# soham97/mellow

Hardware: AMD Instinct MI355X
Metric: audio-pair responses/sec (v0 167M, 2x10s clips, max_len=64, greedy) (higher is better)
Workload: dtype f32 (encoder/prefill GEMM operands split EXACTLY into 3 bf16 terms, 6 bf16 MFMA products per fp32 product, f32 accumulate: fp32-accurate, parity suite green; mel included, the STFT is an fp32 FFT; attentions and decode on exact fp32 MFMA / VALU)

## Files before the change

### mellow_amd/csrc/decode.hip

```cpp
#include "common.h"
#include "kernels.h"
#include <cstdio>
#include <mutex>
#include <set>
#include <type_traits>
#include <utility>

namespace mellow {

__device__ uint64_t* g_kdbg = nullptr;
#ifdef MELLOW_KDEBUG
__device__ __forceinline__ void kstamp(int slot, int idx, bool who) {
    if (g_kdbg && who) g_kdbg[slot * 8 + idx] = __builtin_readcyclecounter();
}
__device__ __forceinline__ void kspan(int seq, int end) {
    if (g_kdbg && seq >= 0 && seq < 480 && threadIdx.x == 0) {
        const unsigned long long t = wall_clock64();
        if (end) atomicMax(reinterpret_cast<unsigned long long*>(g_kdbg) + 64 + 2 * seq + 1, t);
        else atomicMin(reinterpret_cast<unsigned long long*>(g_kdbg) + 64 + 2 * seq, t);
    }
}
#else
#define kstamp(slot, idx, who) ((void)0)
#define kspan(seq, end) ((void)0)
#endif
void set_kernel_debug_buffer(uint64_t* p) { (void)hipMemcpyToSymbol(HIP_SYMBOL(g_kdbg), &p, sizeof(p)); }

__device__ __forceinline__ float fast_exp(float x) { return __builtin_amdgcn_exp2f(x * 1.44269504088896340736f); }
#ifdef MELLOW_NO_BLK_EXIT
#define MELLOW_BLK_EXIT(RB)
#else
#define MELLOW_BLK_EXIT(RB) if (BLK) { if (a.blk_live[RB] == 0) return; }
#endif
__device__ __forceinline__ float4 ldg_nt(const float4* p) {
#ifdef MELLOW_NO_NT
    return *p;
#else
    const f32x4 v = __builtin_nontemporal_load(reinterpret_cast<const f32x4*>(p));
    return make_float4(v[0], v[1], v[2], v[3]);
#endif
}
template <bool W8>
__device__ __forceinline__ float4 ldw(const float* __restrict__ Wp, int64_t slot) {
    if constexpr (W8) {
        const uint32_t u = __builtin_nontemporal_load(reinterpret_cast<const uint32_t*>(Wp) + slot);
        const auto lo = __builtin_amdgcn_cvt_pk_f32_fp8(u, false), hi = __builtin_amdgcn_cvt_pk_f32_fp8(u, true);
        return make_float4(lo[0], lo[1], hi[0], hi[1]);
    } else {
        return ldg_nt(reinterpret_cast<const float4*>(Wp) + slot);
    }
}
__device__ __forceinline__ uint32_t ldw8(const float* __restrict__ Wp, int64_t slot) {
    return __builtin_nontemporal_load(reinterpret_cast<const uint32_t*>(Wp) + slot);
}
__device__ __forceinline__ float f4amax(float4 v) { return fmaxf(fmaxf(fabsf(v.x), fabsf(v.y)), fmaxf(fabsf(v.z), fabsf(v.w))); }
__device__ __forceinline__ uint32_t q4_e4m3(float4 v, float inv) {
    int w = 0;
    w = __builtin_amdgcn_cvt_pk_fp8_f32(v.x * inv, v.y * inv, w, false);
    w = __builtin_amdgcn_cvt_pk_fp8_f32(v.z * inv, v.w * inv, w, true);
    return (uint32_t)w;
}
__device__ __forceinline__ long pk64(uint32_t lo, uint32_t hi) { return (long)(((uint64_t)hi << 32) | (uint64_t)lo); }
template <int N>
__device__ __forceinline__ f32x16 mfma8_32(f32x16 acc, const uint32_t (&w)[N], const uint32_t (&x)[N]) {
#pragma unroll
    for (int i = 0; i < N; i += 2)
        acc = __builtin_amdgcn_mfma_f32_32x32x16_fp8_fp8(pk64(w[i], i + 1 < N ? w[i + 1] : 0u), pk64(x[i], i + 1 < N ? x[i + 1] : 0u), acc, 0, 0, 0);
    return acc;
}
template <int N>
__device__ __forceinline__ f32x4 mfma8_16(f32x4 acc, const uint32_t (&w)[N], const uint32_t (&x)[N]) {
#pragma unroll
    for (int i = 0; i < N; i += 2)
        acc = __builtin_amdgcn_mfma_f32_16x16x32_fp8_fp8(pk64(w[i], i + 1 < N ? w[i + 1] : 0u), pk64(x[i], i + 1 < N ? x[i + 1] : 0u), acc, 0, 0, 0);
    return acc;
}
__device__ __forceinline__ void a8_scales(float amax, float& inv, float& sc) {
    inv = amax > 0.f ? 448.0f / amax : 0.f;
    sc = amax * (1.0f / 448.0f);
}
#ifndef MELLOW_ST_MODE
#define MELLOW_ST_MODE 0
#endif
__device__ __forceinline__ void st_out(float4* p, float4 v) {
#if MELLOW_ST_MODE == 1
    __builtin_nontemporal_store(f32x4{v.x, v.y, v.z, v.w}, reinterpret_cast<f32x4*>(p));
#elif MELLOW_ST_MODE == 2
    const f32x4 r = {v.x, v.y, v.z, v.w};
    asm volatile("global_store_dwordx4 %0, %1, off sc0 sc1" ::"v"(p), "v"(r) : "memory");
#else
    *p = v;
#endif
}
#ifdef MELLOW_HOIST_ON
#define MELLOW_HOIST(x) asm volatile("" ::"s"(x))
#else
#define MELLOW_HOIST(x) ((void)0)
#endif
__device__ __forceinline__ float4 f4add(float4 a, float4 b) { return make_float4(a.x + b.x, a.y + b.y, a.z + b.z, a.w + b.w); }
__device__ __forceinline__ float f4ssq(float4 v) { return (v.x * v.x + v.y * v.y) + (v.z * v.z + v.w * v.w); }
__device__ __forceinline__ f32x16 mfma4(f32x16 acc, float4 w, float4 x) {
    acc = __builtin_amdgcn_mfma_f32_32x32x2f32(w.x, x.x, acc, 0, 0, 0);
    acc = __builtin_amdgcn_mfma_f32_32x32x2f32(w.y, x.y, acc, 0, 0, 0);
    acc = __builtin_amdgcn_mfma_f32_32x32x2f32(w.z, x.z, acc, 0, 0, 0);
    acc = __builtin_amdgcn_mfma_f32_32x32x2f32(w.w, x.w, acc, 0, 0, 0);
    return acc;
}
__device__ __forceinline__ int64_t f32_idx(int rb, int K8, int m, int k) {
    return ((int64_t)rb * K8 + (k >> 3)) * 64 + m + 32 * ((k >> 2) & 1);
}

__device__ __forceinline__ void split_pair(float4 a, float4 b, i32x4& p0, i32x4& p1, i32x4& p2) {
    const float v[8] = {a.x, a.y, a.z, a.w, b.x, b.y, b.z, b.w};
    split8(v, p0, p1, p2);
}
#define MELLOW_BF16(W, X, ACC) ACC = __builtin_amdgcn_mfma_f32_32x32x16_bf16(__builtin_bit_cast(bf16x8, W), __builtin_bit_cast(bf16x8, X), ACC, 0, 0, 0)
__device__ __forceinline__ f32x16 mma6(f32x16 acc, const i32x4 (&w)[3], const i32x4 (&x)[3]) {
    MELLOW_BF16(w[2], x[0], acc);
    MELLOW_BF16(w[0], x[2], acc);
    MELLOW_BF16(w[1], x[1], acc);
    MELLOW_BF16(w[1], x[0], acc);
    MELLOW_BF16(w[0], x[1], acc);
    MELLOW_BF16(w[0], x[0], acc);
    return acc;
}

struct F3Quad { uint2 p[3]; };
__device__ __forceinline__ F3Quad f3_split4(float4 y) {
    __bf16 h[4], m[4], l[4];
    split3(y.x, h[0], m[0], l[0]); split3(y.y, h[1], m[1], l[1]); split3(y.z, h[2], m[2], l[2]); split3(y.w, h[3], m[3], l[3]);
    typedef __bf16 bf16x4 __attribute__((ext_vector_type(4)));
    F3Quad q;
    q.p[0] = __builtin_bit_cast(uint2, bf16x4{h[0], h[1], h[2], h[3]});
    q.p[1] = __builtin_bit_cast(uint2, bf16x4{m[0], m[1], m[2], m[3]});
    q.p[2] = __builtin_bit_cast(uint2, bf16x4{l[0], l[1], l[2], l[3]});
    return q;
}
__device__ __forceinline__ unsigned dpp_xor1(unsigned v) { return (unsigned)__builtin_amdgcn_update_dpp(0, (int)v, 0xB1, 0xF, 0xF, true); }
__device__ __forceinline__ F3Quad f3_partner(const F3Quad& q) {
    F3Quad o;
#pragma unroll
    for (int c = 0; c < 3; ++c) { o.p[c].x = dpp_xor1(q.p[c].x); o.p[c].y = dpp_xor1(q.p[c].y); }
    return o;
}
__device__ __forceinline__ void f3_store8(void* base, int64_t slot0, const F3Quad& lo, const F3Quad& hi) {
    uint4* p = reinterpret_cast<uint4*>(base) + slot0;
    p[0] = make_uint4(lo.p[0].x, lo.p[0].y, hi.p[0].x, hi.p[0].y);
    p[64] = make_uint4(lo.p[1].x, lo.p[1].y, hi.p[1].x, hi.p[1].y);
    p[128] = make_uint4(lo.p[2].x, lo.p[2].y, hi.p[2].x, hi.p[2].y);
}
__device__ __forceinline__ int64_t f3_32_slot(int rb, int KP, int m, int k) {
    return ((int64_t)rb * KP + (k >> 4)) * 3 * 64 + m + 32 * ((k >> 3) & 1);
}
__device__ __forceinline__ int64_t f3_16_slot(int rb, int KP, int m, int k) {
    return (((int64_t)rb * KP + (k >> 5)) * 2 + (m >> 4)) * 3 * 64 + (m & 15) + 16 * ((k >> 3) & 3);
}
__device__ __forceinline__ void pair_natural(float4& a, float4& b) {
    float* pa = &a.x; float* pb = &b.x;
#pragma unroll
    for (int j = 0; j < 4; ++j) {
        auto r = __builtin_amdgcn_permlane32_swap(__float_as_uint(pa[j]), __float_as_uint(pb[j]), false, false);
        pa[j] = __uint_as_float(r[0]);
        pb[j] = __uint_as_float(r[1]);
    }
}

#ifndef MELLOW_QKV_WAVES
#define MELLOW_QKV_WAVES 9
#endif
constexpr int QW = MELLOW_QKV_WAVES;
constexpr int QKV_THREADS = QW * 64 < 256 ? 256 : QW * 64;
template <int KCD, bool BLK, bool FIRST, int W8>
__global__ __launch_bounds__(QKV_THREADS) void dec_qkv_kernel(const float* __restrict__ Wp, const float* __restrict__ xmidF_p,
                                                              const float* __restrict__ dslabF_p, int K8p, const DecArgs a,
                                                              const float* __restrict__ wscale) {
    kspan(a.dbg_seq, 0);
    __shared__ __attribute__((aligned(16))) float red[QW * 16 * 64];
    __shared__ float ssq_s[QW * 32];
    const int tid = threadIdx.x, lane = tid & 63, wave = tid >> 6;
    const int nt = blockIdx.x, kc = blockIdx.y, rb = blockIdx.z;
    constexpr int KPW = 72 / (DEC_KC_QKV * QW);
    if (FIRST && nt == 29 && kc == 0 && rb == 0 && tid < 32) {
        const int p = *a.d_pos + a.inc_pos;
        const float c = a.rope_cos[(int64_t)p * 32 + tid], sn = a.rope_sin[(int64_t)p * 32 + tid];
        a.rope_cur[tid] = c;
        a.rope_cur[32 + tid] = sn;
        if (tid == 0 && a.inc_pos) *a.d_pos = p;
    }
    MELLOW_BLK_EXIT(rb)
    if (wave < QW) {
        const int k8_0 = (kc * QW + wave) * KPW;
        const int64_t wslot = ((int64_t)nt * K8p + k8_0) * 64 + lane;
        const float4* xb = reinterpret_cast<const float4*>(xmidF_p) + ((int64_t)rb * 72 + k8_0) * 64 + lane;
        const float4* sb = reinterpret_cast<const float4*>(dslabF_p) + ((int64_t)rb * 72 + k8_0) * 64 + lane;
        float4 w[KPW], x[KPW], sl[KPW][KCD > 0 ? KCD : 1];
        uint32_t w8[KPW];
#pragma unroll
        for (int i = 0; i < KPW; ++i) {
            if constexpr (W8 == 2) w8[i] = ldw8(Wp, wslot + i * 64);
            else w[i] = ldw<W8 != 0>(Wp, wslot + i * 64);
            x[i] = xb[i * 64];
#pragma unroll
            for (int s = 0; s < KCD; ++s) sl[i][s] = sb[(int64_t)s * a.slabF_stride4 + i * 64];
        }
        MELLOW_HOIST(a.pq); MELLOW_HOIST(a.rows); MELLOW_HOIST(a.ssq1); MELLOW_HOIST(a.xnewR);
        if (W8) MELLOW_HOIST(wscale);
        __builtin_amdgcn_sched_barrier(0);
        f32x16 acc;
#pragma unroll
        for (int r = 0; r < 16; ++r) acc[r] = 0.f;
        float ssp = 0.f;
#pragma unroll
        for (int i = 0; i < KPW; ++i) {
            float4 xv = x[i];
#pragma unroll
            for (int s = 0; s < KCD; ++s) xv = f4add(xv, sl[i][s]);
            if constexpr (W8 == 2) x[i] = xv;
            else acc = mfma4(acc, w[i], xv);
            if (nt == 0) ssp += f4ssq(xv);
            if (nt == 1)
                *reinterpret_cast<float4*>(a.xnewR + ((int64_t)rb * 32 + (lane & 31)) * 576 + (k8_0 + i) * 8 + (lane >> 5) * 4) = xv;
        }
        if constexpr (W8 == 2) {
            float am = 0.f, inv, sc;
#pragma unroll
            for (int i = 0; i < KPW; ++i) am = fmaxf(am, f4amax(x[i]));
            a8_scales(half_max(am), inv, sc);
            uint32_t xq[KPW];
#pragma unroll
            for (int i = 0; i < KPW; ++i) xq[i] = q4_e4m3(x[i], inv);
            acc = mfma8_32<KPW>(acc, w8, xq);
#pragma unroll
            for (int r = 0; r < 16; ++r) acc[r] *= sc;
        }
        if (nt == 0) {
            ssp = half_sum(ssp);
            if (lane < 32) ssq_s[wave * 32 + lane] = ssp;
        }
#pragma unroll
        for (int r = 0; r < 16; ++r) red[(wave * 16 + r) * 64 + lane] = acc[r];
    }
    __syncthreads();
    if (nt == 0 && tid < 32)
    {
        float ssum = ssq_s[tid & 31];
// ... 576 lines not shown
            acc = __builtin_amdgcn_mfma_f32_16x16x4f32(w[i].z, O.z * inv, acc, 0, 0, 0);
            acc = __builtin_amdgcn_mfma_f32_16x16x4f32(w[i].w, O.w * inv, acc, 0, 0, 0);
        }
    }
    if constexpr (W8 == 2) {
        float am = 0.f, inv, sc;
#pragma unroll
        for (int i = 0; i < TPW; ++i) am = fmaxf(am, f4amax(os[i][0]));
        am = fmaxf(am, swz_xor16(am));
        a8_scales(half_max(am), inv, sc);
        uint32_t xq[TPW];
#pragma unroll
        for (int i = 0; i < TPW; ++i) xq[i] = q4_e4m3(os[i][0], inv);
        acc = mfma8_16<TPW>(acc, w8, xq);
#pragma unroll
        for (int r = 0; r < 4; ++r) acc[r] *= sc;
    }
#pragma unroll
    for (int r = 0; r < 4; ++r) red[(wave * 4 + r) * 64 + lane] = acc[r];
    __syncthreads();
    if (tid < 64 && erow_ok) {
        const int src_lane = em + 16 * enq;
        float v[4] = {0.f, 0.f, 0.f, 0.f};
#pragma unroll
        for (int wv = 0; wv < OP_WAVES; ++wv)
#pragma unroll
            for (int r = 0; r < 4; ++r) v[r] += red[(wv * 4 + r) * 64 + src_lane];
        if (W8) {
#pragma unroll
            for (int r = 0; r < 4; ++r) v[r] *= wscale[nt * 16 + enq * 4 + r];
        }
        const float4 y = make_float4(xres.x + v[0], xres.y + v[1], xres.z + v[2], xres.w + v[3]);
        const int k = nt * 16 + enq * 4;
        st_out(reinterpret_cast<float4*>(a.xmidF) + f32_idx(rb, 72, mh * 16 + em, k), y);
        if (a.xmid3_32) {
            const F3Quad yq = f3_split4(y), yo = f3_partner(yq);
            if (!(enq & 1)) {
                f3_store8(a.xmid3_32, f3_32_slot(rb, 36, mh * 16 + em, k), yq, yo);
                f3_store8(a.xmid3_16, f3_16_slot(rb, 18, mh * 16 + em, k), yq, yo);
            }
        } else
        st_out(reinterpret_cast<float4*>(a.xmidF16) + (((int64_t)rb * 36 + nt) * 2 + mh) * 64 + em + 16 * enq, y);
        float ss = f4ssq(y);
        ss += dpp_mov<0xB1>(ss);
        ss += dpp_mov<0x4E>(ss);
        if (enq == 0) a.ssq[erow * 40 + nt] = ss;
    }
    kspan(a.dbg_seq, 1);
}

enum { OUT_LOGITS = 1 };
#ifndef MELLOW_LM_WAVES
#define MELLOW_LM_WAVES 8
#endif
constexpr int LM_WAVES = MELLOW_LM_WAVES;
template <int OUT, bool BLK, int W8>
__global__ __launch_bounds__(LM_WAVES * 64) void dec_fullk_kernel(const float* __restrict__ Wp, const float* __restrict__ XF, int K8p,
                                                        int N, const DecArgs a, const float* __restrict__ wscale) {
    kspan(a.dbg_seq, 0);
    __shared__ __attribute__((aligned(16))) float red[LM_WAVES * 16 * 64];
    constexpr int KPW = 72 / LM_WAVES;
    const int tid = threadIdx.x, lane = tid & 63, wave = tid >> 6;
    const int nt = blockIdx.x, rb = blockIdx.z;
    MELLOW_BLK_EXIT(rb)
    const int k8_0 = wave * KPW;
    const int64_t wslot = ((int64_t)nt * K8p + k8_0) * 64 + lane;
    const float4* xp = reinterpret_cast<const float4*>(XF) + ((int64_t)rb * 72 + k8_0) * 64 + lane;
    float4 w[KPW], x[KPW];
    uint32_t w8[KPW];
    const bool dbg = tid == 0 && nt == 0 && rb == 0;
    const int dslot = 5;
    kstamp(dslot, 0, dbg);
#pragma unroll
    for (int i = 0; i < KPW; ++i) {
        if constexpr (W8 == 2) w8[i] = ldw8(Wp, wslot + i * 64);
        else w[i] = ldw<W8 != 0>(Wp, wslot + i * 64);
        x[i] = xp[i * 64];
    }
    MELLOW_HOIST(a.logits); MELLOW_HOIST(a.cand_val); MELLOW_HOIST(a.cand_idx); MELLOW_HOIST(N);
    if (W8) MELLOW_HOIST(wscale);
    __builtin_amdgcn_sched_barrier(0);
    kstamp(dslot, 1, dbg);
    f32x16 acc;
#pragma unroll
    for (int r = 0; r < 16; ++r) acc[r] = 0.f;
    if constexpr (W8 == 2) {
        float am = 0.f, inv, sc;
#pragma unroll
        for (int i = 0; i < KPW; ++i) am = fmaxf(am, f4amax(x[i]));
        a8_scales(half_max(am), inv, sc);
        uint32_t xq[KPW];
#pragma unroll
        for (int i = 0; i < KPW; ++i) xq[i] = q4_e4m3(x[i], inv);
        acc = mfma8_32<KPW>(acc, w8, xq);
#pragma unroll
        for (int r = 0; r < 16; ++r) acc[r] *= sc;
    } else {
#pragma unroll
        for (int i = 0; i < KPW; ++i) acc = mfma4(acc, w[i], x[i]);
    }
    kstamp(dslot, 2, dbg && acc[0] == acc[0]);
#pragma unroll
    for (int r = 0; r < 16; ++r) red[(wave * 16 + r) * 64 + lane] = acc[r];
    __syncthreads();
    kstamp(dslot, 3, dbg);
    const bool epi = tid < 256;
    const int mm = tid & 31, hh = (tid >> 5) & 1, gq = (tid >> 6) & 3;
    float v[4];
#pragma unroll
    for (int j = 0; j < 4; ++j) {
        const int r = 4 * gq + j;
        float sacc = red[r * 64 + mm + 32 * hh];
#pragma unroll
        for (int wv = 1; wv < LM_WAVES; ++wv) sacc += red[(wv * 16 + r) * 64 + mm + 32 * hh];
        v[j] = sacc;
    }
    {
        const int n = nt * 32 + 8 * gq + 4 * hh;
        if (W8) {
#pragma unroll
            for (int j = 0; j < 4; ++j) v[j] *= wscale[n + j];
        }
        const int64_t row = (int64_t)rb * 32 + mm;
        if (epi && a.logits && n < N) *reinterpret_cast<float4*>(a.logits + row * N + n) = make_float4(v[0], v[1], v[2], v[3]);
        __syncthreads();
        float bv = v[0];
        int bi = n;
#pragma unroll
        for (int j = 1; j < 4; ++j)
            if (arg_better(v[j], n + j, bv, bi)) { bv = v[j]; bi = n + j; }
        if (epi) {
            red[tid] = bv;
            reinterpret_cast<int*>(red)[256 + tid] = bi;
        }
        __syncthreads();
        if (tid < 32) {
            float best = red[tid];
            int idx = reinterpret_cast<int*>(red)[256 + tid];
#pragma unroll
            for (int q = 1; q < 8; ++q) {
                const float ov = red[tid + 32 * q];
                const int oi = reinterpret_cast<int*>(red)[256 + tid + 32 * q];
                if (arg_better(ov, oi, best, idx)) { best = ov; idx = oi; }
            }
            const int64_t o = ((int64_t)rb * 32 + tid) * (N >> 5) + nt;
            a.cand_val[o] = best;
            a.cand_idx[o] = idx;
        }
    }
    kspan(a.dbg_seq, 1);
}


#ifndef MELLOW_H3_NW
#define MELLOW_H3_NW 8
#endif
#ifndef MELLOW_H3R_D1
#define MELLOW_H3R_D1 1
#endif
#ifndef MELLOW_H3R_D2
#define MELLOW_H3R_D2 1
#endif
#ifndef MELLOW_H3R_D4
#define MELLOW_H3R_D4 1
#endif
constexpr int H3_NW = MELLOW_H3_NW, H3_CP = 3, H3_NC = 36 / H3_CP;
template <int G, int D, bool BLK>
__global__ __launch_bounds__(H3_NW * 64) void dec_head3r_kernel(const float* __restrict__ Wp, const i32x4* __restrict__ X3, int K8p, int N,
                                                                int RB_p, const DecArgs a) {
    kspan(a.dbg_seq, 0);
    extern __shared__ __attribute__((aligned(16))) i32x4 xs[];
    constexpr int PPH = 36 / G, NCH = PPH / H3_CP;
    constexpr int STAGE = G * PPH * 3 * 64;
    static_assert(PPH * G == 36 && NCH * H3_CP == PPH && H3_NC % D == 0 && NCH % D == 0, "phases hold whole chunks");
    const int tid = threadIdx.x, lane = tid & 63, wave = tid >> 6;
    const int nt = blockIdx.x * H3_NW + wave;
    const float4* wbase = reinterpret_cast<const float4*>(Wp) + (int64_t)nt * K8p * 64 + lane;
    for (int rb0 = 0; rb0 < RB_p; rb0 += G) {
        const int gn = min(G, RB_p - rb0);
        f32x16 acc[G];
#pragma unroll
        for (int g = 0; g < G; ++g)
#pragma unroll
            for (int r = 0; r < 16; ++r) acc[g][r] = 0.f;
        float4 wn[D][2 * H3_CP];
#pragma unroll
        for (int d = 0; d < D; ++d)
#pragma unroll
            for (int i = 0; i < 2 * H3_CP; ++i) wn[d][i] = ldg_nt(wbase + (d * 2 * H3_CP + i) * 64);
        for (int ph = 0; ph < G; ++ph) {
            if (ph || rb0) __syncthreads();
            {
                constexpr int FILL = (STAGE + H3_NW * 64 - 1) / (H3_NW * 64);
                i32x4 t[FILL];
#pragma unroll
                for (int j = 0; j < FILL; ++j) {
                    const int i = tid + j * H3_NW * 64;
                    if (i < STAGE) {
                        const int g = i / (PPH * 3 * 64), rest = i % (PPH * 3 * 64);
                        t[j] = X3[(((int64_t)(rb0 + (g < gn ? g : 0)) * 36 + ph * PPH) * 3) * 64 + rest];
                    }
                }
#pragma unroll
                for (int j = 0; j < FILL; ++j) {
                    const int i = tid + j * H3_NW * 64;
                    if (i < STAGE) xs[i] = t[j];
                }
            }
            __syncthreads();
            for (int c0 = 0; c0 < NCH; c0 += D) {
#pragma unroll
                for (int d = 0; d < D; ++d) {
                    const int cc = c0 + d, c = ph * NCH + cc;
                    float4 w[2 * H3_CP];
#pragma unroll
                    for (int i = 0; i < 2 * H3_CP; ++i) w[i] = wn[d][i];
                    if (c + D < H3_NC) {
#pragma unroll
                        for (int i = 0; i < 2 * H3_CP; ++i) wn[d][i] = ldg_nt(wbase + ((c + D) * 2 * H3_CP + i) * 64);
                    }
                    __builtin_amdgcn_sched_barrier(0);
                    i32x4 wp[H3_CP][3];
#pragma unroll
                    for (int p = 0; p < H3_CP; ++p) {
                        pair_natural(w[2 * p], w[2 * p + 1]);
                        split_pair(w[2 * p], w[2 * p + 1], wp[p][0], wp[p][1], wp[p][2]);
                    }
                    const i32x4* st = xs + (cc * H3_CP) * 3 * 64 + lane;
#pragma unroll
                    for (int g = 0; g < G; ++g) {
                        if (g < gn) {
#pragma unroll
                            for (int p = 0; p < H3_CP; ++p) {
                                const i32x4 xq[3] = {st[((g * PPH + p) * 3 + 0) * 64], st[((g * PPH + p) * 3 + 1) * 64], st[((g * PPH + p) * 3 + 2) * 64]};
                                acc[g] = mma6(acc[g], wp[p], xq);
                            }
                        }
                    }
                    __builtin_amdgcn_sched_barrier(0);
                }
            }
        }
        const int m = lane & 31, h = lane >> 5;
#pragma unroll
        for (int g = 0; g < G; ++g) {
            if (g < gn && !(BLK && a.blk_live[rb0 + g] == 0)) {
                const int64_t row = (int64_t)(rb0 + g) * 32 + m;
                float bv = -INFINITY;
                int bi = 0x7fffffff;
#pragma unroll
                for (int q = 0; q < 4; ++q) {
                    const int n = nt * 32 + 8 * q + 4 * h;
                    if (a.logits) *reinterpret_cast<float4*>(a.logits + row * N + n) = make_float4(acc[g][4 * q], acc[g][4 * q + 1], acc[g][4 * q + 2], acc[g][4 * q + 3]);
#pragma unroll
                    for (int j = 0; j < 4; ++j)
                        if (arg_better(acc[g][4 * q + j], n + j, bv, bi)) { bv = acc[g][4 * q + j]; bi = n + j; }
                }
                auto rv = __builtin_amdgcn_permlane32_swap(__float_as_uint(bv), __float_as_uint(bv), false, false);
                auto ri = __builtin_amdgcn_permlane32_swap((unsigned)bi, (unsigned)bi, false, false);
                const float ov = __uint_as_float(h ? rv[0] : rv[1]);
                const int oi = (int)(h ? ri[0] : ri[1]);
                if (arg_better(ov, oi, bv, bi)) { bv = ov; bi = oi; }
                if (h == 0) {
                    const int64_t o = row * (N >> 5) + nt;
                    a.cand_val[o] = bv;
                    a.cand_idx[o] = bi;
                }
            }
        }
    }
    kspan(a.dbg_seq, 1);
}

#define MELLOW_BF16S(W, X, ACC) ACC = __builtin_amdgcn_mfma_f32_16x16x32_bf16(__builtin_bit_cast(bf16x8, W), __builtin_bit_cast(bf16x8, X), ACC, 0, 0, 0)
__device__ __forceinline__ f32x4 mma6s(f32x4 acc, const i32x4 (&w)[3], const i32x4 (&x)[3]) {
    MELLOW_BF16S(w[2], x[0], acc);
    MELLOW_BF16S(w[0], x[2], acc);
    MELLOW_BF16S(w[1], x[1], acc);
    MELLOW_BF16S(w[1], x[0], acc);
    MELLOW_BF16S(w[0], x[1], acc);
    MELLOW_BF16S(w[0], x[0], acc);
    return acc;
}
template <int NP, int NPA>
__device__ __forceinline__ void x3_load(i32x4 (&xq)[NPA][3], const i32x4* __restrict__ x3, int64_t off) {
#pragma unroll
    for (int p = 0; p < NP; ++p)
#pragma unroll
        for (int c = 0; c < 3; ++c) xq[p][c] = x3[off + (p * 3 + c) * 64];
}
template <int NP, int RBM, int NPA>
__device__ __forceinline__ void x3_tile_job(const i32x4 (&wp)[NPA][3], i32x4 (&xq)[2][NPA][3], const i32x4* __restrict__ x3 ,
                                            int64_t rb_stride, int rb0, int gn, f32x16 (&acc)[RBM]) {
#pragma unroll
    for (int g = 0; g < RBM; ++g) {
        if (g < gn) {
            if (g + 1 < RBM && g + 1 < gn) x3_load<NP, NPA>(xq[(g + 1) & 1], x3, (int64_t)(rb0 + g + 1) * rb_stride);
#pragma unroll
            for (int p = 0; p < NP; ++p) acc[g] = mma6(acc[g], wp[p], xq[g & 1][p]);
        }
    }
}
#ifndef MELLOW_Q3_WAVES
#define MELLOW_Q3_WAVES 6
#endif
constexpr int Q3W = MELLOW_Q3_WAVES;
template <int NP, int RBM, bool BLK>
__device__ __forceinline__ void q3_body(const float4* __restrict__ wp4, const i32x4* __restrict__ xsrc, int64_t rb_stride, int nt, int slab,
                                        bool side, int RB_p, const DecArgs& a, float* red) {
    const int tid = threadIdx.x, lane = tid & 63, wave = tid >> 6;
    i32x4 wp[NP][3];
    i32x4 xq[2][NP][3];
    constexpr bool ALL = RBM <= 2;
    {
        float4 w[2 * NP];
#pragma unroll
        for (int i = 0; i < 2 * NP; ++i) w[i] = ldg_nt(wp4 + i * 64);
        x3_load<NP, NP>(xq[0], xsrc, 0);
        if (ALL && RBM == 2 && RB_p > 1) x3_load<NP, NP>(xq[1], xsrc, rb_stride);
        __builtin_amdgcn_sched_barrier(0);
#pragma unroll
        for (int p = 0; p < NP; ++p) {
            pair_natural(w[2 * p], w[2 * p + 1]);
            split_pair(w[2 * p], w[2 * p + 1], wp[p][0], wp[p][1], wp[p][2]);
        }
    }
    for (int rb0 = 0; rb0 < RB_p; rb0 += RBM) {
        const int gn = min(RBM, RB_p - rb0);
        f32x16 acc[RBM];
#pragma unroll
        for (int g = 0; g < RBM; ++g)
#pragma unroll
            for (int r = 0; r < 16; ++r) acc[g][r] = 0.f;
        if (rb0) {
            x3_load<NP, NP>(xq[0], xsrc, (int64_t)rb0 * rb_stride);
            if (ALL && RBM == 2 && gn > 1) x3_load<NP, NP>(xq[1], xsrc, (int64_t)(rb0 + 1) * rb_stride);
        }
        if constexpr (ALL && RBM == 2) {
            if (gn > 1) {
#pragma unroll
                for (int p = 0; p < NP; ++p) {
#define MELLOW_Q3_TERM(PW, PX) MELLOW_BF16(wp[p][PW], xq[0][p][PX], acc[0]); MELLOW_BF16(wp[p][PW], xq[1][p][PX], acc[1]);
                    MELLOW_Q3_TERM(2, 0) MELLOW_Q3_TERM(0, 2) MELLOW_Q3_TERM(1, 1) MELLOW_Q3_TERM(1, 0) MELLOW_Q3_TERM(0, 1) MELLOW_Q3_TERM(0, 0)
#undef MELLOW_Q3_TERM
                }
            } else {
#pragma unroll
                for (int p = 0; p < NP; ++p) acc[0] = mma6(acc[0], wp[p], xq[0][p]);
            }
        } else if constexpr (ALL) {
#pragma unroll
            for (int p = 0; p < NP; ++p) acc[0] = mma6(acc[0], wp[p], xq[0][p]);
        } else {
            x3_tile_job<NP, RBM, NP>(wp, xq, xsrc, rb_stride, rb0, gn, acc);
        }
        if (rb0) __syncthreads();
#pragma unroll
        for (int g = 0; g < RBM; ++g)
#pragma unroll
            for (int r = 0; r < 16; ++r) red[((wave * RBM + g) * 16 + r) * 64 + lane] = acc[g][r];
        __syncthreads();
        if (tid < 256) {
            const int mm = tid & 31, hh = (tid >> 5) & 1, gq = tid >> 6;
            const int n = nt * 32 + 8 * gq + 4 * hh;
            for (int g = 0; g < gn; ++g) {
                const int rb = rb0 + g;
                if (BLK && a.blk_live[rb] == 0) continue;
                float v[4];
#pragma unroll
                for (int j = 0; j < 4; ++j) {
                    const int q = 4 * gq + j;
                    float sacc = red[((0 * RBM + g) * 16 + q) * 64 + mm + 32 * hh];
#pragma unroll
                    for (int wv = 1; wv < Q3W; ++wv) sacc += red[((wv * RBM + g) * 16 + q) * 64 + mm + 32 * hh];
                    v[j] = sacc;
                }
                const float4 o = make_float4(v[0], v[1], v[2], v[3]);
                if (side) st_out(reinterpret_cast<float4*>(a.dslabF) + (int64_t)slab * a.slabF_stride4 + f32_idx(rb, 72, mm, n), o);
                else st_out(reinterpret_cast<float4*>(a.pq + ((int64_t)slab * a.rows + rb * 32 + mm) * 960 + n), o);
            }
        }
    }
}
template <bool BLK, int RBM>
__global__ __launch_bounds__(Q3W * 64) void dec_qkv2x3_kernel(const float* __restrict__ Wx, const float* __restrict__ Wh,
                                                              const float* __restrict__ Wd, const i32x4* __restrict__ xmid3,
                                                              const i32x4* __restrict__ h3, int K8x, int K8h, int RB_p, const DecArgs a) {
    kspan(a.dbg_seq, 0);
    extern __shared__ __attribute__((aligned(16))) float red_dyn[];
    const int lane = threadIdx.x & 63, wave = threadIdx.x >> 6;
    const int b = blockIdx.x;
    constexpr int XP = 18 / Q3W, HP = (96 / Q2_HC) / Q3W;
    static_assert(XP * Q3W == 18 && HP * Q3W * Q2_HC == 96 && Q3W * 64 >= 256, "waves must divide the k-chunks into whole pairs; the epilogue is 256 threads wide");
    if (b < 60) {
        const int nt = b % 30, slab = b / 30;
        const int T0 = slab * 18 + wave * XP;
        q3_body<XP, RBM, BLK>(reinterpret_cast<const float4*>(Wx) + ((int64_t)nt * K8x + 2 * T0) * 64 + lane, xmid3 + (int64_t)T0 * 3 * 64 + lane,
                              (int64_t)36 * 3 * 64, nt, slab, false, RB_p, a, red_dyn);
    } else {
        const int idx = b - 60, hc = idx / 48, nt = idx % 48;
        const bool side = nt >= 30;
        const int T0 = hc * (96 / Q2_HC) + wave * HP;
        const float4* wp4 = side ? reinterpret_cast<const float4*>(Wd) + ((int64_t)(nt - 30) * 192 + 2 * T0) * 64 + lane
                                 : reinterpret_cast<const float4*>(Wh) + ((int64_t)nt * K8h + 2 * T0) * 64 + lane;
        q3_body<HP, RBM, BLK>(wp4, h3 + (int64_t)T0 * 3 * 64 + lane, (int64_t)96 * 3 * 64, side ? nt - 30 : nt, side ? hc : 2 + hc, side, RB_p, a, red_dyn);
    }
    kspan(a.dbg_seq, 1);
}

#ifndef MELLOW_GU3_WAVES
#define MELLOW_GU3_WAVES 6
#endif
#ifndef MELLOW_G3_ABL
#define MELLOW_G3_ABL 0
#endif
constexpr int GU3W = MELLOW_GU3_WAVES;
template <bool BLK, int RBM>
__global__ __launch_bounds__(GU3W * 64) void dec_gateup3_kernel(const float* __restrict__ Wp16, const i32x4* __restrict__ x3,
                                                                const float* __restrict__ ssq_in, int RB_p, const DecArgs a) {
    kspan(a.dbg_seq, 0);
    extern __shared__ __attribute__((aligned(16))) float red_dyn[];
// ... 64 lines not shown
                    for (int p = 0; p < NP; ++p)
#pragma unroll
                        for (int c = 0; c < 6; ++c) xq[(g + 1) & 1][p][c / 3][c % 3] = xsrc[(int64_t)(rb0 + g + 1) * RBS + (p * 6 + c) * 64];
                }
#pragma unroll
                for (int p = 0; p < NP; ++p) {
                    if (MELLOW_G3_ABL & 2) { acc0[g][0] += __int_as_float(wp[p][0][0] ^ xq[g & 1][p][0][0][0]); acc1[g][1] += __int_as_float(wp[p][2][1] ^ xq[g & 1][p][1][2][1]); continue; }
#define MELLOW_G3_TERM(PW, PX) MELLOW_BF16S(wp[p][PW], xq[g & 1][p][0][PX], acc0[g]); MELLOW_BF16S(wp[p][PW], xq[g & 1][p][1][PX], acc1[g]);
                    MELLOW_G3_TERM(2, 0) MELLOW_G3_TERM(0, 2) MELLOW_G3_TERM(1, 1) MELLOW_G3_TERM(1, 0) MELLOW_G3_TERM(0, 1) MELLOW_G3_TERM(0, 0)
#undef MELLOW_G3_TERM
                }
            }
        }
        if (rb0) __syncthreads();
#pragma unroll
        for (int g = 0; g < RBM; ++g)
#pragma unroll
            for (int r = 0; r < 4; ++r) {
                red[((wave * RBM + g) * 8 + r) * 64 + lane] = acc0[g][r];
                red[((wave * RBM + g) * 8 + 4 + r) * 64 + lane] = acc1[g][r];
            }
        __syncthreads();
        static_assert(RBM * 64 <= 2 * GU3W * 64, "two epilogue rounds cover a pass");
#pragma unroll
        for (int k = 0; k < 2; ++k) {
            const int e = tid + k * GU3W * 64;
            if (e >= gn * 64 || (k == 1 && RBM * 64 <= GU3W * 64)) continue;
            const int g = e >> 6, t = e & 63, rb = rb0 + g;
            if (BLK && a.blk_live[rb] == 0) continue;
            const int m = t >> 1, q = t & 1;
            const int gl = (m & 15) + 16 * q, ul = gl + 32, rbase = (m >> 4) * 4;
            float ss = 0.f;
#pragma unroll
            for (int j = 0; j < 9; ++j) ss += (s4[k][j].x + s4[k][j].y) + (s4[k][j].z + s4[k][j].w);
            const float r2 = 1.0f / sqrtf(ss / 576.0f + a.eps);
            float h[4];
#pragma unroll
            for (int r = 0; r < 4; ++r) {
                float gv = red[((0 * RBM + g) * 8 + rbase + r) * 64 + gl], uv = red[((0 * RBM + g) * 8 + rbase + r) * 64 + ul];
#pragma unroll
                for (int wv = 1; wv < GU3W; ++wv) {
                    gv += red[((wv * RBM + g) * 8 + rbase + r) * 64 + gl];
                    uv += red[((wv * RBM + g) * 8 + rbase + r) * 64 + ul];
                }
                h[r] = __fmul_rn(siluf_(gv * r2), uv * r2);
            }
            const float4 hv = make_float4(h[0], h[1], h[2], h[3]);
            if (!(MELLOW_G3_ABL & 16)) st_out(reinterpret_cast<float4*>(a.guF) + ((int64_t)rb * 192 + nt) * 64 + m + 32 * q, hv);
            const F3Quad hq = f3_split4(hv), ho = f3_partner(hq);
            if (!(MELLOW_G3_ABL & 1) && q == 0) f3_store8(a.h3, f3_32_slot(rb, 96, m, 8 * nt), hq, ho);
        }
    }
    kspan(a.dbg_seq, 1);
}

#ifndef MELLOW_GU_WAVES
#define MELLOW_GU_WAVES 4
#endif
constexpr int GU_WAVES = MELLOW_GU_WAVES;
template <bool BLK, int W8>
__global__ __launch_bounds__(GU_WAVES * 64) void dec_gateup16_kernel(const float* __restrict__ Wp16, const float* __restrict__ xF16,
                                                                     const float* __restrict__ ssq_in, const DecArgs a,
                                                                     const float* __restrict__ wscale) {
    kspan(a.dbg_seq, 0);
    __shared__ __attribute__((aligned(16))) float red[GU_WAVES * 8 * 64];
    constexpr int K16 = 36, TPW = K16 / GU_WAVES;
    static_assert(TPW * GU_WAVES == K16, "waves must divide the 36 k16-tiles");
    const int tid = threadIdx.x, lane = tid & 63, wave = tid >> 6;
    const int nt = blockIdx.x, rb = blockIdx.y;
    MELLOW_BLK_EXIT(rb)
    const int t0 = wave * TPW;
    const int64_t wslot = ((int64_t)nt * K16 + t0) * 64 + lane;
    const float4* xp = reinterpret_cast<const float4*>(xF16) + (((int64_t)rb * 36 + t0) * 2) * 64 + lane;
    const float4* sq = reinterpret_cast<const float4*>(ssq_in + ((int64_t)rb * 32 + ((tid >> 1) & 31)) * 40);
    float4 w[TPW], x0[TPW], x1[TPW], s4[9];
    uint32_t w8[TPW];
#pragma unroll
    for (int i = 0; i < TPW; ++i) {
        if constexpr (W8 == 2) w8[i] = ldw8(Wp16, wslot + i * 64);
        else w[i] = ldw<W8 != 0>(Wp16, wslot + i * 64);
        x0[i] = xp[(i * 2) * 64];
        x1[i] = xp[(i * 2 + 1) * 64];
    }
    if (tid < 64) {
#pragma unroll
        for (int j = 0; j < 9; ++j) s4[j] = sq[j];
    }
    MELLOW_HOIST(a.eps); MELLOW_HOIST(a.guF);
    if (W8) MELLOW_HOIST(wscale);
    __builtin_amdgcn_sched_barrier(0);
    f32x4 acc0 = {0.f, 0.f, 0.f, 0.f}, acc1 = {0.f, 0.f, 0.f, 0.f};
    if constexpr (W8 == 2) {
        float am0 = 0.f, am1 = 0.f, inv0, sc0, inv1, sc1;
#pragma unroll
        for (int i = 0; i < TPW; ++i) { am0 = fmaxf(am0, f4amax(x0[i])); am1 = fmaxf(am1, f4amax(x1[i])); }
        am0 = fmaxf(am0, swz_xor16(am0)); am1 = fmaxf(am1, swz_xor16(am1));
        a8_scales(half_max(am0), inv0, sc0);
        a8_scales(half_max(am1), inv1, sc1);
        uint32_t q0[TPW], q1[TPW];
#pragma unroll
        for (int i = 0; i < TPW; ++i) { q0[i] = q4_e4m3(x0[i], inv0); q1[i] = q4_e4m3(x1[i], inv1); }
        acc0 = mfma8_16<TPW>(acc0, w8, q0);
        acc1 = mfma8_16<TPW>(acc1, w8, q1);
#pragma unroll
        for (int r = 0; r < 4; ++r) { acc0[r] *= sc0; acc1[r] *= sc1; }
    } else {
#pragma unroll
    for (int i = 0; i < TPW; ++i) {
        acc0 = __builtin_amdgcn_mfma_f32_16x16x4f32(w[i].x, x0[i].x, acc0, 0, 0, 0);
        acc1 = __builtin_amdgcn_mfma_f32_16x16x4f32(w[i].x, x1[i].x, acc1, 0, 0, 0);
        acc0 = __builtin_amdgcn_mfma_f32_16x16x4f32(w[i].y, x0[i].y, acc0, 0, 0, 0);
        acc1 = __builtin_amdgcn_mfma_f32_16x16x4f32(w[i].y, x1[i].y, acc1, 0, 0, 0);
        acc0 = __builtin_amdgcn_mfma_f32_16x16x4f32(w[i].z, x0[i].z, acc0, 0, 0, 0);
        acc1 = __builtin_amdgcn_mfma_f32_16x16x4f32(w[i].z, x1[i].z, acc1, 0, 0, 0);
        acc0 = __builtin_amdgcn_mfma_f32_16x16x4f32(w[i].w, x0[i].w, acc0, 0, 0, 0);
        acc1 = __builtin_amdgcn_mfma_f32_16x16x4f32(w[i].w, x1[i].w, acc1, 0, 0, 0);
    }
    }
#pragma unroll
    for (int r = 0; r < 4; ++r) {
        red[(wave * 8 + r) * 64 + lane] = acc0[r];
        red[(wave * 8 + 4 + r) * 64 + lane] = acc1[r];
    }
    __syncthreads();
    if (tid < 64) {
        const int m = tid >> 1, q = tid & 1;
        const int gl = (m & 15) + 16 * q, ul = gl + 32, rbase = (m >> 4) * 4;
        float ss = 0.f;
#pragma unroll
        for (int j = 0; j < 9; ++j) ss += (s4[j].x + s4[j].y) + (s4[j].z + s4[j].w);
        const float r2 = 1.0f / sqrtf(ss / 576.0f + a.eps);
        float h[4];
#pragma unroll
        for (int r = 0; r < 4; ++r) {
            float gv = red[(rbase + r) * 64 + gl], uv = red[(rbase + r) * 64 + ul];
#pragma unroll
            for (int wv = 1; wv < GU_WAVES; ++wv) {
                gv += red[(wv * 8 + rbase + r) * 64 + gl];
                uv += red[(wv * 8 + rbase + r) * 64 + ul];
            }
            if (W8) { gv *= wscale[nt * 16 + 4 * q + r]; uv *= wscale[nt * 16 + 8 + 4 * q + r]; }
            h[r] = __fmul_rn(siluf_(gv * r2), uv * r2);
        }
        st_out(reinterpret_cast<float4*>(a.guF) + ((int64_t)rb * 192 + nt) * 64 + m + 32 * q, make_float4(h[0], h[1], h[2], h[3]));
    }
    kspan(a.dbg_seq, 1);
}

#ifndef MELLOW_DOWN_WAVES
#define MELLOW_DOWN_WAVES 4
#endif
constexpr int DN_WAVES = MELLOW_DOWN_WAVES;
static_assert(DN_WAVES >= 4 && 192 % (8 * DN_WAVES) == 0, "the epilogue needs 256 threads; waves must divide the k-tiles");
template <bool BLK, int W8>
__global__ __launch_bounds__(DN_WAVES * 64) void dec_down_kernel(const float* __restrict__ Wp, const float* __restrict__ guF_p, int K8p,
                                                                 const DecArgs a, const float* __restrict__ wscale) {
    kspan(a.dbg_seq, 0);
    __shared__ __attribute__((aligned(16))) float red[DN_WAVES * 16 * 64];
    constexpr int KPW = 192 / (DEC_KC_DOWN * DN_WAVES);
    const int tid = threadIdx.x, lane = tid & 63, wave = tid >> 6;
    const int nt = blockIdx.x, kc = blockIdx.y, rb = blockIdx.z;
    MELLOW_BLK_EXIT(rb)
    const int k8_0 = (kc * DN_WAVES + wave) * KPW;
    const int64_t wslot = ((int64_t)nt * K8p + k8_0) * 64 + lane;
    const float4* hp = reinterpret_cast<const float4*>(guF_p) + ((int64_t)rb * 192 + k8_0) * 64 + lane;
    const bool dbg = tid == 0 && nt == 0 && kc == 0 && rb == 0;
    kstamp(4, 0, dbg);
    float4 w[KPW], h4[KPW];
    uint32_t w8[KPW];
#pragma unroll
    for (int i = 0; i < KPW; ++i) {
        if constexpr (W8 == 2) w8[i] = ldw8(Wp, wslot + i * 64);
        else w[i] = ldw<W8 != 0>(Wp, wslot + i * 64);
        h4[i] = hp[i * 64];
    }
    MELLOW_HOIST(a.dslabF); MELLOW_HOIST(a.slabF_stride4);
    if (W8) MELLOW_HOIST(wscale);
    __builtin_amdgcn_sched_barrier(0);
    kstamp(4, 1, dbg);
    f32x16 acc;
#pragma unroll
    for (int q = 0; q < 16; ++q) acc[q] = 0.f;
    if constexpr (W8 == 2) {
        float am = 0.f, inv, sc;
#pragma unroll
        for (int i = 0; i < KPW; ++i) am = fmaxf(am, f4amax(h4[i]));
        a8_scales(half_max(am), inv, sc);
        uint32_t xq[KPW];
#pragma unroll
        for (int i = 0; i < KPW; ++i) xq[i] = q4_e4m3(h4[i], inv);
        acc = mfma8_32<KPW>(acc, w8, xq);
#pragma unroll
        for (int q = 0; q < 16; ++q) acc[q] *= sc;
    } else {
#pragma unroll
        for (int i = 0; i < KPW; ++i) acc = mfma4(acc, w[i], h4[i]);
    }
    kstamp(4, 2, dbg && acc[0] == acc[0]);
#pragma unroll
    for (int q = 0; q < 16; ++q) red[(wave * 16 + q) * 64 + lane] = acc[q];
    __syncthreads();
    kstamp(4, 3, dbg);
    if (tid < 256) {
        const int mm = tid & 31, hh = (tid >> 5) & 1, gq = tid >> 6;
        float v[4];
#pragma unroll
        for (int j = 0; j < 4; ++j) {
            const int q = 4 * gq + j;
            float sacc = 0.f;
#pragma unroll
            for (int wv = 0; wv < DN_WAVES; ++wv) sacc += red[(wv * 16 + q) * 64 + mm + 32 * hh];
            v[j] = sacc;
        }
        const int n = nt * 32 + 8 * gq + 4 * hh;
        if (W8) {
#pragma unroll
            for (int j = 0; j < 4; ++j) v[j] *= wscale[n + j];
        }
        reinterpret_cast<float4*>(a.dslabF)[(int64_t)kc * a.slabF_stride4 + f32_idx(rb, 72, mm, n)] = make_float4(v[0], v[1], v[2], v[3]);
    }
    kstamp(4, 4, dbg);
    kspan(a.dbg_seq, 1);
}

template <bool BLK, int Q2W, int W8>
__global__ __launch_bounds__(Q2W * 64) void dec_qkv2_kernel(const float* __restrict__ Wx, const float* __restrict__ Wh,
                                                            const float* __restrict__ Wd, const float* __restrict__ xmidF_p,
                                                            const float* __restrict__ guF_p, int K8x, int K8h, const DecArgs a,
                                                            const float* __restrict__ sc_x, const float* __restrict__ sc_h,
                                                            const float* __restrict__ sc_d) {
    kspan(a.dbg_seq, 0);
    __shared__ __attribute__((aligned(16))) float red[Q2W * 16 * 64];
    const int tid = threadIdx.x, lane = tid & 63, wave = tid >> 6;
    const int b = blockIdx.x, rb = blockIdx.y;
    MELLOW_BLK_EXIT(rb)
    const bool dbg = tid == 0 && b == 60 && rb == 0;
    kstamp(7, 0, dbg);
    constexpr int XT = 36 / Q2W, HT = (192 / Q2_HC) / Q2W;
    static_assert(XT * Q2W == 36 && HT * Q2W * Q2_HC == 192, "waves must divide the k-chunks");
    f32x16 acc;
#pragma unroll
    for (int r = 0; r < 16; ++r) acc[r] = 0.f;
    int nt, slab;
    bool side = false;
    const float* wsc = sc_x;
    if (b < 60) {
        nt = b % 30; slab = b / 30;
        const int k8_0 = slab * 36 + wave * XT;
        const int64_t wslot = ((int64_t)nt * K8x + k8_0) * 64 + lane;
        const float4* xb = reinterpret_cast<const float4*>(xmidF_p) + ((int64_t)rb * 72 + k8_0) * 64 + lane;
        float4 w[XT], x[XT];
        uint32_t w8[XT];
#pragma unroll
        for (int i = 0; i < XT; ++i) {
            if constexpr (W8 == 2) w8[i] = ldw8(Wx, wslot + i * 64);
            else w[i] = ldw<W8 != 0>(Wx, wslot + i * 64);
            x[i] = xb[i * 64];
        }
        MELLOW_HOIST(a.pq); MELLOW_HOIST(a.rows);
        if (W8) MELLOW_HOIST(sc_x);
        __builtin_amdgcn_sched_barrier(0);
        if constexpr (W8 == 2) {
            float am = 0.f, inv, sc;
#pragma unroll
            for (int i = 0; i < XT; ++i) am = fmaxf(am, f4amax(x[i]));
            a8_scales(half_max(am), inv, sc);
            uint32_t xq[XT];
#pragma unroll
            for (int i = 0; i < XT; ++i) xq[i] = q4_e4m3(x[i], inv);
            acc = mfma8_32<XT>(acc, w8, xq);
#pragma unroll
            for (int r = 0; r < 16; ++r) acc[r] *= sc;
        } else {
#pragma unroll
            for (int i = 0; i < XT; ++i) acc = mfma4(acc, w[i], x[i]);
        }
    } else {
        const int idx = b - 60, hc = idx / 48;
        nt = idx % 48;
        side = nt >= 30;
        slab = side ? hc : 2 + hc;
        wsc = side ? sc_d : sc_h;
        const int k8_0 = hc * (192 / Q2_HC) + wave * HT;
        const float* wbase = side ? Wd : Wh;
        const int64_t wslot = side ? ((int64_t)(nt - 30) * 192 + k8_0) * 64 + lane : ((int64_t)nt * K8h + k8_0) * 64 + lane;
        const float4* hp = reinterpret_cast<const float4*>(guF_p) + ((int64_t)rb * 192 + k8_0) * 64 + lane;
        float4 w[HT], h4[HT];
        uint32_t w8[HT];
#pragma unroll
        for (int i = 0; i < HT; ++i) {
            if constexpr (W8 == 2) w8[i] = ldw8(wbase, wslot + i * 64);
            else w[i] = ldw<W8 != 0>(wbase, wslot + i * 64);
            h4[i] = hp[i * 64];
        }
        MELLOW_HOIST(a.pq); MELLOW_HOIST(a.rows); MELLOW_HOIST(a.dslabF); MELLOW_HOIST(a.slabF_stride4);
        if (W8) MELLOW_HOIST(wsc);
        __builtin_amdgcn_sched_barrier(0);
        kstamp(7, 1, dbg);
        if constexpr (W8 == 2) {
            float am = 0.f, inv, sc;
#pragma unroll
            for (int i = 0; i < HT; ++i) am = fmaxf(am, f4amax(h4[i]));
            a8_scales(half_max(am), inv, sc);
            uint32_t xq[HT];
#pragma unroll
            for (int i = 0; i < HT; ++i) xq[i] = q4_e4m3(h4[i], inv);
            acc = mfma8_32<HT>(acc, w8, xq);
#pragma unroll
            for (int r = 0; r < 16; ++r) acc[r] *= sc;
        } else {
#pragma unroll
            for (int i = 0; i < HT; ++i) acc = mfma4(acc, w[i], h4[i]);
        }
        kstamp(7, 2, dbg && acc[0] == acc[0]);
        if (side) nt -= 30;
    }
#pragma unroll
    for (int r = 0; r < 16; ++r) red[(wave * 16 + r) * 64 + lane] = acc[r];
    __syncthreads();
    kstamp(7, 3, dbg);
    if (tid < 256) {
        const int mm = tid & 31, hh = (tid >> 5) & 1, gq = tid >> 6;
        float v[4];
#pragma unroll
        for (int j = 0; j < 4; ++j) {
            const int q = 4 * gq + j;
            float sacc = red[q * 64 + mm + 32 * hh];
#pragma unroll
            for (int wv = 1; wv < Q2W; ++wv) sacc += red[(wv * 16 + q) * 64 + mm + 32 * hh];
            v[j] = sacc;
        }
        const int n = nt * 32 + 8 * gq + 4 * hh;
        if (W8) {
#pragma unroll
            for (int j = 0; j < 4; ++j) v[j] *= wsc[n + j];
        }
        const float4 o = make_float4(v[0], v[1], v[2], v[3]);
        if (side) st_out(reinterpret_cast<float4*>(a.dslabF) + (int64_t)slab * a.slabF_stride4 + f32_idx(rb, 72, mm, n), o);
        else st_out(reinterpret_cast<float4*>(a.pq + ((int64_t)slab * a.rows + rb * 32 + mm) * 960 + n), o);
    }
    kstamp(7, 4, dbg);
    kspan(a.dbg_seq, 1);
}

template <int KCD, bool BLK>
__global__ __launch_bounds__(192) void dec_final_norm_kernel(const float* __restrict__ norm_w, const float* __restrict__ xmidF_p,
                                                             const float* __restrict__ dslabF_p, int64_t stride4_p, const DecArgs a) {
    kspan(a.dbg_seq, 0);
    __shared__ float part[3];
    const int b = blockIdx.x, tid = threadIdx.x;
    if (BLK && b == 0 && tid < 32) a.blk_snap[tid] = a.blk_live[tid];
    MELLOW_BLK_EXIT(b >> 5)
    const int xi = tid < 144 ? tid : 0;
    const int64_t fi = f32_idx(b >> 5, 72, b & 31, xi * 4);
    float4 v = reinterpret_cast<const float4*>(xmidF_p)[fi];
    float4 xs[KCD > 0 ? KCD : 1];
#pragma unroll
    for (int s = 0; s < KCD; ++s) xs[s] = reinterpret_cast<const float4*>(dslabF_p)[(int64_t)s * stride4_p + fi];
    const float4 wv = reinterpret_cast<const float4*>(norm_w)[xi];
#pragma unroll
    for (int s = 0; s < KCD; ++s) v = f4add(v, xs[s]);
    float ss = tid < 144 ? f4ssq(v) : 0.f;
    ss = wave_sum(ss);
    if ((tid & 63) == 0) part[tid >> 6] = ss;
    __syncthreads();
    const float r = 1.0f / sqrtf((part[0] + part[1] + part[2]) / 576.0f + a.eps);
    if (tid < 144) {
        float4 y;
        y.x = __fmul_rn(wv.x, __fmul_rn(v.x, r)); y.y = __fmul_rn(wv.y, __fmul_rn(v.y, r));
        y.z = __fmul_rn(wv.z, __fmul_rn(v.z, r)); y.w = __fmul_rn(wv.w, __fmul_rn(v.w, r));
        if (!a.xn3) reinterpret_cast<float4*>(a.xnF)[fi] = y;
    }
// ... 85 lines not shown
    const int tid = threadIdx.x, lane = tid & 63, wave = tid >> 6;
    const int nblk = (B + 31) >> 5;
    int row = -1, active = 0;
    if (tid < B) {
        row = lp.row_of_slot[tid];
        active = row >= 0 && lp.blk_live[tid >> 5] != 0 && lp.seen_stop[row] == 0;
    }
    const unsigned long long m = __ballot(active);
    const int before = __popcll(m & ((1ull << lane) - 1ull));
    if (lane == 0) wsum[wave] = __popcll(m);
    if (tid == 0) {
        int live = 0;
        for (int k = 0; k < nblk; ++k) live += lp.blk_live[k] != 0;
        n_live_s = live;
    }
    src_of[tid] = -1;
    row_new[tid] = -1;
    __syncthreads();
    int base = 0;
    for (int w = 0; w < wave; ++w) base += wsum[w];
    if (tid == 0) {
        int n = 0;
        for (int w = 0; w < 16; ++w) n += wsum[w];
        n_act_s = n;
    }
    __syncthreads();
    const int n_act = n_act_s;
    if ((n_act + 31) / 32 >= n_live_s) return;
    if (active) { src_of[base + before] = tid; row_new[base + before] = row; }
    __syncthreads();
    float4* x = reinterpret_cast<float4*>(a.xmidF);
    for (int d0 = 0; d0 < n_act; d0 += 7) {
        const int d = d0 + tid / 144, c = tid % 144;
        const bool mv = tid < 1008 && d < n_act && src_of[d] != d;
        float4 v = make_float4(0.f, 0.f, 0.f, 0.f);
        if (mv) v = x[f32_idx(src_of[d] >> 5, 72, src_of[d] & 31, c * 4)];
        __syncthreads();
        if (mv) x[f32_idx(d >> 5, 72, d & 31, c * 4)] = v;
        __syncthreads();
    }
    if (tid < B) lp.row_of_slot[tid] = row_new[tid];
    if (tid < 32) {
        const int left = tid < nblk ? min(max(n_act - 32 * tid, 0), 32) : 0;
        lp.blk_left[tid] = left;
        lp.blk_live[tid] = left > 0;
    }
    if (tid == 0) *lp.n_compactions += 1;
}
__global__ __launch_bounds__(256) void kv_to_bf16_kernel(const float4* __restrict__ src, uint4* __restrict__ dst, int64_t n8) {
    for (int64_t i = (int64_t)blockIdx.x * 256 + threadIdx.x; i < n8; i += (int64_t)gridDim.x * 256) {
        const float4 a = src[2 * i], b = src[2 * i + 1];
        typedef __bf16 bf16x8v __attribute__((ext_vector_type(8)));
        const bf16x8v o = {static_cast<__bf16>(a.x), static_cast<__bf16>(a.y), static_cast<__bf16>(a.z), static_cast<__bf16>(a.w),
                           static_cast<__bf16>(b.x), static_cast<__bf16>(b.y), static_cast<__bf16>(b.z), static_cast<__bf16>(b.w)};
        dst[i] = __builtin_bit_cast(uint4, o);
    }
}
void launch_kv_to_bf16(const float* src, void* dst, int64_t n, hipStream_t s) {
    const int64_t n8 = n >> 3;
    const int blocks = (int)((n8 + 255) / 256 < 8192 ? (n8 + 255) / 256 : 8192);
    hipLaunchKernelGGL(kv_to_bf16_kernel, dim3(blocks), dim3(256), 0, s, reinterpret_cast<const float4*>(src), reinterpret_cast<uint4*>(dst), n8);
}
void launch_dec_compact(const DecArgs& a, int B, const LoopArgs& loop, hipStream_t s) {
    hipLaunchKernelGGL(dec_compact_kernel, dim3(1), dim3(1024), 0, s, a, B, loop);
}

__global__ __launch_bounds__(192) void dec_load_rows_kernel(const DecArgs a, const float* __restrict__ in, int64_t ld,
                                                            const int32_t* __restrict__ row_ids, int T_last, int n_src) {
    const int b = blockIdx.x, tid = threadIdx.x;
    const int64_t src = row_ids ? (int64_t)min(max(row_ids[b], 0), n_src - 1) : (int64_t)b * T_last + (T_last - 1);
    if (tid < 144) {
        const float4 e = reinterpret_cast<const float4*>(in + src * ld)[tid];
        reinterpret_cast<float4*>(a.xmidF)[f32_idx(b >> 5, 72, b & 31, tid * 4)] = e;
    }
}

void set_max_dynamic_lds(const void* fn, size_t bytes) {
    if (bytes <= 64 * 1024) return;
    static std::mutex mu;
    static std::set<std::pair<const void*, int>> done;
    int dev = 0;
    (void)hipGetDevice(&dev);
    std::lock_guard<std::mutex> lk(mu);
    if (done.insert({fn, dev}).second) {
        const hipError_t e = hipFuncSetAttribute(fn, hipFuncAttributeMaxDynamicSharedMemorySize, (int)bytes);
        if (e != hipSuccess) fprintf(stderr, "mellow: hipFuncSetAttribute(max dynamic LDS %zu) failed: %s\n", bytes, hipGetErrorString(e));
    }
}
template <class F> static inline void with_bool(bool v, F&& f) {
    if (v) f(std::true_type{}); else f(std::false_type{});
}
template <int V0, int... Vs, class F> static inline void with_int(int v, F&& f) {
    if constexpr (sizeof...(Vs) == 0) f(std::integral_constant<int, V0>{});
    else if (v == V0) f(std::integral_constant<int, V0>{});
    else with_int<Vs...>(v, f);
}
static inline int w8_mode(const DecArgs& a, const float* wscale) { return wscale ? (a.a8 ? 2 : 1) : 0; }
template <class F> static inline void with_blk_w8(const DecArgs& a, const float* wscale, F&& f) {
    with_bool(a.blk_live != nullptr, [&](auto blk) { with_int<2, 1, 0>(w8_mode(a, wscale), [&](auto w8) { f(blk, w8); }); });
}
void launch_dec_qkv(const DecArgs& a, const float* Wp, int K8p, int kcd, hipStream_t s, const float* wscale) {
    const dim3 grid(30, DEC_KC_QKV, a.RB);
    with_int<0, DEC_KC_DOWN>(kcd, [&](auto kcd_c) { with_bool(a.first != 0, [&](auto first) { with_blk_w8(a, wscale, [&](auto blk, auto w8) {
        hipLaunchKernelGGL((dec_qkv_kernel<kcd_c.value, blk.value, first.value, w8.value>), grid, dim3(QKV_THREADS), 0, s, Wp, (const float*)a.xmidF,
                           (const float*)a.dslabF, K8p, a, wscale);
    }); }); });
}
void launch_dec_attn(const DecArgs& a, float* k_cache, float* v_cache, bool fused, hipStream_t s) {
    const dim3 grid(3, a.rows, a.ts);
    const bool one = a.RB == 1 && !a.blk_live;
    if (a.ts != DEC_TS && (one || a.kv16 || a.ts != DEC_TS_MULTI)) {
        fprintf(stderr, "mellow: decode attention launched with %d key splits at RB = %d\n", a.ts, a.RB);
        abort();
    }
    auto launch = [&](auto blk, auto one_c) { with_bool(fused, [&](auto fused_c) { with_bool(a.kv16 != 0, [&](auto kv16) {
        constexpr bool ONE = one_c.value, KV16 = kv16.value;
        constexpr int NW = !KV16 ? DA_WAVES : MELLOW_DA16_MFMA && DA_WAVES == 8 && !ONE ? MELLOW_DA16_NW : DA_WAVES;
        constexpr int TSM = ONE || KV16 ? DEC_TS : DEC_TS_MULTI;
        with_int<DEC_TS, TSM>(a.ts, [&](auto ts) {
            hipLaunchKernelGGL((dec_attn_kernel<blk.value, fused_c.value, ONE, KV16, NW, ts.value>), grid, dim3(NW * 64), 0, s, k_cache, v_cache,
                               (const int32_t*)a.d_pos, (const float*)a.pq, (const float*)a.xmidF, a.Tmax, a.gs, a.rows, a);
        });
    }); }); };
    if (one) launch(std::false_type{}, std::true_type{});
    else with_bool(a.blk_live != nullptr, [&](auto blk) { launch(blk, std::false_type{}); });
}
static void launch_dec_qkv2_any(const DecArgs& a, const float* Wx, int K8x, const float* Wh, int K8h, const float* Wd,
                                const float* sc_x, const float* sc_h, const float* sc_d, hipStream_t s) {
    const dim3 grid(Q2_BLOCKS, a.RB);
#ifdef MELLOW_Q2_WAVES_FORCED
    bool few = false;
#else
    bool few = a.RB == 1;
#endif
    if (w8_mode(a, sc_x) == 2) few = false;
    with_bool(few, [&](auto few_c) { with_blk_w8(a, sc_x, [&](auto blk, auto w8) {
        constexpr int WV = few_c.value ? 4 : Q2_WAVES;
        hipLaunchKernelGGL((dec_qkv2_kernel<blk.value, WV, w8.value>), grid, dim3(WV * 64), 0, s, Wx, Wh, Wd, (const float*)a.xmidF,
                           (const float*)a.guF, K8x, K8h, a, sc_x, sc_h, sc_d);
    }); });
}
constexpr size_t dec_qkv2x3_lds(int rbm) { return (size_t)Q3W * rbm * 16 * 64 * 4; }
constexpr size_t dec_gateup3_lds(int rbm) { return (size_t)GU3W * rbm * 8 * 64 * 4; }
constexpr size_t dec_head3r_lds() { return (size_t)36 * 3 * 64 * 16; }
template <class F> static inline void with_qkv2x3(int rb, bool blk, F&& f) {
    with_int<1, 2, 4>(rb, [&](auto rbm) { with_bool(blk, [&](auto b) { f(&dec_qkv2x3_kernel<b.value, rbm.value>, dec_qkv2x3_lds(rbm.value)); }); });
}
template <class F> static inline void with_gateup3(int rb, bool blk, F&& f) {
    with_int<1, 2, 4>(rb, [&](auto rbm) { with_bool(blk, [&](auto b) { f(&dec_gateup3_kernel<b.value, rbm.value>, dec_gateup3_lds(rbm.value)); }); });
}
template <class F> static inline void with_head3r(int rb, bool blk, F&& f) {
    with_int<1, 2, 4>(rb, [&](auto g) { with_bool(blk, [&](auto b) {
        constexpr int G = g.value, D = G == 1 ? MELLOW_H3R_D1 : G == 2 ? MELLOW_H3R_D2 : MELLOW_H3R_D4;
        f(&dec_head3r_kernel<G, D, b.value>, dec_head3r_lds());
    }); });
}
void launch_dec_qkv2x3(const DecArgs& a, const float* Wq2, const float* Wd, hipStream_t s) {
    const float* Wh = Wq2 + (size_t)72 * 64 * 4;
    const i32x4 *x3 = reinterpret_cast<const i32x4*>(a.xmid3_32), *h3 = reinterpret_cast<const i32x4*>(a.h3);
    with_qkv2x3(a.RB, a.blk_live != nullptr, [&](auto* kernel, size_t lds) {
        set_max_dynamic_lds(reinterpret_cast<const void*>(kernel), lds);
        hipLaunchKernelGGL(kernel, dim3(Q2_BLOCKS), dim3(Q3W * 64), lds, s, Wq2, Wh, Wd, x3, h3, Q2_K8, Q2_K8, a.RB, a);
    });
}
void launch_dec_gateup3(const DecArgs& a, const float* Wp16, hipStream_t s) {
    const i32x4* x3 = reinterpret_cast<const i32x4*>(a.xmid3_16);
    with_gateup3(a.RB, a.blk_live != nullptr, [&](auto* kernel, size_t lds) {
        set_max_dynamic_lds(reinterpret_cast<const void*>(kernel), lds);
        hipLaunchKernelGGL(kernel, dim3(192), dim3(GU3W * 64), lds, s, Wp16, x3, (const float*)a.ssq, a.RB, a);
    });
}
void launch_dec_qkv2(const DecArgs& a, const float* Wq2, const float* Wd, hipStream_t s) {
    launch_dec_qkv2_any(a, Wq2, Q2_K8, Wq2 + (size_t)72 * 64 * 4, Q2_K8, Wd, nullptr, nullptr, nullptr, s);
}
void launch_dec_qkv2_w8(const DecArgs& a, const float* Wx8, const float* sc_x, const float* Wh8, const float* sc_h,
                        const float* Wd8, const float* sc_d, hipStream_t s) {
    launch_dec_qkv2_any(a, Wx8, 72, Wh8, 192, Wd8, sc_x, sc_h, sc_d, s);
}
__global__ __launch_bounds__(256) void compose_f64_kernel(const float* __restrict__ A, const float* __restrict__ B, float* __restrict__ C,
                                                          int M, int N, int K) {
    __shared__ double as[16][17], bs[16][17];
    const int tx = threadIdx.x & 15, ty = threadIdx.x >> 4;
    const int m = blockIdx.y * 16 + ty, n = blockIdx.x * 16 + tx;
    double acc = 0.0;
    for (int k0 = 0; k0 < K; k0 += 16) {
        as[ty][tx] = (m < M && k0 + tx < K) ? (double)A[(int64_t)m * K + k0 + tx] : 0.0;
        bs[ty][tx] = (k0 + ty < K && n < N) ? (double)B[(int64_t)(k0 + ty) * N + n] : 0.0;
        __syncthreads();
#pragma unroll
        for (int kk = 0; kk < 16; ++kk) acc += as[ty][kk] * bs[kk][tx];
        __syncthreads();
    }
    if (m < M && n < N) C[(int64_t)m * N + n] = (float)acc;
}
void launch_compose_f64(const float* A, const float* B, float* C, int M, int N, int K, hipStream_t s) {
    hipLaunchKernelGGL(compose_f64_kernel, dim3((N + 15) / 16, (M + 15) / 16), dim3(256), 0, s, A, B, C, M, N, K);
}
int dec_attn_chunk_groups(bool kv16) { return DA_WAVES * (kv16 && MELLOW_DA16_MFMA ? DA_GM : DA_G); }
void launch_dec_oproj(const DecArgs& a, const float* Wp16, hipStream_t s, const float* wscale) {
#ifdef MELLOW_OPROJ_ROWS
    const int rows = MELLOW_OPROJ_ROWS;
#else
    const int rows = a.RB == 1 ? 8 : 16;
#endif
    with_int<8, 16>(rows, [&](auto rows_c) { with_int<1, DEC_TS>(a.ts, [&](auto ts) { with_blk_w8(a, wscale, [&](auto blk, auto w8) {
        constexpr int ROWS = rows_c.value, PARTS = ROWS == 8 ? 4 : 2;
        hipLaunchKernelGGL((dec_oproj_kernel<blk.value, w8.value, ROWS, ts.value>), dim3(36, PARTS * a.RB), dim3(OP_WAVES * 64), 0, s, Wp16,
                           (const float*)a.attF16, (const float*)a.att_ml, (const float*)a.xnewR, a.RB, a.rows, a, wscale);
    }); }); });
}
void launch_dec_gateup(const DecArgs& a, const float* Wp16, hipStream_t s, const float* wscale) {
    with_blk_w8(a, wscale, [&](auto blk, auto w8) {
        hipLaunchKernelGGL((dec_gateup16_kernel<blk.value, w8.value>), dim3(192, a.RB), dim3(GU_WAVES * 64), 0, s, Wp16, a.xmidF16, a.ssq, a, wscale);
    });
}
void launch_dec_down(const DecArgs& a, const float* Wp, int K8p, hipStream_t s, const float* wscale) {
    with_blk_w8(a, wscale, [&](auto blk, auto w8) {
        hipLaunchKernelGGL((dec_down_kernel<blk.value, w8.value>), dim3(18, DEC_KC_DOWN, a.RB), dim3(DN_WAVES * 64), 0, s, Wp, (const float*)a.guF,
                           K8p, a, wscale);
    });
}
void launch_dec_final_norm(const DecArgs& a, const float* norm_w, int kcd, hipStream_t s) {
    with_int<0, DEC_KC_DOWN>(kcd, [&](auto kcd_c) { with_bool(a.blk_live != nullptr, [&](auto blk) {
        hipLaunchKernelGGL((dec_final_norm_kernel<kcd_c.value, blk.value>), dim3(a.rows), dim3(192), 0, s, norm_w, (const float*)a.xmidF,
                           (const float*)a.dslabF, a.slabF_stride4, a);
    }); });
}
bool dec_head3r_fits(int vocab) { return vocab % 32 == 0 && (vocab / 32) % H3_NW == 0; }
void launch_dec_lm_head(const DecArgs& a, const float* Wp, int K8p, int vocab, hipStream_t s, const float* wscale) {
    if ((a.x3 & DEC_X3_HEAD) && !wscale && a.xn3 && (vocab / 32) % H3_NW == 0) {
        const i32x4* X3 = reinterpret_cast<const i32x4*>(a.xn3);
        with_head3r(a.RB, a.blk_live != nullptr, [&](auto* kernel, size_t lds) {
            set_max_dynamic_lds(reinterpret_cast<const void*>(kernel), lds);
            hipLaunchKernelGGL(kernel, dim3(vocab / 32 / H3_NW), dim3(H3_NW * 64), lds, s, Wp, X3, K8p, vocab, a.RB, a);
        });
        return;
    }
    with_blk_w8(a, wscale, [&](auto blk, auto w8) {
        hipLaunchKernelGGL((dec_fullk_kernel<OUT_LOGITS, blk.value, w8.value>), dim3(vocab / 32, 1, a.RB), dim3(LM_WAVES * 64), 0, s, Wp,
                           (const float*)a.xnF, K8p, vocab, a, wscale);
    });
}
void dec_prepare_lds_attributes() {
    const auto raise = [](auto* kernel, size_t lds) { set_max_dynamic_lds(reinterpret_cast<const void*>(kernel), lds); };
    for (const int rb : {1, 2, 4})
        for (const bool blk : {false, true}) {
            with_head3r(rb, blk, raise);
            with_qkv2x3(rb, blk, raise);
            with_gateup3(rb, blk, raise);
        }
}
__global__ __launch_bounds__(256) void pack_dec_fp8_kernel(const float4* __restrict__ Wp, int slots, int rows, uint32_t* __restrict__ out,
                                                           float* __restrict__ scale) {
    __shared__ unsigned amax_s[32];
    __shared__ float inv_s[32];
    const int tile = blockIdx.x, tid = threadIdx.x;
    if (tid < 32) amax_s[tid] = 0u;
    __syncthreads();
    const float4* src = Wp + (int64_t)tile * slots;
    for (int i = tid; i < slots; i += 256) {
        const float4 v = src[i];
        const float m = fmaxf(fmaxf(fabsf(v.x), fabsf(v.y)), fmaxf(fabsf(v.z), fabsf(v.w)));
        atomicMax(&amax_s[(i & 63) & (rows - 1)], __float_as_uint(m));
    }
    __syncthreads();
    if (tid < rows) {
        const float am = __uint_as_float(amax_s[tid]);
        const float sc = am > 0.f ? am / 448.0f : 1.0f;
        scale[(int64_t)tile * rows + tid] = sc;
        inv_s[tid] = 1.0f / sc;
    }
    __syncthreads();
    for (int i = tid; i < slots; i += 256) {
        const float4 v = src[i];
        const float inv = inv_s[(i & 63) & (rows - 1)];
        int w = 0;
        w = __builtin_amdgcn_cvt_pk_fp8_f32(v.x * inv, v.y * inv, w, false);
        w = __builtin_amdgcn_cvt_pk_fp8_f32(v.z * inv, v.w * inv, w, true);
        out[(int64_t)tile * slots + i] = (uint32_t)w;
    }
}
void launch_pack_dec_fp8(const float* Wp, int tiles, int slots_per_tile, int rows_per_tile, void* out, float* scale, hipStream_t s) {
    hipLaunchKernelGGL(pack_dec_fp8_kernel, dim3(tiles), dim3(256), 0, s, reinterpret_cast<const float4*>(Wp), slots_per_tile,
                       rows_per_tile, reinterpret_cast<uint32_t*>(out), scale);
}
void launch_dec_argmax(const DecArgs& a, int B, int n_tiles, int32_t* tokens, const float* embed, int write_x,
                       const LoopArgs& loop, hipStream_t s) {
    hipLaunchKernelGGL(dec_argmax_kernel, dim3(B), dim3(256), 0, s, (const float*)a.cand_val, (const int32_t*)a.cand_idx, n_tiles, a, tokens, embed,
                       write_x, loop);
}
void launch_dec_load_rows(const DecArgs& a, int B, const float* in, int64_t ld, const int32_t* row_ids, int T_last,
                          int n_src, hipStream_t s) {
    hipLaunchKernelGGL(dec_load_rows_kernel, dim3(B), dim3(192), 0, s, a, in, ld, row_ids, T_last, n_src);
}

__global__ __launch_bounds__(1024) void argmax_kernel(const float* __restrict__ logits, int V, int64_t ld,
                                                      int32_t* __restrict__ tokens) {
    __shared__ float bv[16];
    __shared__ int bi[16];
    const int b = blockIdx.x, tid = threadIdx.x;
    const float4* row = reinterpret_cast<const float4*>(logits + (int64_t)b * ld);
    float best = -INFINITY;
    int idx = 0x7fffffff;
    for (int i = tid; i < (V >> 2); i += 1024) {
        const float4 v = row[i];
        const float vv[4] = {v.x, v.y, v.z, v.w};
#pragma unroll
        for (int j = 0; j < 4; ++j)
            if (arg_better(vv[j], 4 * i + j, best, idx)) { best = vv[j]; idx = 4 * i + j; }
    }
#pragma unroll
    for (int off = 32; off > 0; off >>= 1) {
        const float ov = __shfl_xor(best, off, 64);
        const int oi = __shfl_xor(idx, off, 64);
        if (arg_better(ov, oi, best, idx)) { best = ov; idx = oi; }
    }
    if ((tid & 63) == 0) { bv[tid >> 6] = best; bi[tid >> 6] = idx; }
    __syncthreads();
    if (tid == 0) {
        for (int w = 1; w < 16; ++w)
            if (arg_better(bv[w], bi[w], best, idx)) { best = bv[w]; idx = bi[w]; }
        tokens[b] = min(max(idx, 0), V - 1);
    }
}
void launch_argmax(const float* logits, int B, int V, int64_t ld, int32_t* tokens, hipStream_t s) {
    hipLaunchKernelGGL(argmax_kernel, dim3(B), dim3(1024), 0, s, logits, V, ld, tokens);
}

__global__ void pack_weight16_kernel(const float* __restrict__ w, int N, int K, float* __restrict__ out) {
    const int64_t total = (int64_t)(N / 16) * (K / 16) * 64;
    for (int64_t i = (int64_t)blockIdx.x * blockDim.x + threadIdx.x; i < total; i += (int64_t)gridDim.x * blockDim.x) {
        const int lane = (int)(i & 63);
        const int64_t tile = i >> 6;
        const int k16 = (int)(tile % (K / 16)), nt = (int)(tile / (K / 16));
        const int n = nt * 16 + (lane & 15), k0 = k16 * 16 + 4 * (lane >> 4);
        reinterpret_cast<float4*>(out)[i] = *reinterpret_cast<const float4*>(w + (int64_t)n * K + k0);
    }
}
__global__ void pack_weight16n_kernel(const float* __restrict__ w, int N, int K, float* __restrict__ out) {
    const int64_t total = (int64_t)(N / 16) * (K / 32) * 128;
    for (int64_t i = (int64_t)blockIdx.x * blockDim.x + threadIdx.x; i < total; i += (int64_t)gridDim.x * blockDim.x) {
        const int lane = (int)(i & 63), half = (int)((i >> 6) & 1);
        const int64_t tile = i >> 7;
        const int T = (int)(tile % (K / 32)), nt = (int)(tile / (K / 32));
        const int n = nt * 16 + (lane & 15), k0 = T * 32 + 8 * (lane >> 4) + 4 * half;
        reinterpret_cast<float4*>(out)[i] = *reinterpret_cast<const float4*>(w + (int64_t)n * K + k0);
    }
}
void launch_pack_weight16n(const float* w, int N, int K, float* out, hipStream_t s) {
    const int64_t total = (int64_t)(N / 16) * (K / 32) * 128;
    const int blocks = (int)((total + 255) / 256 < 4096 ? (total + 255) / 256 : 4096);
    hipLaunchKernelGGL(pack_weight16n_kernel, dim3(blocks), dim3(256), 0, s, w, N, K, out);
}
void launch_pack_weight16(const float* w, int N, int K, float* out, hipStream_t s) {
    const int64_t total = (int64_t)(N / 16) * (K / 16) * 64;
    const int blocks = (int)((total + 255) / 256 < 4096 ? (total + 255) / 256 : 4096);
    hipLaunchKernelGGL(pack_weight16_kernel, dim3(blocks), dim3(256), 0, s, w, N, K, out);
}

}
```

### mellow_amd/csrc/engine.cpp

```cpp
#include "engine_internal.h"

static thread_local std::string g_err;
int fail(const char* fmt, ...) {
    char buf[1024];
    va_list ap;
    va_start(ap, fmt);
    vsnprintf(buf, sizeof(buf), fmt, ap);
    va_end(ap);
    g_err = buf;
    return 1;
}
int ensure(mellow_engine* e, mellow_engine::Buf& b, size_t floats) {
    if (b.cap >= floats) return 0;
    if (b.p) HIPCHK(hipFree(b.p));
    b.p = nullptr;
    b.cap = 0;
    HIPCHK(hipMalloc(&b.p, floats * sizeof(float)));
    b.cap = floats;
    return 0;
}
int dev_alloc(mellow_engine* e, float** out, size_t floats) {
    const size_t bytes = (floats * sizeof(float) + 4095) / 4096 * 4096;
    if (!e->arena) {
        const size_t want = (size_t)(e->opt.arena_mb < 0 ? 0 : e->opt.arena_mb) << 20;
// ... 113 lines not shown
        for (int wc = 0; wc < nwc; ++wc)
            for (int i = 0; i < ws; ++i)
                for (int j = 0; j < ws; ++j) {
                    const int hs = wr * ws + i, wsx = wc * ws + j;
                    const int m = (wr * nwc + wc) * ws * ws + i * ws + j;
                    out[m] = ((hs + shift) % R) * R + (wsx + shift) % R;
                }
}
void pack_weight_host(const float* w, int N, int K, int NP, int KP, float* out) {
    const int K8 = KP / 8;
    for (int nt = 0; nt < NP / 32; ++nt)
        for (int k8 = 0; k8 < K8; ++k8)
            for (int lane = 0; lane < 64; ++lane)
                for (int j = 0; j < 4; ++j) {
                    const int n = nt * 32 + (lane & 31), k = k8 * 8 + 4 * (lane >> 5) + j;
                    out[(((int64_t)nt * K8 + k8) * 64 + lane) * 4 + j] = (n < N && k < K) ? w[(int64_t)n * K + k] : 0.f;
                }
}

void rope_tables_host(float theta, int head_dim, int P, float* c, float* s) {
    const int half = head_dim / 2;
    for (int i = 0; i < half; ++i) {
        const float x = (float)(2 * i) / (float)head_dim;
        const float inv = 1.0f / (float)pow((double)theta, (double)x);
        for (int p = 0; p < P; ++p) {
            const float a = inv * (float)p;
            c[(size_t)p * half + i] = (float)cos((double)a);
            s[(size_t)p * half + i] = (float)sin((double)a);
        }
    }
}

extern "C" {

int mellow_abi_version(void) { return MELLOW_ABI_VERSION; }
int mellow_host_rope_tables(float theta, int head_dim, int max_pos, float* cos_out, float* sin_out) {
    if (!(theta > 0.f) || head_dim <= 0 || head_dim % 2 || max_pos <= 0 || !cos_out || !sin_out) return fail("bad rope table arguments");
    rope_tables_host(theta, head_dim, max_pos, cos_out, sin_out);
    return 0;
}
const char* mellow_last_error(void) { return g_err.c_str(); }
int mellow_device_count(void) {
    int n = 0;
    if (hipGetDeviceCount(&n) != hipSuccess) return 0;
    return n;
}
int mellow_engine_num_required(void) { return (int)default_required().size(); }
const char* mellow_engine_required_key(int i) {
    const auto& k = default_required();
    if (i < 0 || i >= (int)k.size()) return nullptr;
    return k[i].c_str();
}
int mellow_prof_num_families(void) { return PF_COUNT; }
const char* mellow_prof_family_name(int i) { return (i >= 0 && i < PF_COUNT) ? kFamilyNames[i] : nullptr; }

int mellow_host_window_map(int R, int shift, int32_t* out) {
    if (R <= 0 || (R % 8 && R > 8) || !out) return fail("bad window map arguments");
    window_map_host(R, shift, out);
    return 0;
}
int mellow_host_pack_weight(const float* w, int N, int K, int npad, float* out, int64_t out_capacity) {
    if (!w || !out || N <= 0 || K <= 0 || npad <= 0 || npad % 32) return fail("bad pack arguments");
    const int NP = rup(N, npad), KP = rup(K, 32);
    if (out_capacity < (int64_t)NP * KP) return fail("pack output too small: need %lld floats", (long long)NP * KP);
    pack_weight_host(w, N, K, NP, KP, out);
    return 0;
}

int mellow_engine_create(const mellow_config_t* cfg, int device, mellow_engine_t** out) {
    if (!cfg || !out) return fail("null argument");
    if (cfg->abi_version != MELLOW_ABI_VERSION) return fail("ABI version mismatch: caller %d, library %d", cfg->abi_version, MELLOW_ABI_VERSION);
    if (cfg->hidden_size != 576 || cfg->head_dim != 64 || cfg->num_heads != 9 || cfg->num_kv_heads != 3 ||
        cfg->intermediate_size != 1536)
        return fail("unsupported decoder geometry (engine is built for SmolLM2-135M: hidden 576, 9q/3kv heads x 64, inter 1536)");
    if (cfg->prefix_len != 2 * 129 + 2 + cfg->text_len) return fail("prefix_len must be 2*129+2+text_len");
    if (cfg->vocab_size % 128) return fail("vocab_size must be a multiple of 128");
    int n = 0;
    if (hipGetDeviceCount(&n) != hipSuccess || n <= 0) return fail("no HIP device available: the Mellow engine has no CPU fallback");
    if (device < 0 || device >= n) return fail("device %d out of range (%d devices)", device, n);
    HIPCHK(hipSetDevice(device));
    mellow_engine* e = new mellow_engine();
    e->cfg = *cfg;
    e->device = device;
    HIPCHK(hipStreamCreateWithFlags(&e->stream, hipStreamNonBlocking));
    HIPCHK(hipEventCreateWithFlags(&e->ev_fork, hipEventDisableTiming));
    for (int i = 0; i < 3; ++i) HIPCHK(hipEventCreateWithFlags(&e->ev_join[i], hipEventDisableTiming));
    for (int i = 0; i < 4; ++i) HIPCHK(hipEventCreate(&e->ev_phase[i]));
    *out = e;
    return mellow_engine_set_precision(e, MELLOW_PRECISION_F32X3);
}

void mellow_engine_destroy(mellow_engine_t* e) {
    if (!e) return;
    hipSetDevice(e->device);
    if (e->stream) hipStreamSynchronize(e->stream);
    if (e->parent && --e->parent->n_forks == 0) e->parent->prefill_parts = e->parent->prefill_parts_saved;
    e->graphs.reset();
    for (void* p : e->allocs) hipFree(p);
    for (auto ev : e->ev_pool) hipEventDestroy(ev);
    for (int i = 0; i < 4; ++i)
        if (e->ev_phase[i]) hipEventDestroy(e->ev_phase[i]);
    if (e->d_tokens) hipFree(e->d_tokens);
    if (e->h_progress) hipHostFree(e->h_progress);
    if (e->ev_fork) hipEventDestroy(e->ev_fork);
    for (int i = 0; i < 3; ++i) {
        if (e->ev_join[i]) hipEventDestroy(e->ev_join[i]);
        if (e->stream2[i]) hipStreamDestroy(e->stream2[i]);
    }
    if (e->stream) hipStreamDestroy(e->stream);
    delete e;
}

int mellow_engine_load_tensor(mellow_engine_t* e, const char* key, const void* data, const int64_t* shape, int ndim,
                              int dtype) {
    if (!e || !key || !data) return fail("null argument");
    if (e->finalized) return fail("engine already finalized");
    std::string k = key;
    if (k.rfind("module.", 0) == 0) k = k.substr(7);
    if (is_ignored_key(k)) return 0;
    bool known = (k == "mellow.rope_cos" || k == "mellow.rope_sin");
    if (!known) {
        for (const auto& r : build_required(&e->cfg))
            if (r == k) { known = true; break; }
    }
    if (!known) return fail("unexpected key in state_dict: %s", key);
    HostTensor t;
    t.dtype = dtype;
    for (int i = 0; i < ndim; ++i) t.shape.push_back(shape[i]);
    const size_t esz = dtype == MELLOW_I64 ? 8 : 4;
    t.data.resize((size_t)t.numel() * esz);
    HIPCHK(hipSetDevice(e->device));
    HIPCHK(hipMemcpy(t.data.data(), data, t.data.size(), hipMemcpyDefault));
    e->host[k] = std::move(t);
    return 0;
}

}

int alloc_state_words(mellow_engine* e) {
    HIPCHK(hipMalloc(&e->d_tokens, 4096 * sizeof(int32_t)));
    HIPCHK(hipMemset(e->d_tokens, 0, 4096 * sizeof(int32_t)));
    e->d_step = e->d_tokens + 1024;
    e->d_pos = e->d_tokens + 1025;
    e->d_nseen = e->d_tokens + 1026;
    e->d_arrive = e->d_tokens + 1027;
    e->d_ticket = e->d_tokens + 1028;
    e->d_params = e->d_tokens + 1032;
    e->d_sparams = reinterpret_cast<uint32_t*>(e->d_tokens + 1536);
    e->d_blk_left = e->d_tokens + 1040;
    e->d_blk_live = e->d_tokens + 1072;
    e->d_seen = e->d_tokens + 2048;
    e->d_row_of_slot = e->d_tokens + 3072;
    e->d_ncompact = e->d_tokens + 1029;
    HIPCHK(hipHostMalloc(reinterpret_cast<void**>(&e->h_progress), 64, hipHostMallocMapped | hipHostMallocCoherent));
    *e->h_progress = 0;
    HIPCHK(hipHostGetDevicePointer(reinterpret_cast<void**>(&e->d_progress), e->h_progress, 0));
    return 0;
}

__global__ void stream_probe_kernel(unsigned long long* out, unsigned long long ticks) {
    const unsigned long long t0 = wall_clock64();
    out[0] = t0;
    while (wall_clock64() - t0 < ticks) __builtin_amdgcn_s_sleep(8);
    out[1] = wall_clock64();
}
static int streams_overlap(mellow_engine* e, hipStream_t a, hipStream_t b, bool* yes) {
    unsigned long long* d = nullptr;
    HIPCHK(hipMalloc(&d, 4 * sizeof(unsigned long long)));
    HIPCHK(hipMemsetAsync(d, 0, 4 * sizeof(unsigned long long), a));
    HIPCHK(hipStreamSynchronize(a));
    HIPCHK(hipStreamSynchronize(b));
    hipLaunchKernelGGL(stream_probe_kernel, dim3(1), dim3(1), 0, a, d, 20000ull);
    hipLaunchKernelGGL(stream_probe_kernel, dim3(1), dim3(1), 0, b, d + 2, 2000ull);
    HIPCHK(hipStreamSynchronize(a));
    HIPCHK(hipStreamSynchronize(b));
    unsigned long long h[4];
    HIPCHK(hipMemcpy(h, d, sizeof(h), hipMemcpyDeviceToHost));
    HIPCHK(hipFree(d));
    *yes = h[2] < h[1];
    return 0;
}
int ensure_prefill_streams(mellow_engine* e) {
    if (e->n_forks > 0 || e->parent) return 0;
    if (e->streams_probed) {
        if (++e->probe_backoff < 16) { e->prefill_parts = e->prefill_parts_ok; return 0; }
        e->streams_probed = false;
        e->probe_backoff = 0;
        e->prefill_parts = e->prefill_parts_want;
    }
    int nh = e->prefill_parts < 1 ? 1 : (e->prefill_parts > 4 ? 4 : e->prefill_parts);
    for (int h = 1; h < nh; ++h) {
        if (e->stream2[h - 1]) continue;
        bool ok = false;
        for (int attempt = 0; attempt < 8 && !ok; ++attempt) {
            hipStream_t st = nullptr;
            HIPCHK(hipStreamCreateWithFlags(&st, hipStreamNonBlocking));
            int rc = streams_overlap(e, e->stream, st, &ok);
            for (int k = 1; k < h && ok && !rc; ++k) rc = streams_overlap(e, e->stream2[k - 1], st, &ok);
            if (rc) { hipStreamDestroy(st); return rc; }
            if (ok) e->stream2[h - 1] = st; else hipStreamDestroy(st);
        }
        if (!ok) {
            e->prefill_parts_want = e->prefill_parts;
            e->prefill_parts = e->prefill_parts_ok = h;
            e->streams_probed = true;
            break;
        }
    }
    return 0;
}
struct OptDesc { const char* key; const char* dflt; bool answers; const char* what; };
static const OptDesc kOptions[] = {
    {"prefill_split", "2", false, "f32x3: parts of the split LM prefill (1..4); bit-identical for every value"},
    {"prefill_fuse_norm", "1", true, "f32x3: norm-free LM prefill (GEMM epilogues emit split output + RMS partials); 0 = a normalisation launch per GEMM input"},
    {"decode_fuse", "1", true, "down projection of layer l fused with q/k/v of layer l + 1 through the load-time product W'Wd; 0 = five launches per layer"},
    {"decode_fuse_max_rb", "1", true, "largest number of 32-row blocks that runs the fused down + q/k/v launch on fp32 weights"},
    {"splitk", "8", true, "f32x3 encoder: largest split count of the split-K launches (0 = never split; a summation order)"},
    {"enc_apb", "0x1CC", false, "f32x3 encoder: Swin stages whose producers hand over pre-split (bit st, 4 + st, 8 + st); bit-identical"},
    {"graph", "1", false, "decode steps as hipGraph replays (0 = eager launches)"},
    {"fp8_decode", "1", true, "fp8 mode: e4m3 weights in the decode kernels"},
    {"fp8_prefill", "1", true, "fp8 mode: e4m3 GEMMs in encoder + LM prefill"},
    {"fp8_decode_act", "1", true, "fp8 mode: e4m3 activations in the decode GEMM kernels (fp8 matrix pipe)"},
    {"fp8_kv16", "1", true, "fp8 mode: bf16 shadow of the K/V pages for the decode step"},
    {"fp8_attn_bf16", "1", true, "fp8 mode: q / k / v stored once as bf16 (LM: bf16 K/V pages + bf16-once prefill attention; Swin: bf16 q/k/v rows into the exact window attention); 0 = fp32 q/k/v, the 3-way split attention"},
    {"decode_x3", "7", true, "f32x3: mask of decode GEMM launches on the bf16 pipe (1 lm_head, 2 gate/up, 4 fused down + q/k/v)"},
    {"decode_x3_min_rb", "2", true, "f32x3: fewest 32-row blocks at which the layer launches take their f32x3 forms"},
    {"x3_stft", "1", true, "f32x3: STFT / mel GEMMs on the split kernel (0 = exact fp32 kernel)"},
    {"stft_fft", "1", true, "f32x3: STFT as a 1024-point FFT when the checkpoint's conv weights are the windowed DFT basis"},
    {"x3_apb", "1", true, "f32x3 LM prefill: producers hand over pre-split, GEMMs staged by LDS-DMA (0 = register-staged kernel on fp32 activations)"},
    {"x3_attn", "1", true, "f32x3: prefill attention on exact bf16 splits (0 = exact fp32 MFMA kernel)"},
    {"x3w", "1", false, "f32x3: K = 96 GEMMs on the weight-stationary persistent kernel; bit-identical"},
    {"row_migration", "1", false, "reference-semantics loop, B > 32: rows still running are packed into the lowest 32-row blocks; tokens unchanged"},
    {"arena_mb", "3400", false, "size of the weight arena in MiB (before the first tensor is loaded)"},
};
static const OptDesc* find_opt(const char* key) {
    for (const auto& o : kOptions)
        if (!strcmp(o.key, key)) return &o;
    return nullptr;
}
static long opt_val(const mellow_engine* e, const char* key) {
    auto it = e->opt.given.find(key);
    return strtol(it != e->opt.given.end() ? it->second.c_str() : find_opt(key)->dflt, nullptr, 0);
}
int apply_options(mellow_engine* e) {
    const int mode = e->opt.mode;
    e->prefill_parts = (int)opt_val(e, "prefill_split");
    e->opt.prefill_fuse_norm = opt_val(e, "prefill_fuse_norm") != 0;
    e->opt.decode_fuse = opt_val(e, "decode_fuse") != 0;
    e->opt.dec_fuse_max_rb = (int)opt_val(e, "decode_fuse_max_rb");
    e->opt.sk_max = (int)opt_val(e, "splitk");
    e->opt.enc_apb_stages = (int)opt_val(e, "enc_apb");
    e->use_graph = opt_val(e, "graph") != 0;
    e->opt.x3_stft = opt_val(e, "x3_stft") != 0;
    e->opt.stft_fft = opt_val(e, "stft_fft") != 0 && e->opt.x3_stft;
    e->opt.x3_apb = opt_val(e, "x3_apb") != 0;
    e->opt.x3_attn = opt_val(e, "x3_attn") != 0;
    e->opt.x3w = opt_val(e, "x3w") != 0;
    e->opt.row_migration = opt_val(e, "row_migration") != 0;
    e->opt.arena_mb = (int)opt_val(e, "arena_mb");
    e->opt.fp8 = mode == MELLOW_PRECISION_FP8;
    e->opt.fp8_decode = e->opt.fp8 && opt_val(e, "fp8_decode") != 0;
    e->opt.fp8_decode_act = e->opt.fp8_decode && opt_val(e, "fp8_decode_act") != 0;
    e->opt.fp8_prefill = opt_val(e, "fp8_prefill") != 0;
    e->opt.fp8_attn_bf16 = opt_val(e, "fp8_attn_bf16") != 0;
    e->opt.kv16 = e->opt.fp8_decode && opt_val(e, "fp8_kv16") != 0;
    e->opt.f32x3_terms = mode == MELLOW_PRECISION_F32X3 ? 6 : 0;
    e->opt.dec_x3 = mode == MELLOW_PRECISION_F32X3 ? ((int)opt_val(e, "decode_x3") & DEC_X3_ALL) : 0;
    e->opt.dec_x3_min_rb = (int)opt_val(e, "decode_x3_min_rb") < 1 ? 1 : (int)opt_val(e, "decode_x3_min_rb");
    return 0;
}

extern "C" {

int mellow_engine_set_option(mellow_engine_t* e, const char* key, const char* value) {
    if (!e || !key || !value) return fail("null argument");
    if (e->finalized) return fail("options must be set before mellow_engine_finalize");
    const OptDesc* o = find_opt(key);
    if (!o) return fail("unknown option \"%s\" (mellow_engine_describe lists them)", key);
    char* end = nullptr;
    const long v = strtol(value, &end, 0);
    if (end == value || *end) return fail("option \"%s\": \"%s\" is not an integer", key, value);
    if (!strcmp(key, "prefill_split") && (v < 1 || v > 4)) return fail("option prefill_split must be 1..4");
    if (!strcmp(key, "arena_mb") && e->arena) return fail("option arena_mb must be set before the first tensor is loaded");
    e->opt.given[key] = value;
    return apply_options(e);
}

int64_t mellow_engine_describe(mellow_engine_t* e, char* buf, int64_t capacity) {
    if (!e) return -1;
    std::string s = "{\"abi\": [" + std::to_string(MELLOW_ABI_VERSION) + ", " + std::to_string(MELLOW_ABI_MINOR) + "], \"precision\": \"";
    s += e->opt.mode == MELLOW_PRECISION_F32 ? "f32" : e->opt.mode == MELLOW_PRECISION_FP8 ? "fp8" : "f32x3";
    s += "\", \"reads_environment\": false, \"finalized\": ";
    s += e->finalized ? "true" : "false";
    s += ", \"stft_is_fft\": ";
    s += e->w.fft_win ? "true" : "false";
    s += ", \"non_default\": [";
    bool first = true;
    for (const auto& o : kOptions)
        if (opt_val(e, o.key) != strtol(o.dflt, nullptr, 0)) { s += std::string(first ? "" : ", ") + "\"" + o.key + "\""; first = false; }
    s += "], \"options\": {";
    first = true;
    for (const auto& o : kOptions) {
        s += std::string(first ? "" : ", ") + "\"" + o.key + "\": {\"value\": " + std::to_string(opt_val(e, o.key)) + ", \"default\": " +
             std::to_string(strtol(o.dflt, nullptr, 0)) + ", \"changes_answers\": " + (o.answers ? "true" : "false") + "}";
        first = false;
    }
    s += "}}";
    if (buf && capacity > (int64_t)s.size()) memcpy(buf, s.c_str(), s.size() + 1);
    return (int64_t)s.size() + 1;
}

int mellow_last_steps_enqueued(mellow_engine_t* e) { return e ? e->last_steps_enqueued : -1; }

int mellow_last_row_repacks(mellow_engine_t* e) { return e ? e->last_compactions : -1; }

int mellow_stft_is_fft(mellow_engine_t* e) { return e && e->w.fft_win ? 1 : 0; }

int mellow_abi_minor(void) { return MELLOW_ABI_MINOR; }
int mellow_prefill_parts(mellow_engine_t* e) {
    if (!e) return -1;
    if (!e->opt.f32x3_terms && !(e->opt.fp8 && e->opt.fp8_prefill)) return 1;
    if (hipSetDevice(e->device) != hipSuccess) return -1;
    if (ensure_prefill_streams(e) != 0) return -1;
    return e->prefill_parts < 1 ? 1 : (e->prefill_parts > 4 ? 4 : e->prefill_parts);
}

int mellow_prof_enable(mellow_engine_t* e, int on) {
    if (!e) return fail("null engine");
    e->prof_on = on != 0;
    return 0;
}

int mellow_prof_reset(mellow_engine_t* e) {
    if (!e) return fail("null engine");
    hipStreamSynchronize(e->stream);
    e->prof.clear();
    e->ev_used = 0;
    return 0;
}

int mellow_prof_get(mellow_engine_t* e, int i, int64_t* launches, double* ms, double* flops, double* bytes) {
    if (!e || i < 0 || i >= PF_COUNT) return fail("bad argument");
    HIPCHK(hipSetDevice(e->device));
    HIPCHK(hipStreamSynchronize(e->stream));
    int64_t n = 0;
    double t = 0, f = 0, by = 0;
    for (const auto& r : e->prof)
        if (r.fam == i) {
            float m = 0.f;
            HIPCHK(hipEventElapsedTime(&m, r.a, r.b));
            t += m; f += r.flops; by += r.bytes; ++n;
        }
    if (launches) *launches = n;
    if (ms) *ms = t;
    if (flops) *flops = f;
    if (bytes) *bytes = by;
    return 0;
}

int mellow_last_phase_ms(mellow_engine_t* e, float* encode_ms, float* prefill_ms, float* decode_ms) {
    if (!e) return fail("null engine");
    if (encode_ms) *encode_ms = e->phase_ms[0];
    if (prefill_ms) *prefill_ms = e->phase_ms[1];
    if (decode_ms) *decode_ms = e->phase_ms[2];
    return 0;
}

int mellow_engine_set_precision(mellow_engine_t* e, int mode) {
    if (!e) return fail("null engine");
    if (e->finalized) return fail("precision must be chosen before mellow_engine_finalize");
    if (mode != MELLOW_PRECISION_F32 && mode != MELLOW_PRECISION_FP8 && mode != MELLOW_PRECISION_F32X3)
        return fail("unknown precision mode %d", mode);
    e->opt.mode = mode;
    return apply_options(e);
}

int mellow_engine_fork(mellow_engine_t* parent, mellow_engine_t** out) {
    if (!parent || !out) return fail("null argument");
    if (!parent->finalized) return fail("fork needs a finalized engine");
    HIPCHK(hipSetDevice(parent->device));
    HIPCHK(hipStreamSynchronize(parent->stream));
    mellow_engine* c = new mellow_engine();
    c->cfg = parent->cfg; c->device = parent->device; c->finalized = true; c->owns_weights = false;
    c->opt = parent->opt;
    c->w = parent->w;
    c->use_graph = parent->use_graph;
    c->resample_banks = parent->resample_banks;
#define FORK_HIPCHK(x) do { hipError_t e_ = (x); if (e_ != hipSuccess) { mellow_engine_destroy(c); return fail("HIP error %s at %s:%d", hipGetErrorString(e_), __FILE__, __LINE__); } } while (0)
    FORK_HIPCHK(hipStreamCreateWithFlags(&c->stream, hipStreamNonBlocking));
    c->prefill_parts = 1;
    FORK_HIPCHK(hipEventCreateWithFlags(&c->ev_fork, hipEventDisableTiming));
    for (int i = 0; i < 3; ++i) FORK_HIPCHK(hipEventCreateWithFlags(&c->ev_join[i], hipEventDisableTiming));
    for (int i = 0; i < 4; ++i) FORK_HIPCHK(hipEventCreate(&c->ev_phase[i]));
#undef FORK_HIPCHK
    if (alloc_state_words(c)) { mellow_engine_destroy(c); return 1; }
    c->parent = parent;
    if (parent->n_forks++ == 0) { parent->prefill_parts_saved = parent->prefill_parts; parent->prefill_parts = 1; }
    *out = c;
    return 0;
}

// ... 8 lines not shown
```

### mellow_amd/csrc/engine_internal.h

```cpp
#pragma once
#include <hip/hip_runtime.h>

#include <chrono>
#include <cmath>
#include <cstdarg>
#include <cstdio>
#include <cstdlib>
#include <cstring>
#include <map>
#include <unordered_map>
#include <string>
#include <thread>
#include <type_traits>
#include <utility>
#include <vector>

#include "../../include/mellow_hip.h"
#include "kernels.h"

using namespace mellow;

int fail(const char* fmt, ...);
struct mellow_engine;
int apply_options(mellow_engine* e);
#define HIPCHK(expr)                                                                              \
    do {                                                                                          \
        hipError_t _e = (expr);                                                                   \
        if (_e != hipSuccess) return fail("%s failed: %s (%s:%d)", #expr, hipGetErrorString(_e), __FILE__, __LINE__); \
    } while (0)
#define CHK(expr)            \
    do {                     \
        int _r = (expr);     \
        if (_r) return _r;   \
    } while (0)

static const int kDepths[4] = {2, 2, 6, 2};
static const int kHeads[4] = {4, 8, 16, 32};
static const int kWin = 8;
static const int kHop = 320, kNfft = 1024, kNfreq = 513, kMel = 64;
static const int kClasses = 527, kEncOut = 768, kProj = 576;
static const int kLongCrop = 689, kLongHop = 344;
static const char* ENC = "audio_encoder.base.htsat.";
static const char* C2L = "audio_encoder.base.c2l.";
static const char* PRJ = "audio_encoder.projection.";
static const char* LMK = "caption_decoder.lm.";

static inline int rup(int x, int m) { return (x + m - 1) / m * m; }

enum { PF_GEMM = 0, PF_SKINNY, PF_PREFILL_ATTN, PF_DECODE_ATTN, PF_WINDOW_ATTN, PF_NORM, PF_MISC, PF_LM_HEAD, PF_COUNT };
static const char* kFamilyNames[PF_COUNT] = {"gemm_f32_mfma", "skinny_gemm_m32", "prefill_attention",
                                             "decode_attention", "window_attention", "norm", "misc", "lm_head_all_positions"};

struct HostTensor {
    std::vector<char> data;
    std::vector<int64_t> shape;
    int dtype = 0;
    int64_t numel() const {
        int64_t n = 1;
        for (auto d : shape) n *= d;
        return n;
    }
    const float* f() const { return reinterpret_cast<const float*>(data.data()); }
};

struct Packed {
    float* p = nullptr;
    int N = 0, K = 0, NP = 0, KP = 0;
    int Nw = 0;
};

struct SwinBlockW {
    float *n1w, *n1b, *n2w, *n2b;
    Packed qkv, proj, fc1, fc2;
    float *qkv_b, *proj_b, *fc1_b, *fc2_b;
    float* bias_exp;
    float* mask;
};
struct MergeW {
    float *nw, *nb;
    Packed red;
};
struct DecW {
    const float *p, *scale;
};
struct LMLayerW {
    Packed qkv, o, gateup, down;
    Packed qkv_f, gateup_f;
    float* o16 = nullptr;
    float* gu16n = nullptr;
    float* gu16 = nullptr;
    float* qkv2 = nullptr;
    float *q2h8 = nullptr, *q2h_sc = nullptr;
    float *qkv8 = nullptr, *qkv_sc = nullptr, *o8 = nullptr, *o_sc = nullptr, *gu8 = nullptr, *gu_sc = nullptr, *dn8 = nullptr,
          *dn_sc = nullptr;
    float *in_ln, *post_ln;
    DecW qkv_w() const { return qkv8 ? DecW{qkv8, qkv_sc} : DecW{qkv_f.p, nullptr}; }
    DecW o_w() const { return o8 ? DecW{o8, o_sc} : DecW{o16, nullptr}; }
    DecW gateup_w() const { return gu8 ? DecW{gu8, gu_sc} : DecW{gu16, nullptr}; }
    DecW down_w() const { return dn8 ? DecW{dn8, dn_sc} : DecW{down.p, nullptr}; }
};

struct ProfRec {
    int fam;
    hipEvent_t a, b;
    double flops, bytes;
    int M = 0, N = 0, K = 0, epi = 0;
};

#define LOCAL __attribute__((visibility("hidden")))
struct mellow_engine {
    struct Buf {
        float* p = nullptr;
        size_t cap = 0;
        Buf() = default; Buf(const Buf&) = delete; Buf& operator=(const Buf&) = delete;
        Buf(Buf&& o) noexcept : p(o.p), cap(o.cap) { o.p = nullptr; o.cap = 0; }
        Buf& operator=(Buf&& o) noexcept { std::swap(p, o.p); std::swap(cap, o.cap); return *this; }
        LOCAL ~Buf() { if (p) (void)hipFree(p); }
    };
    struct LOCAL Options {
        std::map<std::string, std::string> given;
        int mode = MELLOW_PRECISION_F32X3;
        bool x3_stft = true, stft_fft = true, x3_apb = true, x3_attn = true, x3w = true, row_migration = true, decode_fuse = true;
        int arena_mb = 3400;
        bool kv16 = false;
        bool fp8 = false;
        bool fp8_decode = false;
        bool fp8_decode_act = false;
        bool fp8_attn_bf16 = true;
        bool fp8_prefill = true;
        int dec_x3_min_rb = 2;
        int dec_x3 = 0;
        int f32x3_terms = 0;
        bool prefill_fuse_norm = true;
        int enc_apb_stages = 0x1CC;
        int sk_max = 8;
        int dec_fuse_max_rb = 1;
    };
    struct Fp8W { uint8_t* w8; float* scale; };
    struct LOCAL Weights {
        Packed dft, mel;
        float *fft_win = nullptr, *fft_tw1 = nullptr, *fft_tw2 = nullptr;
        float *bn_alpha = nullptr, *bn_beta = nullptr;
        float *pe_w = nullptr, *pe_b = nullptr, *pe_nw = nullptr, *pe_nb = nullptr;
        std::vector<SwinBlockW> blocks[4];
        MergeW merge[3];
        int32_t* win_map[4][2] = {{nullptr}};
        float *fn_w = nullptr, *fn_b = nullptr;
        Packed tscam, c2l, lin1, lin2;
        float *tscam_b = nullptr, *c2l_b = nullptr, *pln_w = nullptr, *pln_b = nullptr;
        int32_t* emb_row_map = nullptr;
        float* embed = nullptr;
        Packed lm_head;
        std::vector<LMLayerW> layers;
        float* final_norm = nullptr;
        float *rope_cos = nullptr, *rope_sin = nullptr;
        float *head8 = nullptr, *head_sc = nullptr;
        DecW head_w() const { return head8 ? DecW{head8, head_sc} : DecW{lm_head.p, nullptr}; }
        std::unordered_map<const float*, void*> bf_w;
        std::unordered_map<const float*, Fp8W> fp8_w;
    };
    struct LOCAL StepGraphs {
        struct Key {
            int B = -1, Tmax = -1, sample = -1;
            const void *out_tok = nullptr, *blk_live = nullptr, *row_of_slot = nullptr;
            bool operator==(const Key& k) const { return B == k.B && Tmax == k.Tmax && out_tok == k.out_tok && blk_live == k.blk_live && row_of_slot == k.row_of_slot && sample == k.sample; }
        };
        hipGraphExec_t one = nullptr, eight = nullptr;
        Key key;
        StepGraphs() = default; StepGraphs(const StepGraphs&) = delete; StepGraphs& operator=(const StepGraphs&) = delete;
        void reset() {
            for (hipGraphExec_t* x : {&one, &eight}) if (*x) { (void)hipGraphExecDestroy(*x); *x = nullptr; }
        }
        ~StepGraphs() { reset(); }
    };

    mellow_config_t cfg;
    int device = 0;
    hipStream_t stream = nullptr;
    Options opt;
    Weights w;
    bool use_graph = true;
    int prefill_parts = 2;
    bool streams_probed = false;
    int probe_backoff = 0, prefill_parts_ok = 1, prefill_parts_want = 2;
    hipStream_t stream2[3] = {nullptr, nullptr, nullptr};
    hipEvent_t ev_fork = nullptr, ev_join[3] = {nullptr, nullptr, nullptr};
    bool finalized = false;
    bool owns_weights = true;
    std::map<std::string, HostTensor> host;
    std::vector<void*> allocs;
    char* arena = nullptr;
    size_t arena_size = 0, arena_used = 0;
    bool decode_only_weight = false;

    Buf wavcat, wpad, power, logmel, X0, X1, T, QKV, H, ats, fpx, fpxavg, latv, emb33, e1, gbuf, sbuf, proj33;
    Buf lm_x, lm_xn, lm_q, lm_o, lm_h, kcache, vcache;
    Buf kcache16, vcache16;
    bool kv16_direct = false;
    Buf lm_xn3, lm_o3, lm_h3;
    Buf lm_ssq;
    Buf dec;
    Buf dlogits, cand;
    Buf sc_prefix, sc_part, sc_ws;
    Buf sk_ws;
    bool sk_enable = false;
    Buf enc_a3, enc_h3;
    Buf a8, a8_scale;
    DecArgs da;
    int32_t *d_tokens = nullptr, *d_step = nullptr, *d_pos = nullptr, *d_seen = nullptr, *d_nseen = nullptr;
    int32_t *d_arrive = nullptr, *d_ticket = nullptr, *d_params = nullptr;
    int32_t *d_blk_left = nullptr, *d_blk_live = nullptr;
    int32_t *d_row_of_slot = nullptr, *d_ncompact = nullptr;
    int last_compactions = 0;
    unsigned long long* h_progress = nullptr;
    unsigned long long* d_progress = nullptr;
    std::map<std::pair<int, int>, float*> resample_banks;
    int32_t h_params[2] = {0, 0};
    uint32_t* d_sparams = nullptr;
    uint32_t h_sparams[SMP_WORDS] = {0};
    bool sample_on = false;
    int32_t h_blk[64] = {0};
    std::vector<int32_t> h_ident;
    int last_steps_enqueued = 0;
    Buf out_tok;
    int kv_B = 0, kv_Tmax = 0;
    int cur_B = 0, cur_pos = 0;
    int32_t h_pos_word = 0;
    StepGraphs graphs;

    bool taps_on = false;
    std::map<std::string, Buf> taps;
    std::map<std::string, int64_t> tap_numel;

    uint64_t dbg_spans[960] = {};
    int dbg_seq0 = -1;
    mellow_engine* parent = nullptr;
    int n_forks = 0, prefill_parts_saved = 2;

    bool prof_on = false;
    std::vector<ProfRec> prof;
    std::vector<hipEvent_t> ev_pool;
    size_t ev_used = 0;
    hipEvent_t ev_phase[4] = {nullptr, nullptr, nullptr, nullptr};
    float phase_ms[3] = {0, 0, 0};
};

#undef LOCAL
static_assert(!std::is_copy_constructible<mellow_engine::Buf>::value, "a Buf owns its device memory: it moves, it is never copied");
static_assert(std::is_copy_assignable<mellow_engine::Weights>::value && std::is_copy_assignable<mellow_engine::Options>::value, "a fork copies these by assignment: no owning member (Buf, StepGraphs) belongs in them");

int ensure(mellow_engine* e, mellow_engine::Buf& b, size_t floats);
int dev_alloc(mellow_engine* e, float** out, size_t floats);
int upload(mellow_engine* e, float** out, const float* src, size_t floats, size_t alloc_floats = 0);
hipEvent_t next_event(mellow_engine* e);
int tap(mellow_engine* e, const char* name, const float* src, int64_t n);
std::vector<std::string> build_required(const mellow_config_t* cfg);
const std::vector<std::string>& default_required();
bool is_ignored_key(const std::string& k);
void window_map_host(int R, int shift, int32_t* out);
void pack_weight_host(const float* w, int N, int K, int NP, int KP, float* out);
void rope_tables_host(float theta, int head_dim, int P, float* c, float* s);
int alloc_state_words(mellow_engine* e);
struct ProfScope {
    mellow_engine* e;
    ProfRec r;
    bool on;
    ProfScope(mellow_engine* e_, int fam, double flops, double bytes) : e(e_), on(e_->prof_on) {
        if (on) {
            r.fam = fam;
            r.flops = flops;
            r.bytes = bytes;
            r.a = next_event(e);
            r.b = next_event(e);
            hipEventRecord(r.a, e->stream);
        }
    }
    ~ProfScope() {
        if (on) {
            hipEventRecord(r.b, e->stream);
            e->prof.push_back(r);
        }
    }
};
int run_gemm(mellow_engine* e, const GemmArgs& a);
int run_gemm_apb(mellow_engine* e, const GemmArgs& a, const void* a3, hipStream_t st = nullptr, const void* a3_scales = nullptr);
GemmArgs lin(const float* A, int64_t lda, int M, const Packed& w, float* C, int64_t ldc, const float* bias);
int run_encoder(mellow_engine* e, const float* wav, int n, int64_t n_samples, int want_logmel_only, int apply_bn, float* logmel_out);
static inline int rb_of(int B) { return (B + 31) / 32; }
static inline size_t kv_layer_floats(const mellow_engine* e) { return (size_t)e->kv_B * 3 * e->kv_Tmax * 64; }
struct RecordArgs {
    bool embed_next = false;
};
int ensure_lm(mellow_engine* e, int B, int T, int Tmax, int ctx_end = 0);
int clear_page_tails(mellow_engine* e, int T, int t_end);
LoopArgs loop_args(mellow_engine* e);
int run_lm_head(mellow_engine* e, int B, int pending_kcd, const RecordArgs* rec);
int run_prefill(mellow_engine* e, int B, int T, const RecordArgs* rec, bool all_positions = false);
int enqueue_decode_layer_range(mellow_engine* e, int B, int l_begin, int l_end, bool inc_pos);
int enqueue_decode_layers(mellow_engine* e, int B, const RecordArgs* rec);
int ensure_prefill_streams(mellow_engine* e);
int encode_pair_to_prefix(mellow_engine* e, const float* a1, const float* a2, int64_t n_samples, const int32_t* ids, int B, float* prefix_out);
int run_score_head(mellow_engine* e, int B, int T, int from_pos, int n, const int32_t* targets, float* out_logprob,
                   int32_t* out_argmax, float* out_lse, float* out_max);
void clear_bad_id(mellow_engine* e);
int check_bad_id(mellow_engine* e);
```

### mellow_amd/csrc/engine_lm.cpp

```cpp
#include "engine_internal.h"

int ensure_lm(mellow_engine* e, int B, int T, int Tmax, int ctx_end) {
    if (B > 1024) return fail("batch of %d exceeds the 1024 rows one pass takes (mellow_generate chunks larger batches itself; the decode state block is sized for 32 row blocks)", B);
    if (ctx_end <= 0 || ctx_end > Tmax) ctx_end = Tmax;
    if (Tmax > e->cfg.max_positions) return fail("prefix + max_len = %d exceeds max_positions %d", Tmax, e->cfg.max_positions);
    const size_t Mp = (size_t)B * T;
    CHK(ensure(e, e->lm_x, Mp * 576));
    CHK(ensure(e, e->lm_xn, Mp * 576));
    CHK(ensure(e, e->lm_q, Mp * 576));
    CHK(ensure(e, e->lm_o, Mp * 576));
    CHK(ensure(e, e->lm_h, Mp * 1536));
    if (e->opt.f32x3_terms || (e->opt.fp8 && e->opt.fp8_prefill)) {
        const size_t Mq = (size_t)rup((int)Mp, 128) + 3 * 128;
        CHK(ensure(e, e->lm_xn3, Mq * 576 * 6 / 4));
        CHK(ensure(e, e->lm_o3, Mq * 576 * 6 / 4));
        CHK(ensure(e, e->lm_h3, Mq * 1536 * 6 / 4));
        CHK(ensure(e, e->lm_ssq, Mq * 2 * 16));
    }
    e->kv16_direct = e->opt.kv16 && e->opt.fp8 && e->opt.fp8_prefill && e->opt.fp8_attn_bf16 && e->opt.x3_apb && e->opt.x3_attn && !e->w.layers.empty() &&
                     e->w.fp8_w.count(e->w.layers[0].qkv.p) != 0;
    dec_prepare_lds_attributes();
    const int Bp = rb_of(B) * 32;
    if (e->kv_B != Bp || e->kv_Tmax != Tmax) {
        e->kv_B = Bp;
        e->kv_Tmax = Tmax;
        CHK(ensure(e, e->kcache, kv_layer_floats(e) * e->cfg.num_layers));
        CHK(ensure(e, e->vcache, kv_layer_floats(e) * e->cfg.num_layers));
        if (e->opt.kv16) {
            CHK(ensure(e, e->kcache16, kv_layer_floats(e) * e->cfg.num_layers / 2));
            CHK(ensure(e, e->vcache16, kv_layer_floats(e) * e->cfg.num_layers / 2));
        }
        HIPCHK(hipMemsetAsync(e->kcache.p, 0, kv_layer_floats(e) * e->cfg.num_layers * sizeof(float), e->stream));
        HIPCHK(hipMemsetAsync(e->vcache.p, 0, kv_layer_floats(e) * e->cfg.num_layers * sizeof(float), e->stream));
        if (e->opt.kv16) {
            HIPCHK(hipMemsetAsync(e->kcache16.p, 0, kv_layer_floats(e) * e->cfg.num_layers * sizeof(float) / 2, e->stream));
            HIPCHK(hipMemsetAsync(e->vcache16.p, 0, kv_layer_floats(e) * e->cfg.num_layers * sizeof(float) / 2, e->stream));
        }
        e->graphs.reset();
    }
    {
        const size_t RB = (size_t)Bp / 32, V = (size_t)e->cfg.vocab_size;
        const size_t n_x = (size_t)Bp * 576;
        size_t off = 0;
        auto take = [&](size_t n) { size_t o = off; off += (n + 63) / 64 * 64; return o; };
        const size_t o_xmidF = take(n_x), o_xnewR = take(n_x), o_xnF = take(n_x * 3 / 2);
        const size_t o_dslabF = take(DEC_KC_DOWN * n_x), o_ssq1 = take((size_t)Bp * DEC_KC_QKV), o_rope = take(64);
        const size_t o_pq = take((size_t)DEC_KC_QKV * Bp * 960);
        const size_t o_att = take((size_t)DEC_TS * n_x), o_aml = take((size_t)DEC_TS * 9 * Bp * 2);
        const size_t o_ssq = take((size_t)Bp * 40), o_gu = take(RB * 192 * 256), o_xmidF16 = take(n_x);
        const bool x3l = (e->opt.dec_x3 & DEC_X3_GATEUP) && (e->opt.dec_x3 & DEC_X3_QKV) && (int)RB >= e->opt.dec_x3_min_rb && !e->opt.fp8_decode &&
                         e->w.layers.size() > 1 && e->w.layers[1].qkv2 != nullptr && e->w.layers[1].gu16n != nullptr;
        const size_t o_x3a = take(x3l ? n_x * 3 / 2 : 0), o_x3b = take(x3l ? n_x * 3 / 2 : 0), o_h3 = take(x3l ? RB * 192 * 256 * 3 / 2 : 0);
        const bool fresh = e->dec.cap < off;
        CHK(ensure(e, e->dec, off));
        CHK(ensure(e, e->dlogits, (size_t)Bp * V));
        CHK(ensure(e, e->cand, (size_t)2 * Bp * (V / 32)));
        if (fresh) {
            HIPCHK(hipMemsetAsync(e->dec.p, 0, off * sizeof(float), e->stream));
            e->graphs.reset();
        }
        float* p = e->dec.p;
        DecArgs& a = e->da;
        a.rows = Bp; a.RB = (int)RB; a.Tmax = Tmax; a.eps = e->cfg.rms_norm_eps; a.d_pos = e->d_pos; a.inc_pos = 0; a.first = 0;
        a.a8 = e->opt.fp8_decode_act ? 1 : 0;
        a.kv16 = e->opt.kv16 ? 1 : 0;
        a.x3 = e->opt.dec_x3;
        a.blk_live = nullptr;
        a.row_of_slot = nullptr;
        a.rope_cos = e->w.rope_cos; a.rope_sin = e->w.rope_sin;
        a.xmidF = p + o_xmidF; a.xnewR = p + o_xnewR; a.xnF = p + o_xnF;
        a.xn3 = (a.x3 & DEC_X3_HEAD) && !e->w.head8 && dec_head3r_fits(e->cfg.vocab_size) ? (void*)(p + o_xnF) : nullptr;
        a.xmid3_32 = x3l ? (void*)(p + o_x3a) : nullptr; a.xmid3_16 = x3l ? (void*)(p + o_x3b) : nullptr; a.h3 = x3l ? (void*)(p + o_h3) : nullptr;
        a.dslabF = p + o_dslabF; a.slabF_stride4 = (int64_t)(n_x / 4); a.ssq1 = p + o_ssq1; a.rope_cur = p + o_rope;
        {
            const int ng_end = (ctx_end - 1 + 3) / 4, chunk = dec_attn_chunk_groups(e->opt.kv16);
            a.ts = dec_key_splits((int)RB, e->opt.kv16 || e->opt.mode != MELLOW_PRECISION_F32X3);
            int gs = (ng_end + a.ts - 1) / a.ts;
            if (gs > chunk && gs % chunk <= 4) gs -= gs % chunk;
            gs = gs < 1 ? 1 : gs;
            if (gs != a.gs) e->graphs.reset();
            a.gs = gs;
        }
        a.pq = p + o_pq; a.attF16 = p + o_att; a.att_ml = p + o_aml; a.ssq = p + o_ssq; a.guF = p + o_gu; a.xmidF16 = p + o_xmidF16;
        a.logits = e->dlogits.p; a.cand_val = e->cand.p; a.cand_idx = reinterpret_cast<int32_t*>(e->cand.p + (size_t)Bp * (V / 32));
    }
    if (Bp > 1024) return fail("batch too large for the decode state block");
    return 0;
}

int clear_page_tails(mellow_engine* e, int T, int t_end) {
    const int Tmax = e->kv_Tmax;
    if (t_end > Tmax) t_end = Tmax;
    if (T >= t_end) return 0;
    if (e->kv16_direct) launch_clear_page_slots(e->vcache16.p, (int64_t)e->cfg.num_layers * e->kv_B * 3, Tmax, T, t_end, e->stream, true);
    else launch_clear_page_slots(e->vcache.p, (int64_t)e->cfg.num_layers * e->kv_B * 3, Tmax, T, t_end, e->stream);
    HIPCHK(hipGetLastError());
    return 0;
}

LoopArgs loop_args(mellow_engine* e) {
    LoopArgs lp;
    lp.out_tokens = reinterpret_cast<int32_t*>(e->out_tok.p);
    lp.params = e->d_params; lp.seen_stop = e->d_seen; lp.n_seen = e->d_nseen; lp.arrive = e->d_arrive; lp.ticket = e->d_ticket;
    lp.host_progress = e->d_progress; lp.T0 = e->cfg.prefix_len;
    if (e->da.blk_live) { lp.blk_left = e->d_blk_left; lp.blk_live = e->d_blk_live; lp.blk_snap = e->d_blk_live + 32; }
    if (e->da.row_of_slot) { lp.row_of_slot = e->d_row_of_slot; lp.n_compactions = e->d_ncompact; }
    return lp;
}

int run_lm_head(mellow_engine* e, int B, int pending_kcd, const RecordArgs* rec) {
    const int NT = e->cfg.vocab_size / 32, Bp = e->da.rows;
    auto dh = [&](int k) { DecArgs x = e->da; x.dbg_seq = e->dbg_seq0 >= 0 ? e->dbg_seq0 + 5 * e->cfg.num_layers + k : -1000; return x; };
    { ProfScope ps(e, PF_NORM, 0, (double)(pending_kcd + 2) * Bp * 576 * 4);
      launch_dec_final_norm(dh(0), e->w.final_norm, pending_kcd, e->stream); }
    { ProfScope ps(e, PF_SKINNY, 2.0 * Bp * 576.0 * e->cfg.vocab_size, 576.0 * e->cfg.vocab_size * 4);
      const DecW h = e->w.head_w();
      launch_dec_lm_head(dh(1), h.p, e->w.lm_head.KP / 8, e->cfg.vocab_size, e->stream, h.scale); }
    { ProfScope ps(e, PF_MISC, 0, 0);
      if (e->sample_on) {
          SampleArgs sa;
          sa.logits = e->da.logits; sa.ld = e->cfg.vocab_size; sa.prm = e->d_sparams;
          launch_dec_sample(sa, dh(2), B, e->d_tokens, e->w.embed, (rec && rec->embed_next) ? 1 : 0, rec ? loop_args(e) : LoopArgs(),
                            e->stream);
      } else {
          launch_dec_argmax(dh(2), B, NT, e->d_tokens, e->w.embed, (rec && rec->embed_next) ? 1 : 0, rec ? loop_args(e) : LoopArgs(),
                            e->stream);
      }
      if (rec && e->da.row_of_slot) launch_dec_compact(e->da, B, loop_args(e), e->stream); }
    return 0;
}

int run_prefill(mellow_engine* e, int B, int T, const RecordArgs* rec, bool all_positions) {
    hipStream_t s = e->stream;
    const int M = B * T, Tmax = e->kv_Tmax;
    const int NL = e->cfg.num_layers;
    float *x = e->lm_x.p, *xn = e->lm_xn.p;
    const bool amx = e->opt.fp8 && e->opt.fp8_prefill && e->opt.x3_apb && e->w.fp8_w.count(e->w.layers[0].qkv.p) != 0;
    const bool apb = (e->opt.f32x3_terms && e->opt.x3_apb) || amx;
    if (apb && !e->prof_on && (e->prefill_parts > 1 || e->streams_probed)) CHK(ensure_prefill_streams(e));
    int nh = (apb && !e->prof_on) ? e->prefill_parts : 1;
    nh = nh < 1 ? 1 : (nh > 4 ? 4 : nh);
    if (nh > B) nh = B;
    int hb0[4], hB[4];
    size_t prow[4];
    hipStream_t hs[4] = {s, e->stream2[0], e->stream2[1], e->stream2[2]};
    for (int h = 0, b0 = 0, r = 0; h < nh; ++h) {
        hb0[h] = b0; hB[h] = B / nh + (h < B % nh ? 1 : 0); prow[h] = (size_t)r;
        b0 += hB[h]; r += rup(hB[h] * T, 128);
    }
    const bool split = nh > 1;
    struct Join {
        mellow_engine* e; hipStream_t* hs; int nh; bool done;
        int run() {
            if (done) return 0;
            done = true;
            for (int h = 1; h < nh; ++h) {
                HIPCHK(hipEventRecord(e->ev_join[h - 1], hs[h]));
                HIPCHK(hipStreamWaitEvent(hs[0], e->ev_join[h - 1], 0));
            }
            return 0;
        }
        ~Join() { (void)run(); }
    } join{e, hs, nh, !split};
    if (split) {
        HIPCHK(hipEventRecord(e->ev_fork, s));
        for (int h = 1; h < nh; ++h) HIPCHK(hipStreamWaitEvent(hs[h], e->ev_fork, 0));
    }
    for (int l = 0; l < NL; ++l) {
        const LMLayerW& w = e->w.layers[l];
        bool last = false;
        for (int h = 0; h < nh; ++h) {
            hipStream_t st = hs[h];
            const int64_t r0 = (int64_t)hb0[h] * T;
            const int Mh = hB[h] * T, Bh = hB[h];
            float* xh = x + r0 * 576;
            float* xnh = xn + r0 * 576;
            float* qh = e->lm_q.p + r0 * 576;
            float* oh = e->lm_o.p + r0 * 576;
            float* hh = e->lm_h.p + r0 * 1536;
            const bool p16 = amx && e->kv16_direct;
            float* kc = p16 ? e->kcache16.p + (kv_layer_floats(e) * l + (size_t)hb0[h] * 3 * Tmax * 64) / 2
                            : e->kcache.p + kv_layer_floats(e) * l + (size_t)hb0[h] * 3 * Tmax * 64;
            float* vc = p16 ? e->vcache16.p + (kv_layer_floats(e) * l + (size_t)hb0[h] * 3 * Tmax * 64) / 2
                            : e->vcache.p + kv_layer_floats(e) * l + (size_t)hb0[h] * 3 * Tmax * 64;
            char* xn3 = apb ? reinterpret_cast<char*>(e->lm_xn3.p) + prow[h] * 576 * 6 : nullptr;
            char* o3 = apb ? reinterpret_cast<char*>(e->lm_o3.p) + prow[h] * 576 * 6 : nullptr;
            char* h3 = apb ? reinterpret_cast<char*>(e->lm_h3.p) + prow[h] * 1536 * 6 : nullptr;
            char *xn3s = nullptr, *o3s = nullptr, *h3s = nullptr;
            if (amx) {
                xn3s = xn3 + (size_t)rup(Mh, 128) * 576; o3s = o3 + (size_t)rup(Mh, 128) * 576; h3s = h3 + (size_t)rup(Mh, 128) * 1536;
            }
            auto c3_amx = [&](GemmArgs& g, char* scales, int kt64) { if (amx) { g.c3_fmt = 1; g.C3s = reinterpret_cast<uint8_t*>(scales); g.c3_kt64 = kt64; } };
            const bool fz = apb && e->opt.prefill_fuse_norm && w.gateup_f.p != nullptr;
            float* ssq_in = fz ? e->lm_ssq.p + prow[h] * 9 : nullptr;
            float* ssq_mid = fz ? e->lm_ssq.p + e->lm_ssq.cap / 2 + prow[h] * 9 : nullptr;
            auto with_rs = [&](GemmArgs& g, const float* ssq) { g.rs_ssq = ssq; g.rs_parts = 9; g.rs_dim = 576.f; g.rs_eps = e->cfg.rms_norm_eps; };
            (void)ssq_mid;
            const bool fz_in = fz && l > 0;
            if (fz_in) {}
            else if (apb) { ProfScope ps(e, PF_NORM, 0, 2.5 * Mh * 576 * 4); launch_rmsnorm_apb(xh, xn3, Mh, 576, w.in_ln, e->cfg.rms_norm_eps, st, xn3s); }
            else { ProfScope ps(e, PF_NORM, 0, 2.0 * Mh * 576 * 4); launch_rmsnorm(xh, xnh, Mh, 576, w.in_ln, e->cfg.rms_norm_eps, st); }
            {
                GemmArgs g;
                g.A = xnh; g.lda = 576; g.M = Mh; g.K = 576; g.Wp = fz_in ? w.qkv_f.p : w.qkv.p; g.Nw = 960; g.N = 960; g.epi = EPI_QKV_ROPE;
                if (fz_in) with_rs(g, ssq_in);
                g.q_out = qh; g.k_cache = kc; g.v_cache = vc; g.rope_cos = e->w.rope_cos; g.rope_sin = e->w.rope_sin;
                g.T = T; g.Tmax = Tmax; g.q_heads = 9; g.kv_heads = 3; g.kv16 = p16 ? 1 : 0;
                if (apb) CHK(run_gemm_apb(e, g, xn3, st, xn3s)); else CHK(run_gemm(e, g));
            }
            if (l == NL - 1 && !all_positions) { last = true; continue; }
            {
                ProfScope ps(e, PF_PREFILL_ATTN, 4.0 * 64 * 9 * (double)Bh * ((double)T * (T + 1) / 2), 0);
                const bool attn_f32 = !e->opt.x3_attn;
                launch_prefill_attention(qh, kc, vc, oh, apb ? o3 : nullptr, Bh, T, Tmax, (e->opt.f32x3_terms != 0 || amx) && !attn_f32, st, o3s, amx && e->opt.fp8_attn_bf16, p16);
            }
            {
                GemmArgs g = lin(oh, 576, Mh, w.o, xh, 576, nullptr);
                g.resid = xh; g.ldr = 576;
                if (fz) { g.C3 = xn3; g.ssq_out = ssq_mid; g.ssq_parts = 9; c3_amx(g, xn3s, 9); }
                if (apb) CHK(run_gemm_apb(e, g, o3, st, o3s)); else CHK(run_gemm(e, g));
            }
            if (fz) {}
            else if (apb) { ProfScope ps(e, PF_NORM, 0, 2.5 * Mh * 576 * 4); launch_rmsnorm_apb(xh, xn3, Mh, 576, w.post_ln, e->cfg.rms_norm_eps, st, xn3s); }
            else { ProfScope ps(e, PF_NORM, 0, 2.0 * Mh * 576 * 4); launch_rmsnorm(xh, xnh, Mh, 576, w.post_ln, e->cfg.rms_norm_eps, st); }
            {
                GemmArgs g;
                g.A = xnh; g.lda = 576; g.M = Mh; g.K = 576; g.Wp = fz ? w.gateup_f.p : w.gateup.p; g.Nw = 3072; g.N = 1536; g.C = hh; g.ldc = 1536;
                g.epi = EPI_SWIGLU;
                if (fz) with_rs(g, ssq_mid);
                if (apb) { g.C3 = h3; c3_amx(g, h3s, 24); CHK(run_gemm_apb(e, g, xn3, st, xn3s)); } else CHK(run_gemm(e, g));
            }
            {
                GemmArgs g = lin(hh, 1536, Mh, w.down, xh, 576, nullptr);
                g.resid = xh; g.ldr = 576;
                if (fz) { g.C3 = xn3; g.ssq_out = ssq_in; g.ssq_parts = 9; c3_amx(g, xn3s, 9); }
                if (apb) CHK(run_gemm_apb(e, g, h3, st, h3s)); else CHK(run_gemm(e, g));
            }
        }
        if (last) break;
    }
    CHK(join.run());
    if (e->opt.kv16 && !e->kv16_direct && !all_positions) {
        ProfScope ps(e, PF_MISC, 0, 3.0 * kv_layer_floats(e) * NL * 4);
        launch_kv_to_bf16(e->kcache.p, e->kcache16.p, (int64_t)(kv_layer_floats(e) * NL), s);
        launch_kv_to_bf16(e->vcache.p, e->vcache16.p, (int64_t)(kv_layer_floats(e) * NL), s);
    }
    if (all_positions) {
        HIPCHK(hipGetLastError());
        return 0;
    }
    { ProfScope ps(e, PF_MISC, 0, 0); launch_dec_load_rows(e->da, B, x, 576, nullptr, T, 0, s); }
    e->cur_B = B;
    e->cur_pos = T;
    e->h_pos_word = T - 1;
    HIPCHK(hipMemcpyAsync(e->d_pos, &e->h_pos_word, sizeof(int32_t), hipMemcpyHostToDevice, s));
    CHK(enqueue_decode_layer_range(e, B, NL - 1, NL, false));
    CHK(run_lm_head(e, B, DEC_KC_DOWN, rec));
    HIPCHK(hipGetLastError());
    return 0;
}

int enqueue_decode_layer_range(mellow_engine* e, int B, int l_begin, int l_end, bool inc_pos) {
    hipStream_t s = e->stream;
    const int Bp = e->da.rows;
#ifdef MELLOW_DEVPROBE
    static const bool same_w = getenv("MELLOW_DEV_SAME_WEIGHTS") != nullptr, same_kv = getenv("MELLOW_DEV_SAME_KV") != nullptr;
    static const int skip = getenv("MELLOW_DEV_SKIP") ? atoi(getenv("MELLOW_DEV_SKIP")) : 0;
#else
    constexpr bool same_w = false, same_kv = false;
    constexpr int skip = 0;
#endif
    for (int l = l_begin; l < l_end; ++l) {
        const LMLayerW& w = e->w.layers[same_w ? 0 : l];
        const DecW qkv = w.qkv_w(), o = w.o_w(), gu = w.gateup_w(), dn = w.down_w();
        float* kc = e->opt.kv16 ? e->kcache16.p + kv_layer_floats(e) / 2 * (same_kv ? 0 : l) : e->kcache.p + kv_layer_floats(e) * (same_kv ? 0 : l);
        float* vc = e->opt.kv16 ? e->vcache16.p + kv_layer_floats(e) / 2 * (same_kv ? 0 : l) : e->vcache.p + kv_layer_floats(e) * (same_kv ? 0 : l);
        const int kcd = l == l_begin ? 0 : DEC_KC_DOWN;
        const bool x3l = e->da.xmid3_32 != nullptr;
        const bool fuse_rb = x3l || e->da.RB <= e->opt.dec_fuse_max_rb;
        const bool fused_in = l > l_begin && ((w.qkv2 != nullptr && fuse_rb) || w.q2h8 != nullptr) && !same_w;
        DecArgs a = e->da;
        const int sq = e->dbg_seq0 >= 0 ? e->dbg_seq0 + 5 * (l - l_begin) : -1000;
        auto da = [&](int k) { DecArgs x = e->da; x.dbg_seq = sq + k; return x; };
        a.dbg_seq = sq;
        a.first = l == l_begin ? 1 : 0;
        a.inc_pos = (inc_pos && l == l_begin) ? 1 : 0;
        if (!(skip & 1) && !fused_in)
        { ProfScope ps(e, PF_SKINNY, 2.0 * Bp * 576.0 * 960.0, 576.0 * 960.0 * 4);
          launch_dec_qkv(a, qkv.p, w.qkv_f.KP / 8, kcd, s, qkv.scale); }
        if (!(skip & 2))
        { ProfScope ps(e, PF_DECODE_ATTN, 4.0 * 64 * 9 * (double)B * (e->cur_pos + 1), 2.0 * (double)B * 3 * 64 * 4 * (e->cur_pos + 1));
          launch_dec_attn(da(1), kc, vc, fused_in, s); }
        if (!(skip & 4))
        { ProfScope ps(e, PF_SKINNY, 2.0 * Bp * 576.0 * 576.0, 576.0 * 576.0 * 4);
          launch_dec_oproj(da(2), o.p, s, o.scale); }
        if (!(skip & 8))
        { ProfScope ps(e, PF_SKINNY, 2.0 * Bp * 576.0 * 3072.0, 576.0 * 3072.0 * 4);
          if (x3l && !w.gu8) launch_dec_gateup3(da(3), w.gu16n, s);
          else launch_dec_gateup(da(3), gu.p, s, gu.scale); }
        const LMLayerW* nx = (l + 1 < l_end && !same_w) ? &e->w.layers[l + 1] : nullptr;
        if (nx && ((nx->qkv2 && fuse_rb) || nx->q2h8)) {
            if (!(skip & 16))
            { ProfScope ps(e, PF_SKINNY, 2.0 * Bp * (2112.0 * 960.0 + 1536.0 * 576.0), (2112.0 * 960.0 + 1536.0 * 576.0) * (nx->q2h8 ? 1 : 4));
              if (nx->q2h8) launch_dec_qkv2_w8(da(4), nx->qkv8, nx->qkv_sc, nx->q2h8, nx->q2h_sc, w.dn8, w.dn_sc, s);
              else if (x3l) launch_dec_qkv2x3(da(4), nx->qkv2, w.down.p, s);
              else launch_dec_qkv2(da(4), nx->qkv2, w.down.p, s); }
        } else if (!(skip & 16))
        { ProfScope ps(e, PF_SKINNY, 2.0 * Bp * 576.0 * 1536.0, 576.0 * 1536.0 * 4);
          launch_dec_down(da(4), dn.p, w.down.KP / 8, s, dn.scale); }
    }
    return 0;
}
int enqueue_decode_layers(mellow_engine* e, int B, const RecordArgs* rec) {
    CHK(enqueue_decode_layer_range(e, B, 0, e->cfg.num_layers, true));
    CHK(run_lm_head(e, B, DEC_KC_DOWN, rec));
    return 0;
}

static int capture_steps(mellow_engine* e, int B, const RecordArgs* rec, int n, hipGraphExec_t* exec) {
    hipGraph_t gr = nullptr;
    HIPCHK(hipStreamBeginCapture(e->stream, hipStreamCaptureModeThreadLocal));
    int rc = 0;
    for (int k = 0; k < n && !rc; ++k) rc = enqueue_decode_layers(e, B, rec);
    hipError_t err = hipStreamEndCapture(e->stream, &gr);
    if (!rc && err != hipSuccess) rc = fail("hipStreamEndCapture failed: %s", hipGetErrorString(err));
    if (!rc && (err = hipGraphInstantiate(exec, gr, nullptr, nullptr, 0)) != hipSuccess) { *exec = nullptr; rc = fail("instantiating the captured decode step failed: %s", hipGetErrorString(err)); }
    if (gr) (void)hipGraphDestroy(gr);
    return rc;
}

int encode_pair_to_prefix(mellow_engine* e, const float* a1, const float* a2, int64_t n_samples, const int32_t* ids,
                                 int B, float* prefix_out) {
    mellow_engine::Buf& cat = e->wavcat;
    CHK(ensure(e, cat, (size_t)2 * B * n_samples));
    HIPCHK(hipMemcpyAsync(cat.p, a1, (size_t)B * n_samples * 4, hipMemcpyDeviceToDevice, e->stream));
    HIPCHK(hipMemcpyAsync(cat.p + (size_t)B * n_samples, a2, (size_t)B * n_samples * 4, hipMemcpyDeviceToDevice, e->stream));
    CHK(run_encoder(e, cat.p, 2 * B, n_samples, 0, 1, nullptr));
    { ProfScope ps(e, PF_MISC, 0, 0);
      launch_prefix_assemble(e->proj33.p, e->w.embed, ids, B, e->cfg.text_len, e->cfg.sep_token_id, e->cfg.vocab_size, prefix_out,
                             e->d_progress + 1, e->stream); }
    HIPCHK(hipGetLastError());
    return 0;
}

void clear_bad_id(mellow_engine* e) { __atomic_store_n(e->h_progress + 1, 0ull, __ATOMIC_RELEASE); }

int check_bad_id(mellow_engine* e) {
    const unsigned long long w = __atomic_load_n(e->h_progress + 1, __ATOMIC_ACQUIRE);
    if (!w) return 0;
    return fail("index out of range in self: prompt id %d of example %u is outside the vocabulary [0, %d)", (int)(unsigned)(w & 0xffffffffu),
                (unsigned)((w >> 32) & 0x7fffffffu), e->cfg.vocab_size);
}

static int wait_ticket(mellow_engine* e, unsigned want, unsigned* nseen) {
    const auto t0 = std::chrono::steady_clock::now();
    for (unsigned spins = 1;; ++spins) {
        const unsigned long long v = __atomic_load_n(e->h_progress, __ATOMIC_ACQUIRE);
        if ((unsigned)(v >> 32) >= want) {
            if (nseen) *nseen = (unsigned)(v & 0xffffffffu);
            return 0;
        }
        if ((spins & 0x3ff) == 0) {
            const hipError_t q = hipStreamQuery(e->stream);
            if (q == hipSuccess) {
                const unsigned long long v2 = __atomic_load_n(e->h_progress, __ATOMIC_ACQUIRE);
                if ((unsigned)(v2 >> 32) >= want) continue;
                return fail("decode progress word stalled at ticket %u (wanted %u) with an idle stream", (unsigned)(v2 >> 32), want);
            }
            if (q != hipErrorNotReady) return fail("stream error while waiting for a decode step: %s", hipGetErrorString(q));
            if (std::chrono::steady_clock::now() - t0 > std::chrono::seconds(60))
                return fail("timed out waiting for decode ticket %u", want);
        }
#if defined(__x86_64__) || defined(__i386__)
        __builtin_ia32_pause();
#elif defined(__aarch64__)
        __asm__ __volatile__("yield");
#endif
        if (spins > 4096) std::this_thread::yield();
    }
}

static void clear_bad_target(mellow_engine* e) { __atomic_store_n(e->h_progress + 2, 0ull, __ATOMIC_RELEASE); }
static int check_bad_target(mellow_engine* e, const char* what, int lo) {
    const unsigned long long w = __atomic_load_n(e->h_progress + 2, __ATOMIC_ACQUIRE);
    if (!w) return 0;
    return fail("index out of range in self: %s id %d of row %u is outside [%d, %d)", what, (int)(unsigned)(w & 0xffffffffu),
                (unsigned)((w >> 32) & 0x7fffffffu), lo, e->cfg.vocab_size);
}

int run_score_head(mellow_engine* e, int B, int T, int from_pos, int n, const int32_t* targets, float* out_logprob,
                   int32_t* out_argmax, float* out_lse, float* out_max) {
    hipStream_t s = e->stream;
    const int V = e->cfg.vocab_size, rows = B * n, groups = V / 64;
    if (V % 64 != 0 || e->w.lm_head.Nw != V) return fail("the scoring head tiles the vocabulary in groups of 64 columns (vocab %d)", V);
    const size_t ld = (size_t)rup(rows, 64);
    CHK(ensure(e, e->sc_part, (size_t)groups * ld * 3));
    float2* part_ms = reinterpret_cast<float2*>(e->sc_part.p);
    int32_t* part_arg = reinterpret_cast<int32_t*>(e->sc_part.p + (size_t)groups * ld * 2);
    float* tgt_logit = e->sc_ws.p;
    GemmArgs g = lin(e->lm_xn.p, 576, rows, e->w.lm_head, nullptr, 0, nullptr);
    g.epi = EPI_LSE;
    g.lse_target = targets; g.lse_ms = part_ms; g.lse_arg = part_arg; g.lse_tgt = tgt_logit; g.lse_ld = (int64_t)ld;
    ProfScope ps(e, PF_LM_HEAD, gemm_flops(g), 576.0 * V * 4 + (double)rows * 576 * 4 + 3.0 * rows * groups * 12);
    launch_gather_span(e->lm_x.p, B, T, from_pos, n, e->lm_o.p, s);
    launch_rmsnorm(e->lm_o.p, e->lm_xn.p, rows, 576, e->w.final_norm, e->cfg.rms_norm_eps, s);
    launch_gemm(g, s);
    launch_lse_merge(part_ms, part_arg, (int64_t)ld, groups, rows, targets, tgt_logit, V, out_logprob, out_argmax, out_lse, out_max,
                     e->d_progress + 2, s);
    HIPCHK(hipGetLastError());
    return 0;
}

extern "C" {

int mellow_prefix(mellow_engine_t* e, const float* audio1, const float* audio2, int64_t n_samples, const int32_t* input_ids,
                  int B, float* out) {
    if (!e || !e->finalized) return fail("engine not finalized");
    if (!audio1 || !audio2 || !input_ids || !out) return fail("null argument");
    if (B <= 0) return fail("B must be positive");
    HIPCHK(hipSetDevice(e->device));
    clear_bad_id(e);
    CHK(encode_pair_to_prefix(e, audio1, audio2, n_samples, input_ids, B, out));
    HIPCHK(hipStreamSynchronize(e->stream));
    return check_bad_id(e);
}

int mellow_lm_prefill(mellow_engine_t* e, const float* prefix, int B, int T, int reserve, float* logits) {
    if (!e || !e->finalized) return fail("engine not finalized");
    if (!prefix || B <= 0 || T <= 0 || reserve < 0) return fail("bad argument");
    HIPCHK(hipSetDevice(e->device));
    CHK(ensure_lm(e, B, T, T + reserve + 1));
    HIPCHK(hipMemcpyAsync(e->lm_x.p, prefix, (size_t)B * T * 576 * 4, hipMemcpyDeviceToDevice, e->stream));
    CHK(clear_page_tails(e, T, e->kv_Tmax));
    CHK(run_prefill(e, B, T, nullptr));
    if (logits)
        HIPCHK(hipMemcpyAsync(logits, e->dlogits.p, (size_t)B * e->cfg.vocab_size * 4, hipMemcpyDeviceToDevice, e->stream));
    HIPCHK(hipStreamSynchronize(e->stream));
    return 0;
}

int mellow_lm_decode_step(mellow_engine_t* e, const int32_t* token_ids, float* logits) {
    if (!e || !e->finalized) return fail("engine not finalized");
    if (!token_ids) return fail("null argument");
    if (e->cur_B <= 0) return fail("decode step without a prefill");
    if (e->cur_pos + 1 > e->kv_Tmax) return fail("KV pages exhausted (reserve too small)");
    HIPCHK(hipSetDevice(e->device));
    const int B = e->cur_B;
    launch_dec_load_rows(e->da, B, e->w.embed, 576, token_ids, 0, e->cfg.vocab_size, e->stream);
    CHK(enqueue_decode_layers(e, B, nullptr));
    e->cur_pos += 1;
    if (logits)
        HIPCHK(hipMemcpyAsync(logits, e->dlogits.p, (size_t)B * e->cfg.vocab_size * 4, hipMemcpyDeviceToDevice, e->stream));
    HIPCHK(hipGetLastError());
    HIPCHK(hipStreamSynchronize(e->stream));
    return 0;
}

int mellow_debug_dec_head(mellow_engine_t* e, const float* x, int B, int act_fp8, float* logits) {
    if (!e || !e->finalized) return fail("engine not finalized");
    if (!x || !logits || B <= 0 || B > 1024) return fail("bad argument");
    if (e->cfg.hidden_size != 576) return fail("the decode kernels are built for hidden size 576");
    HIPCHK(hipSetDevice(e->device));
// ... 360 lines not shown
```

### mellow_amd/csrc/kernels.h

```cpp
#pragma once
#include <hip/hip_runtime.h>
#include <stdint.h>

namespace mellow {

void launch_pack_weight(const float* w, int N, int K, int64_t ldw, float* out, int NP, int KP, hipStream_t s);
void launch_pack_weight_pairs(const float* w0, const float* w1, int N, int K, int64_t ldw, float* out, int NP,
                              int KP, hipStream_t s);

enum { ACT_NONE = 0, ACT_GELU = 1, ACT_SIGMOID = 2 };
enum { EPI_LINEAR = 0, EPI_POWER = 1, EPI_LOGMEL = 2, EPI_SWIGLU = 3, EPI_QKV_ROPE = 4, EPI_LSE = 5 };
enum { A_PLAIN = 0, A_FRAMES = 1 };

struct GemmArgs {
    const float* A = nullptr;
    int64_t lda = 0;
    int M = 0;
    int K = 0;
    int a_mode = A_PLAIN;
    int fpc = 1;
    int64_t clip_stride = 0;
    int hop = 0;
    const float* Wp = nullptr;
    int Nw = 0;
    int N = 0;
    float* C = nullptr;
    int64_t ldc = 0;
    const float* bias = nullptr;
    const float* resid = nullptr;
    int64_t ldr = 0;
    const int32_t* crow_map = nullptr;
    int rows_in = 1, rows_out = 1;
    int act = ACT_NONE;
    int epi = EPI_LINEAR;
    const float* bn_alpha = nullptr;
    const float* bn_beta = nullptr;
    int apply_bn = 0;
    float* q_out = nullptr;
    float* k_cache = nullptr;
    float* v_cache = nullptr;
    const float* rope_cos = nullptr;
    const float* rope_sin = nullptr;
    int T = 1, Tmax = 1, q_heads = 9, kv_heads = 3;
    int c16 = 0;
    int kv16 = 0;
    void* C3 = nullptr;
    float* sk_ws = nullptr;
    int sk_tiles = 0, sk_max = 0;
    bool no_x3w = false;
    float* ssq_out = nullptr;
    int ssq_parts = 0;
    const float* rs_ssq = nullptr;
    int rs_parts = 0;
    float rs_dim = 1.f, rs_eps = 0.f;
    const uint8_t* A8 = nullptr;
    int64_t lda8 = 0;
    const uint32_t* a_sc = nullptr;
    const uint8_t* W8 = nullptr;
    const float* w_scale = nullptr;
    int c3_fmt = 0;
    uint8_t* C3s = nullptr;
    int c3_kt64 = 0;
    const int32_t* lse_target = nullptr;
    float2* lse_ms = nullptr;
    int32_t* lse_arg = nullptr;
    float* lse_tgt = nullptr;
    int64_t lse_ld = 0;
};
void launch_gemm(const GemmArgs& a, hipStream_t s);
void launch_quant_mx8(const float* A, int64_t lda, int M, int K, void* img, void* sc, hipStream_t s);
void launch_pack_fp8(const float* Wp, int NP, int KP, uint8_t* W8, float* w_scale, hipStream_t s);
void launch_gemm_fp8(const GemmArgs& a, hipStream_t s);
void launch_pack_bf16x3(const float* Wp, int NP, int KP, void* PB, hipStream_t s);
void launch_gemm_bf16x3_fused(const GemmArgs& a, hipStream_t s);
void launch_split_rows_apb(const float* A, int64_t lda, int M, int K, void* out, hipStream_t s);
void launch_gemm_bf16x3_apb(const GemmArgs& a, hipStream_t s);
double gemm_flops(const GemmArgs& a);

void set_max_dynamic_lds(const void* fn, size_t bytes);

constexpr int DEC_KC_QKV = 8;
#ifndef MELLOW_DEC_KC_DOWN
#define MELLOW_DEC_KC_DOWN 8
#endif
constexpr int DEC_KC_DOWN = MELLOW_DEC_KC_DOWN;
#ifndef MELLOW_DEC_TS
#define MELLOW_DEC_TS 2
#endif
constexpr int DEC_TS = MELLOW_DEC_TS;
#ifndef MELLOW_DEC_TS_MULTI
#define MELLOW_DEC_TS_MULTI 1
#endif
constexpr int DEC_TS_MULTI = MELLOW_DEC_TS_MULTI;
inline int dec_key_splits(int RB, bool fixed) { return RB <= 1 || fixed ? DEC_TS : DEC_TS_MULTI; }
#ifndef MELLOW_Q2_HC
#define MELLOW_Q2_HC 4
#endif
#ifndef MELLOW_Q2_WAVES
#define MELLOW_Q2_WAVES 12
#else
#define MELLOW_Q2_WAVES_FORCED 1
#endif
constexpr int Q2_HC = MELLOW_Q2_HC, Q2_WAVES = MELLOW_Q2_WAVES;
constexpr int Q2_NPQ = 2 + Q2_HC;
constexpr int Q2_K8 = 72 + 192;
constexpr int Q2_BLOCKS = 60 + 48 * Q2_HC;
static_assert(Q2_NPQ <= DEC_KC_QKV && Q2_HC <= DEC_KC_DOWN, "the fused kernel reuses the slab buffers of the split-K kernels");
enum { DEC_X3_HEAD = 1, DEC_X3_GATEUP = 2, DEC_X3_QKV = 4, DEC_X3_ALL = 7 };
struct DecArgs {
    int rows = 0, RB = 0;
    int Tmax = 0;
    float eps = 1e-5f;
    int32_t* d_pos = nullptr;
    int first = 0;
    int inc_pos = 0;
    int gs = 1;
    int ts = DEC_TS;
    float* rope_cur = nullptr;
    float* ssq1 = nullptr;
    const float* rope_cos = nullptr;
    const float* rope_sin = nullptr;
    float* xmidF = nullptr;
    float* xnewR = nullptr;
    float* dslabF = nullptr;
    int64_t slabF_stride4 = 0;
    float* pq = nullptr;
    float* attF16 = nullptr;
    float* att_ml = nullptr;
    float* ssq = nullptr;
    float* xmidF16 = nullptr;
    float* guF = nullptr;
    float* xnF = nullptr;
    void *xmid3_32 = nullptr, *xmid3_16 = nullptr, *h3 = nullptr;
    void* xn3 = nullptr;
    const int32_t* blk_live = nullptr;
    int32_t* blk_snap = nullptr;
    const int32_t* row_of_slot = nullptr;
    int kv16 = 0;
    int a8 = 0;
    int x3 = 0;
    int dbg_seq = -1;
    float* logits = nullptr;
    float* cand_val = nullptr; int32_t* cand_idx = nullptr;
};
void launch_dec_qkv(const DecArgs& a, const float* Wp_folded, int K8p, int kcd, hipStream_t s, const float* wscale = nullptr);
void launch_pack_dec_fp8(const float* Wp, int tiles, int slots_per_tile, int rows_per_tile, void* out, float* scale, hipStream_t s);
void launch_dec_attn(const DecArgs& a, float* k_cache, float* v_cache, bool fused, hipStream_t s);
void launch_kv_to_bf16(const float* src, void* dst, int64_t n, hipStream_t s);
void launch_dec_qkv2(const DecArgs& a, const float* Wq2, const float* Wd, hipStream_t s);
void launch_dec_qkv2x3(const DecArgs& a, const float* Wq2, const float* Wd, hipStream_t s);
void dec_prepare_lds_attributes();
void launch_dec_gateup3(const DecArgs& a, const float* Wp16n_folded_pairs, hipStream_t s);
void launch_dec_qkv2_w8(const DecArgs& a, const float* Wx8, const float* sc_x, const float* Wh8, const float* sc_h,
                        const float* Wd8, const float* sc_d, hipStream_t s);
void launch_compose_f64(const float* A, const float* B, float* C, int M, int N, int K, hipStream_t s);
int dec_attn_chunk_groups(bool kv16);
void launch_dec_oproj(const DecArgs& a, const float* Wp16, hipStream_t s, const float* wscale = nullptr);
void launch_dec_gateup(const DecArgs& a, const float* Wp16_folded_pairs, hipStream_t s, const float* wscale = nullptr);
void launch_dec_down(const DecArgs& a, const float* Wp, int K8p, hipStream_t s, const float* wscale = nullptr);
void launch_dec_final_norm(const DecArgs& a, const float* norm_w, int kcd, hipStream_t s);
bool dec_head3r_fits(int vocab);
void launch_dec_lm_head(const DecArgs& a, const float* Wp, int K8p, int vocab, hipStream_t s, const float* wscale = nullptr);
struct LoopArgs {
    int32_t* out_tokens = nullptr;
    const int32_t* params = nullptr;
    int32_t* seen_stop = nullptr;
    int32_t* n_seen = nullptr;
    int32_t* arrive = nullptr;
    int32_t* ticket = nullptr;
    int32_t* blk_left = nullptr;
    int32_t* blk_live = nullptr;
    const int32_t* blk_snap = nullptr;
    int32_t* row_of_slot = nullptr;
    int32_t* n_compactions = nullptr;
    unsigned long long* host_progress = nullptr;
    int T0 = 0;
};
void launch_dec_argmax(const DecArgs& a, int B, int n_tiles, int32_t* tokens, const float* embed, int write_x,
                       const LoopArgs& loop, hipStream_t s);
enum { SMP_SEED_LO = 0, SMP_SEED_HI, SMP_ROW_OFF, SMP_TOP_P, SMP_TEMP, SMP_STEP, SMP_WORDS = 8 };
struct SampleArgs {
    const float* logits = nullptr;
    int64_t ld = 0;
    const uint32_t* prm = nullptr;
    const int32_t* row_ids = nullptr;
};
constexpr int SAMPLE_MAX_V = 49152;
void launch_dec_sample(const SampleArgs& sa, const DecArgs& a, int B, int32_t* tokens, const float* embed, int write_x,
                       const LoopArgs& loop, hipStream_t s);
void launch_sample_logits(const SampleArgs& sa, int B, int32_t* tokens, hipStream_t s);
void launch_dec_compact(const DecArgs& a, int B, const LoopArgs& loop, hipStream_t s);
void launch_dec_load_rows(const DecArgs& a, int B, const float* in, int64_t ld, const int32_t* row_ids, int T_last,
                          int n_src , hipStream_t s);
void launch_pack_weight16(const float* w, int N, int K, float* out, hipStream_t s);
void launch_pack_weight16n(const float* w, int N, int K, float* out, hipStream_t s);
void set_kernel_debug_buffer(uint64_t* p);
void set_gemm_debug_buffer(uint64_t* p);

void launch_resample(const float* x, int n_clips, int64_t n_in, const float* wT, int orig, int nw, int klen, int width,
                     float* out, int64_t n_out, hipStream_t s);
void launch_reflect_pad(const float* wav, int n_clips, int64_t n_samples, float* out, int64_t padded_len, int pad,
                        hipStream_t s);
void launch_fold_patch_embed(const float* logmel_bn, int n_src, int src_frames, int n_crops, int crop_hop,
                             int crop_len, const float* conv_w, const float* conv_b, const float* ln_w,
                             const float* ln_b, float* x0, hipStream_t s);

void launch_layernorm(const float* in, float* out, int M, int C, const float* w, const float* b,
                      const int32_t* row_map, int ntok, hipStream_t s);
void launch_merge_layernorm(const float* in, float* out, int n, int R, int C, const float* w, const float* b,
                            hipStream_t s);
void launch_stft_fft_power(const float* wpad, int fpc, int64_t clip_stride, int hop, int M, const float* win, const float* tw1,
                           const float* tw2, float* power, hipStream_t s);
void launch_rmsnorm(const float* in, float* out, int M, int C, const float* w, float eps, hipStream_t s);
void launch_layernorm_apb(const float* in, void* out_apb, int M, int C, const float* w, const float* b, const int32_t* row_map,
                          int ntok, hipStream_t s, void* out_scales = nullptr);
void launch_rmsnorm_apb(const float* in, void* out_apb, int M, int C, const float* w, float eps, hipStream_t s, void* out_scales = nullptr);

void launch_window_attention(const float* qkv, float* out, int M, int C, int nH, const float* bias_exp,
                             const float* mask, int nW, hipStream_t s, void* out_apb = nullptr, bool qkv16 = false);

void launch_tail_latent_im2col(const float* y, int n, float* latent, int64_t latent_stride, float* a_ts,
                               hipStream_t s);
void launch_crop_average(const float* in, int n, int n_crops, int64_t len, int64_t in_stride, float* out,
                         int64_t out_stride, hipStream_t s);
void launch_gelu(const float* in, float* out, int64_t n, hipStream_t s);
void launch_prefix_assemble(const float* proj33, const float* embed, const int32_t* ids, int B, int text_len,
                            int sep_id, int vocab, float* prefix, unsigned long long* bad_id_word, hipStream_t s);
void launch_gather_rows(const float* table, int width, const int32_t* ids, int n, int n_rows, float* out, hipStream_t s);
void launch_gather_span(const float* in, int B, int T, int from_pos, int n, float* out, hipStream_t s);
void launch_clear_page_slots(float* cache, int64_t pages, int Tmax, int t0, int t1, hipStream_t s, bool pages16 = false);
void launch_downsample33(const float* proj33, int n, float* out, hipStream_t s);

void launch_prefill_attention(const float* q, const float* k_cache, const float* v_cache, float* o, void* o_apb, int B, int T,
                              int Tmax, bool x3, hipStream_t s, void* o_scales = nullptr, bool bf16_once = false, bool pages16 = false);
void launch_lse_merge(const float2* part_ms, const int32_t* part_arg, int64_t ld, int groups, int rows, const int32_t* targets,
                      const float* tgt_logit, int vocab, float* out_logprob, int32_t* out_argmax, float* out_lse, float* out_max,
                      unsigned long long* bad_word, hipStream_t s);
void launch_score_build_input(const float* prefix, const float* embed, const int32_t* cand_ids, const int32_t* cand_len, int K,
                              int L, int P, int vocab, int row0, int nr, float* x, int32_t* targets, unsigned long long* bad_word,
                              hipStream_t s);
void launch_score_sum(const float* logprob, const int32_t* cand_len, int rows, int L, float* out_sum, hipStream_t s);
void launch_argmax(const float* logits, int B, int V, int64_t ld, int32_t* tokens, hipStream_t s);

}
```

Measured before the change: 453.1.

## Fuse final norm, split-k down reduction and argmax into decode tail kernels

For single-row-block f32x3 decode, the last layer's down projection now finishes its split-k reduction in the last-arriving workgroup per tile using a ticket counter and coherent loads and stores. The lm_head kernel computes the final RMSNorm in its prologue, and its last workgroup performs the global argmax plus token and loop bookkeeping. Together these drop two launches per decode step. In exchange it adds atomic tickets, cross-workgroup coherence traffic and redundant norm work in every lm_head workgroup.

```diff
diff --git a/mellow_amd/csrc/decode.hip b/mellow_amd/csrc/decode.hip
--- a/mellow_amd/csrc/decode.hip
+++ b/mellow_amd/csrc/decode.hip
@@ -91,6 +91,35 @@
 #else
     *p = v;
 #endif
+}
+__device__ __forceinline__ void st_coh(float4* p, float4 v) {
+    const f32x4 r = {v.x, v.y, v.z, v.w};
+    asm volatile("global_store_dwordx4 %0, %1, off sc0 sc1" ::"v"(p), "v"(r) : "memory");
+}
+__device__ __forceinline__ void ld_coh8(const float4* p, int64_t stride, float4 (&x)[8]) {
+    f32x4 r0, r1, r2, r3, r4, r5, r6, r7;
+    asm volatile("global_load_dwordx4 %0, %8, off sc0 sc1\n\t"
+                 "global_load_dwordx4 %1, %9, off sc0 sc1\n\t"
+                 "global_load_dwordx4 %2, %10, off sc0 sc1\n\t"
+                 "global_load_dwordx4 %3, %11, off sc0 sc1\n\t"
+                 "global_load_dwordx4 %4, %12, off sc0 sc1\n\t"
+                 "global_load_dwordx4 %5, %13, off sc0 sc1\n\t"
+                 "global_load_dwordx4 %6, %14, off sc0 sc1\n\t"
+                 "global_load_dwordx4 %7, %15, off sc0 sc1\n\t"
+                 "s_waitcnt vmcnt(0)"
+                 : "=&v"(r0), "=&v"(r1), "=&v"(r2), "=&v"(r3), "=&v"(r4), "=&v"(r5), "=&v"(r6), "=&v"(r7)
+                 : "v"(p), "v"(p + stride), "v"(p + 2 * stride), "v"(p + 3 * stride), "v"(p + 4 * stride), "v"(p + 5 * stride),
+                   "v"(p + 6 * stride), "v"(p + 7 * stride)
+                 : "memory");
+    const f32x4 r[8] = {r0, r1, r2, r3, r4, r5, r6, r7};
+#pragma unroll
+    for (int s = 0; s < 8; ++s) x[s] = make_float4(r[s][0], r[s][1], r[s][2], r[s][3]);
+}
+__device__ __forceinline__ bool last_ticket(int32_t* cnt, int n, int* word) {
+    __syncthreads();
+    if (threadIdx.x == 0) *word = __hip_atomic_fetch_add(cnt, 1, __ATOMIC_RELAXED, __HIP_MEMORY_SCOPE_AGENT);
+    __syncthreads();
+    return *word == n - 1;
 }
 #ifdef MELLOW_HOIST_ON
 #define MELLOW_HOIST(x) asm volatile("" ::"s"(x))
@@ -973,6 +1002,97 @@
 }
 
 
+__device__ __forceinline__ void head_tail_epilogue(i32x4* lds, i32x4* ext, float bv, int bi, int N, const DecArgs& a, const HeadTail& t) {
+    float* cv = reinterpret_cast<float*>(ext);
+    int* ci = reinterpret_cast<int*>(ext) + 256;
+    int* word = reinterpret_cast<int*>(ext) + 512 + 32;
+    int* tok = reinterpret_cast<int*>(ext) + 512 + 64;
+    const int tid = threadIdx.x, lane = tid & 63, wave = tid >> 6, m = tid & 31;
+    if (lane < 32) { cv[wave * 32 + m] = bv; ci[wave * 32 + m] = bi; }
+    __syncthreads();
+    if (tid < 32) {
+        float best = cv[tid];
+        int idx = ci[tid];
+#pragma unroll
+        for (int w = 1; w < 8; ++w)
+            if (arg_better(cv[w * 32 + tid], ci[w * 32 + tid], best, idx)) { best = cv[w * 32 + tid]; idx = ci[w * 32 + tid]; }
+        __hip_atomic_store(a.tail_cand + (int64_t)blockIdx.x * 32 + tid, ((unsigned long long)__float_as_uint(best) << 32) | (unsigned)idx,
+                           __ATOMIC_RELAXED, __HIP_MEMORY_SCOPE_AGENT);
+    }
+    asm volatile("s_waitcnt vmcnt(0)" ::: "memory");
+    const int nwg = (int)gridDim.x;
+    if (!last_ticket(a.tail_cnt + DEC_TAIL_HEAD, nwg, word)) return;
+    const LoopArgs& lp = t.lp;
+    const bool rec = lp.out_tokens != nullptr, mine = tid < 32 && tid < t.B;
+    int max_len = 0, stop_id = 0, step = 0, seen = 0;
+    if (rec && mine) {
+        max_len = lp.params[0]; stop_id = lp.params[1];
+        step = *a.d_pos - lp.T0 + 1;
+        seen = lp.seen_stop[tid];
+    }
+    const int grp = tid >> 5;
+    float best = -INFINITY;
+    int idx = 0x7fffffff;
+    for (int w0 = 0; w0 < nwg; w0 += 16 * 12) {
+        unsigned long long g[12];
+#pragma unroll
+        for (int j = 0; j < 12; ++j) {
+            const int w = w0 + grp + 16 * j;
+            g[j] = __hip_atomic_load(a.tail_cand + (int64_t)(w < nwg ? w : 0) * 32 + m, __ATOMIC_RELAXED, __HIP_MEMORY_SCOPE_AGENT);
+        }
+#pragma unroll
+        for (int j = 0; j < 12; ++j) {
+            const float v = __uint_as_float((unsigned)(g[j] >> 32));
+            const int id = (int)(unsigned)g[j];
+            if (w0 + grp + 16 * j < nwg && arg_better(v, id, best, idx)) { best = v; idx = id; }
+        }
+    }
+    float* pv = reinterpret_cast<float*>(lds);
+    int* pi = reinterpret_cast<int*>(lds) + 512;
+    pv[tid] = best; pi[tid] = idx;
+    __syncthreads();
+    if (tid < 32) {
+#pragma unroll
+        for (int q = 1; q < 16; ++q)
+            if (arg_better(pv[q * 32 + tid], pi[q * 32 + tid], best, idx)) { best = pv[q * 32 + tid]; idx = pi[q * 32 + tid]; }
+        idx = min(max(idx, 0), N - 1);
+        tok[tid] = idx;
+        if (mine) {
+            t.tokens[tid] = idx;
+            if (rec) {
+                if (step >= 0 && step < max_len) lp.out_tokens[(int64_t)tid * max_len + step] = idx;
+                if (idx == stop_id && seen == 0) {
+                    lp.seen_stop[tid] = 1;
+                    atomicAdd(lp.n_seen, 1);
+                }
+            }
+        }
+        if (rec) {
+            asm volatile("s_waitcnt vmcnt(0)" ::: "memory");
+            if (tid == 0) {
+                const int tk = *lp.ticket + 1;
+                *lp.ticket = tk;
+                const int ns = atomicAdd(lp.n_seen, 0);
+                __hip_atomic_store(lp.host_progress, ((unsigned long long)(unsigned)tk << 32) | (unsigned)ns, __ATOMIC_RELAXED,
+                                   __HIP_MEMORY_SCOPE_SYSTEM);
+            }
+        }
+        if (tid == 0) __hip_atomic_store(a.tail_cnt + DEC_TAIL_HEAD, 0, __ATOMIC_RELAXED, __HIP_MEMORY_SCOPE_AGENT);
+    }
+    if (t.write_x) {
+        __syncthreads();
+        const int n4 = t.B * 144;
+#pragma unroll
+        for (int j = 0; j < 9; ++j) {
+            const int e = tid + 512 * j;
+            if (e < n4) {
+                const int row = e / 144, c = e % 144;
+                reinterpret_cast<float4*>(a.xmidF)[f32_idx(0, 72, row, c * 4)] = reinterpret_cast<const float4*>(t.embed + (int64_t)tok[row] * 576)[c];
+            }
+        }
+    }
+}
+
 #ifndef MELLOW_H3_NW
 #define MELLOW_H3_NW 8
 #endif
@@ -986,11 +1106,13 @@
 #define MELLOW_H3R_D4 1
 #endif
 constexpr int H3_NW = MELLOW_H3_NW, H3_CP = 3, H3_NC = 36 / H3_CP;
-template <int G, int D, bool BLK>
+constexpr int H3_TAIL_LDS = 4096;
+template <int G, int D, bool BLK, bool TAIL>
 __global__ __launch_bounds__(H3_NW * 64) void dec_head3r_kernel(const float* __restrict__ Wp, const i32x4* __restrict__ X3, int K8p, int N,
-                                                                int RB_p, const DecArgs a) {
+                                                                int RB_p, const DecArgs a, const HeadTail t) {
     kspan(a.dbg_seq, 0);
     extern __shared__ __attribute__((aligned(16))) i32x4 xs[];
+    static_assert(!TAIL || (G == 1 && !BLK && H3_NW == 8), "the fused tail serves one row block");
     constexpr int PPH = 36 / G, NCH = PPH / H3_CP;
     constexpr int STAGE = G * PPH * 3 * 64;
     static_assert(PPH * G == 36 && NCH * H3_CP == PPH && H3_NC % D == 0 && NCH % D == 0, "phases hold whole chunks");
@@ -1011,21 +1133,61 @@
             for (int i = 0; i < 2 * H3_CP; ++i) wn[d][i] = ldg_nt(wbase + (d * 2 * H3_CP + i) * 64);
         for (int ph = 0; ph < G; ++ph) {
             if (ph || rb0) __syncthreads();
-            {
+            if constexpr (TAIL) {
+                float* sq = reinterpret_cast<float*>(xs);
+                float* rinv = reinterpret_cast<float*>(xs + STAGE) + 512;
+                const int m = lane & 31, h = lane >> 5;
+                float4 v[9], wv[9];
+#pragma unroll
+                for (int j = 0; j < 9; ++j) {
+                    const int tl = wave + 8 * j;
+                    v[j] = reinterpret_cast<const float4*>(a.xnF)[tl * 64 + lane];
+                    wv[j] = reinterpret_cast<const float4*>(t.norm_w)[2 * tl + h];
+                }
+#pragma unroll
+                for (int j = 0; j < 9; ++j) sq[m * 145 + 2 * (wave + 8 * j) + h] = f4ssq(v[j]);
+                __syncthreads();
+#pragma unroll
+                for (int r = 0; r < 4; ++r) {
+                    const int row = 4 * wave + r;
+                    float part[3];
+#pragma unroll
+                    for (int q = 0; q < 3; ++q) {
+                        const int xi = 64 * q + lane;
+                        const float ss = wave_sum(xi < 144 ? sq[row * 145 + xi] : 0.f);
+                        part[q] = __uint_as_float(__builtin_amdgcn_readfirstlane(__float_as_uint(ss)));
+                    }
+                    if (lane == 0) rinv[row] = 1.0f / sqrtf((part[0] + part[1] + part[2]) / 576.0f + a.eps);
+                }
+                __syncthreads();
+                const float r = rinv[m];
+                uint2* xs2 = reinterpret_cast<uint2*>(xs);
+#pragma unroll
+                for (int j = 0; j < 9; ++j) {
+                    const int tl = wave + 8 * j;
+                    float4 y;
+                    y.x = __fmul_rn(wv[j].x, __fmul_rn(v[j].x, r)); y.y = __fmul_rn(wv[j].y, __fmul_rn(v[j].y, r));
+                    y.z = __fmul_rn(wv[j].z, __fmul_rn(v[j].z, r)); y.w = __fmul_rn(wv[j].w, __fmul_rn(v[j].w, r));
+                    const F3Quad q = f3_split4(y);
+                    const int slot = (tl >> 1) * 3 * 64 + m + 32 * (tl & 1);
+#pragma unroll
+                    for (int c = 0; c < 3; ++c) xs2[(slot + 64 * c) * 2 + h] = q.p[c];
+                }
+            } else {
                 constexpr int FILL = (STAGE + H3_NW * 64 - 1) / (H3_NW * 64);
-                i32x4 t[FILL];
+                i32x4 tf[FILL];
 #pragma unroll
                 for (int j = 0; j < FILL; ++j) {
                     const int i = tid + j * H3_NW * 64;
                     if (i < STAGE) {
                         const int g = i / (PPH * 3 * 64), rest = i % (PPH * 3 * 64);
-                        t[j] = X3[(((int64_t)(rb0 + (g < gn ? g : 0)) * 36 + ph * PPH) * 3) * 64 + rest];
+                        tf[j] = X3[(((int64_t)(rb0 + (g < gn ? g : 0)) * 36 + ph * PPH) * 3) * 64 + rest];
                     }
                 }
 #pragma unroll
                 for (int j = 0; j < FILL; ++j) {
                     const int i = tid + j * H3_NW * 64;
-                    if (i < STAGE) xs[i] = t[j];
+                    if (i < STAGE) xs[i] = tf[j];
                 }
             }
             __syncthreads();
@@ -1063,6 +1225,8 @@
             }
         }
         const int m = lane & 31, h = lane >> 5;
+        float tail_bv = -INFINITY;
+        int tail_bi = 0x7fffffff;
 #pragma unroll
         for (int g = 0; g < G; ++g) {
             if (g < gn && !(BLK && a.blk_live[rb0 + g] == 0)) {
@@ -1082,12 +1246,17 @@
                 const float ov = __uint_as_float(h ? rv[0] : rv[1]);
                 const int oi = (int)(h ? ri[0] : ri[1]);
                 if (arg_better(ov, oi, bv, bi)) { bv = ov; bi = oi; }
-                if (h == 0) {
+                if (TAIL && t.argmax) {
+                    tail_bv = bv; tail_bi = bi;
+                } else if (h == 0) {
                     const int64_t o = row * (N >> 5) + nt;
                     a.cand_val[o] = bv;
                     a.cand_idx[o] = bi;
                 }
             }
+        }
+        if constexpr (TAIL) {
+            if (t.argmax) head_tail_epilogue(xs, xs + STAGE, tail_bv, tail_bi, N, a, t);
         }
     }
     kspan(a.dbg_seq, 1);
@@ -1458,7 +1627,7 @@
 #endif
 constexpr int DN_WAVES = MELLOW_DOWN_WAVES;
 static_assert(DN_WAVES >= 4 && 192 % (8 * DN_WAVES) == 0, "the epilogue needs 256 threads; waves must divide the k-tiles");
-template <bool BLK, int W8>
+template <bool BLK, int W8, bool FIN>
 __global__ __launch_bounds__(DN_WAVES * 64) void dec_down_kernel(const float* __restrict__ Wp, const float* __restrict__ guF_p, int K8p,
                                                                  const DecArgs a, const float* __restrict__ wscale) {
     kspan(a.dbg_seq, 0);
@@ -1523,7 +1692,25 @@
 #pragma unroll
             for (int j = 0; j < 4; ++j) v[j] *= wscale[n + j];
         }
-        reinterpret_cast<float4*>(a.dslabF)[(int64_t)kc * a.slabF_stride4 + f32_idx(rb, 72, mm, n)] = make_float4(v[0], v[1], v[2], v[3]);
+        float4* dst = reinterpret_cast<float4*>(a.dslabF) + (int64_t)kc * a.slabF_stride4 + f32_idx(rb, 72, mm, n);
+        if constexpr (FIN) st_coh(dst, make_float4(v[0], v[1], v[2], v[3]));
+        else *dst = make_float4(v[0], v[1], v[2], v[3]);
+    }
+    if constexpr (FIN) {
+        static_assert(DEC_KC_DOWN == 8, "ld_coh8 reads eight slabs");
+        asm volatile("s_waitcnt vmcnt(0)" ::: "memory");
+        if (last_ticket(a.tail_cnt + nt, DEC_KC_DOWN, reinterpret_cast<int*>(red))) {
+            if (tid < 256) {
+                const int64_t fi = ((int64_t)rb * 72 + nt * 4) * 64 + tid;
+                float4 x = reinterpret_cast<const float4*>(a.xmidF)[fi];
+                float4 xs[8];
+                ld_coh8(reinterpret_cast<const float4*>(a.dslabF) + fi, a.slabF_stride4, xs);
+#pragma unroll
+                for (int s = 0; s < 8; ++s) x = f4add(x, xs[s]);
+                reinterpret_cast<float4*>(a.xnF)[fi] = x;
+            }
+            if (tid == 0) __hip_atomic_store(a.tail_cnt + nt, 0, __ATOMIC_RELAXED, __HIP_MEMORY_SCOPE_AGENT);
+        }
     }
     kstamp(4, 4, dbg);
     kspan(a.dbg_seq, 1);
@@ -1915,9 +2102,10 @@
 template <class F> static inline void with_head3r(int rb, bool blk, F&& f) {
     with_int<1, 2, 4>(rb, [&](auto g) { with_bool(blk, [&](auto b) {
         constexpr int G = g.value, D = G == 1 ? MELLOW_H3R_D1 : G == 2 ? MELLOW_H3R_D2 : MELLOW_H3R_D4;
-        f(&dec_head3r_kernel<G, D, b.value>, dec_head3r_lds());
+        f(&dec_head3r_kernel<G, D, b.value, false>, dec_head3r_lds());
     }); });
 }
+template <class F> static inline void with_head3r_tail(F&& f) { f(&dec_head3r_kernel<1, MELLOW_H3R_D1, false, true>, dec_head3r_lds() + H3_TAIL_LDS); }
 void launch_dec_qkv2x3(const DecArgs& a, const float* Wq2, const float* Wd, hipStream_t s) {
     const float* Wh = Wq2 + (size_t)72 * 64 * 4;
     const i32x4 *x3 = reinterpret_cast<const i32x4*>(a.xmid3_32), *h3 = reinterpret_cast<const i32x4*>(a.h3);
@@ -1978,8 +2166,13 @@
     });
 }
 void launch_dec_down(const DecArgs& a, const float* Wp, int K8p, hipStream_t s, const float* wscale) {
+    if (a.fin) {
+        if (a.RB != 1 || a.blk_live || wscale || !a.tail_cnt) { fprintf(stderr, "mellow: fused last down launch outside its scope\n"); abort(); }
+        hipLaunchKernelGGL((dec_down_kernel<false, 0, true>), dim3(18, DEC_KC_DOWN, 1), dim3(DN_WAVES * 64), 0, s, Wp, (const float*)a.guF, K8p, a, wscale);
+        return;
+    }
     with_blk_w8(a, wscale, [&](auto blk, auto w8) {
-        hipLaunchKernelGGL((dec_down_kernel<blk.value, w8.value>), dim3(18, DEC_KC_DOWN, a.RB), dim3(DN_WAVES * 64), 0, s, Wp, (const float*)a.guF,
+        hipLaunchKernelGGL((dec_down_kernel<blk.value, w8.value, false>), dim3(18, DEC_KC_DOWN, a.RB), dim3(DN_WAVES * 64), 0, s, Wp, (const float*)a.guF,
                            K8p, a, wscale);
     });
 }
@@ -1995,13 +2188,23 @@
         const i32x4* X3 = reinterpret_cast<const i32x4*>(a.xn3);
         with_head3r(a.RB, a.blk_live != nullptr, [&](auto* kernel, size_t lds) {
             set_max_dynamic_lds(reinterpret_cast<const void*>(kernel), lds);
-            hipLaunchKernelGGL(kernel, dim3(vocab / 32 / H3_NW), dim3(H3_NW * 64), lds, s, Wp, X3, K8p, vocab, a.RB, a);
+            hipLaunchKernelGGL(kernel, dim3(vocab / 32 / H3_NW), dim3(H3_NW * 64), lds, s, Wp, X3, K8p, vocab, a.RB, a, HeadTail());
         });
         return;
     }
     with_blk_w8(a, wscale, [&](auto blk, auto w8) {
         hipLaunchKernelGGL((dec_fullk_kernel<OUT_LOGITS, blk.value, w8.value>), dim3(vocab / 32, 1, a.RB), dim3(LM_WAVES * 64), 0, s, Wp,
                            (const float*)a.xnF, K8p, vocab, a, wscale);
+    });
+}
+void launch_dec_lm_head_tail(const DecArgs& a, const float* Wp, int K8p, int vocab, const HeadTail& t, hipStream_t s) {
+    if (a.RB != 1 || a.blk_live || a.row_of_slot || !(a.x3 & DEC_X3_HEAD) || !dec_head3r_fits(vocab) || !a.tail_cnt || !a.tail_cand || !t.norm_w || t.B > 32) {
+        fprintf(stderr, "mellow: fused head launch outside its scope\n");
+        abort();
+    }
+    with_head3r_tail([&](auto* kernel, size_t lds) {
+        set_max_dynamic_lds(reinterpret_cast<const void*>(kernel), lds);
+        hipLaunchKernelGGL(kernel, dim3(vocab / 32 / H3_NW), dim3(H3_NW * 64), lds, s, Wp, (const i32x4*)nullptr, K8p, vocab, 1, a, t);
     });
 }
 void dec_prepare_lds_attributes() {
@@ -2012,6 +2215,7 @@
             with_qkv2x3(rb, blk, raise);
             with_gateup3(rb, blk, raise);
         }
+    with_head3r_tail(raise);
 }
 __global__ __launch_bounds__(256) void pack_dec_fp8_kernel(const float4* __restrict__ Wp, int slots, int rows, uint32_t* __restrict__ out,
                                                            float* __restrict__ scale) {
diff --git a/mellow_amd/csrc/engine.cpp b/mellow_amd/csrc/engine.cpp
--- a/mellow_amd/csrc/engine.cpp
+++ b/mellow_amd/csrc/engine.cpp
@@ -289,6 +289,7 @@
     e->d_seen = e->d_tokens + 2048;
     e->d_row_of_slot = e->d_tokens + 3072;
     e->d_ncompact = e->d_tokens + 1029;
+    e->d_tail_cnt = e->d_tokens + 1152;
     HIPCHK(hipHostMalloc(reinterpret_cast<void**>(&e->h_progress), 64, hipHostMallocMapped | hipHostMallocCoherent));
     *e->h_progress = 0;
     HIPCHK(hipHostGetDevicePointer(reinterpret_cast<void**>(&e->d_progress), e->h_progress, 0));
@@ -360,6 +361,7 @@
     {"fp8_decode_act", "1", true, "fp8 mode: e4m3 activations in the decode GEMM kernels (fp8 matrix pipe)"},
     {"fp8_kv16", "1", true, "fp8 mode: bf16 shadow of the K/V pages for the decode step"},
     {"fp8_attn_bf16", "1", true, "fp8 mode: q / k / v stored once as bf16 (LM: bf16 K/V pages + bf16-once prefill attention; Swin: bf16 q/k/v rows into the exact window attention); 0 = fp32 q/k/v, the 3-way split attention"},
+    {"decode_tail_fused", "1", false, "f32x3, one 32-row block: final norm in the lm_head's prologue, arg-max + loop bookkeeping in its last workgroup (122 launches per step); 0 = a launch each (124); bit-identical"},
     {"decode_x3", "7", true, "f32x3: mask of decode GEMM launches on the bf16 pipe (1 lm_head, 2 gate/up, 4 fused down + q/k/v)"},
     {"decode_x3_min_rb", "2", true, "f32x3: fewest 32-row blocks at which the layer launches take their f32x3 forms"},
     {"x3_stft", "1", true, "f32x3: STFT / mel GEMMs on the split kernel (0 = exact fp32 kernel)"},
@@ -384,6 +386,7 @@
     e->prefill_parts = (int)opt_val(e, "prefill_split");
     e->opt.prefill_fuse_norm = opt_val(e, "prefill_fuse_norm") != 0;
     e->opt.decode_fuse = opt_val(e, "decode_fuse") != 0;
+    e->opt.tail_fused = opt_val(e, "decode_tail_fused") != 0;
     e->opt.dec_fuse_max_rb = (int)opt_val(e, "decode_fuse_max_rb");
     e->opt.sk_max = (int)opt_val(e, "splitk");
     e->opt.enc_apb_stages = (int)opt_val(e, "enc_apb");
diff --git a/mellow_amd/csrc/engine_internal.h b/mellow_amd/csrc/engine_internal.h
--- a/mellow_amd/csrc/engine_internal.h
+++ b/mellow_amd/csrc/engine_internal.h
@@ -134,6 +134,7 @@
         bool prefill_fuse_norm = true;
         int enc_apb_stages = 0x1CC;
         int sk_max = 8;
+        bool tail_fused = true;
         int dec_fuse_max_rb = 1;
     };
     struct Fp8W { uint8_t* w8; float* scale; };
@@ -210,6 +211,7 @@
     int32_t *d_tokens = nullptr, *d_step = nullptr, *d_pos = nullptr, *d_seen = nullptr, *d_nseen = nullptr;
     int32_t *d_arrive = nullptr, *d_ticket = nullptr, *d_params = nullptr;
     int32_t *d_blk_left = nullptr, *d_blk_live = nullptr;
+    int32_t* d_tail_cnt = nullptr;
     int32_t *d_row_of_slot = nullptr, *d_ncompact = nullptr;
     int last_compactions = 0;
     unsigned long long* h_progress = nullptr;
@@ -295,6 +297,7 @@
 int clear_page_tails(mellow_engine* e, int T, int t_end);
 LoopArgs loop_args(mellow_engine* e);
 int run_lm_head(mellow_engine* e, int B, int pending_kcd, const RecordArgs* rec);
+bool tail_fused(const mellow_engine* e);
 int run_prefill(mellow_engine* e, int B, int T, const RecordArgs* rec, bool all_positions = false);
 int enqueue_decode_layer_range(mellow_engine* e, int B, int l_begin, int l_end, bool inc_pos);
 int enqueue_decode_layers(mellow_engine* e, int B, const RecordArgs* rec);
diff --git a/mellow_amd/csrc/engine_lm.cpp b/mellow_amd/csrc/engine_lm.cpp
--- a/mellow_amd/csrc/engine_lm.cpp
+++ b/mellow_amd/csrc/engine_lm.cpp
@@ -51,6 +51,7 @@
         const bool x3l = (e->opt.dec_x3 & DEC_X3_GATEUP) && (e->opt.dec_x3 & DEC_X3_QKV) && (int)RB >= e->opt.dec_x3_min_rb && !e->opt.fp8_decode &&
                          e->w.layers.size() > 1 && e->w.layers[1].qkv2 != nullptr && e->w.layers[1].gu16n != nullptr;
         const size_t o_x3a = take(x3l ? n_x * 3 / 2 : 0), o_x3b = take(x3l ? n_x * 3 / 2 : 0), o_h3 = take(x3l ? RB * 192 * 256 * 3 / 2 : 0);
+        const size_t o_tcand = take(V / 256 * 32 * 2);
         const bool fresh = e->dec.cap < off;
         CHK(ensure(e, e->dec, off));
         CHK(ensure(e, e->dlogits, (size_t)Bp * V));
@@ -82,6 +83,8 @@
             a.gs = gs;
         }
         a.pq = p + o_pq; a.attF16 = p + o_att; a.att_ml = p + o_aml; a.ssq = p + o_ssq; a.guF = p + o_gu; a.xmidF16 = p + o_xmidF16;
+        a.fin = 0; a.tail_cnt = e->d_tail_cnt; a.tail_cand = reinterpret_cast<unsigned long long*>(p + o_tcand);
+        HIPCHK(hipMemsetAsync(e->d_tail_cnt, 0, DEC_TAIL_WORDS * sizeof(int32_t), e->stream));
         a.logits = e->dlogits.p; a.cand_val = e->cand.p; a.cand_idx = reinterpret_cast<int32_t*>(e->cand.p + (size_t)Bp * (V / 32));
     }
     if (Bp > 1024) return fail("batch too large for the decode state block");
@@ -108,9 +111,29 @@
     return lp;
 }
 
+bool tail_fused(const mellow_engine* e) {
+    const DecArgs& a = e->da;
+    return e->opt.tail_fused && a.RB == 1 && !a.blk_live && !a.row_of_slot && a.xn3 && a.tail_cnt && a.tail_cand;
+}
+
 int run_lm_head(mellow_engine* e, int B, int pending_kcd, const RecordArgs* rec) {
     const int NT = e->cfg.vocab_size / 32, Bp = e->da.rows;
     auto dh = [&](int k) { DecArgs x = e->da; x.dbg_seq = e->dbg_seq0 >= 0 ? e->dbg_seq0 + 5 * e->cfg.num_layers + k : -1000; return x; };
+    if (tail_fused(e) && pending_kcd == DEC_KC_DOWN) {
+        HeadTail t;
+        t.norm_w = e->w.final_norm; t.argmax = e->sample_on ? 0 : 1; t.B = B; t.tokens = e->d_tokens; t.embed = e->w.embed;
+        t.write_x = (rec && rec->embed_next) ? 1 : 0;
+        if (rec) t.lp = loop_args(e);
+        { ProfScope ps(e, PF_SKINNY, 2.0 * Bp * 576.0 * e->cfg.vocab_size, 576.0 * e->cfg.vocab_size * 4);
+          launch_dec_lm_head_tail(dh(1), e->w.lm_head.p, e->w.lm_head.KP / 8, e->cfg.vocab_size, t, e->stream); }
+        if (e->sample_on) {
+            ProfScope ps(e, PF_MISC, 0, 0);
+            SampleArgs sa;
+            sa.logits = e->da.logits; sa.ld = e->cfg.vocab_size; sa.prm = e->d_sparams;
+            launch_dec_sample(sa, dh(2), B, e->d_tokens, e->w.embed, t.write_x, rec ? loop_args(e) : LoopArgs(), e->stream);
+        }
+        return 0;
+    }
     { ProfScope ps(e, PF_NORM, 0, (double)(pending_kcd + 2) * Bp * 576 * 4);
       launch_dec_final_norm(dh(0), e->w.final_norm, pending_kcd, e->stream); }
     { ProfScope ps(e, PF_SKINNY, 2.0 * Bp * 576.0 * e->cfg.vocab_size, 576.0 * e->cfg.vocab_size * 4);
@@ -307,7 +330,9 @@
               else launch_dec_qkv2(da(4), nx->qkv2, w.down.p, s); }
         } else if (!(skip & 16))
         { ProfScope ps(e, PF_SKINNY, 2.0 * Bp * 576.0 * 1536.0, 576.0 * 1536.0 * 4);
-          launch_dec_down(da(4), dn.p, w.down.KP / 8, s, dn.scale); }
+          DecArgs d = da(4);
+          d.fin = (l + 1 == e->cfg.num_layers && tail_fused(e)) ? 1 : 0;
+          launch_dec_down(d, dn.p, w.down.KP / 8, s, dn.scale); }
     }
     return 0;
 }
diff --git a/mellow_amd/csrc/kernels.h b/mellow_amd/csrc/kernels.h
--- a/mellow_amd/csrc/kernels.h
+++ b/mellow_amd/csrc/kernels.h
@@ -142,7 +142,11 @@
     int dbg_seq = -1;
     float* logits = nullptr;
     float* cand_val = nullptr; int32_t* cand_idx = nullptr;
-};
+    int fin = 0;
+    int32_t* tail_cnt = nullptr;
+    unsigned long long* tail_cand = nullptr;
+};
+constexpr int DEC_TAIL_HEAD = 24, DEC_TAIL_WORDS = 32;
 void launch_dec_qkv(const DecArgs& a, const float* Wp_folded, int K8p, int kcd, hipStream_t s, const float* wscale = nullptr);
 void launch_pack_dec_fp8(const float* Wp, int tiles, int slots_per_tile, int rows_per_tile, void* out, float* scale, hipStream_t s);
 void launch_dec_attn(const DecArgs& a, float* k_cache, float* v_cache, bool fused, hipStream_t s);
@@ -161,6 +165,8 @@
 void launch_dec_final_norm(const DecArgs& a, const float* norm_w, int kcd, hipStream_t s);
 bool dec_head3r_fits(int vocab);
 void launch_dec_lm_head(const DecArgs& a, const float* Wp, int K8p, int vocab, hipStream_t s, const float* wscale = nullptr);
+struct HeadTail;
+void launch_dec_lm_head_tail(const DecArgs& a, const float* Wp, int K8p, int vocab, const HeadTail& t, hipStream_t s);
 struct LoopArgs {
     int32_t* out_tokens = nullptr;
     const int32_t* params = nullptr;
@@ -176,6 +182,15 @@
     unsigned long long* host_progress = nullptr;
     int T0 = 0;
 };
+struct HeadTail {
+    const float* norm_w = nullptr;
+    int argmax = 0;
+    int B = 0;
+    int32_t* tokens = nullptr;
+    const float* embed = nullptr;
+    int write_x = 0;
+    LoopArgs lp;
+};
 void launch_dec_argmax(const DecArgs& a, int B, int n_tiles, int32_t* tokens, const float* embed, int write_x,
                        const LoopArgs& loop, hipStream_t s);
 enum { SMP_SEED_LO = 0, SMP_SEED_HI, SMP_ROW_OFF, SMP_TOP_P, SMP_TEMP, SMP_STEP, SMP_WORDS = 8 };
```

Result: slower. 448.3 (-1.1%).
